# 42yeah/GSRast

Measured on AMD Instinct MI355X. Metric: forward_msplats_per_s, higher is better.
Workload: dtype f32

## Files before the change

### gsrast_amd/_capi.py

```python
from __future__ import annotations

import ctypes as C
import os

import torch

_HERE = os.path.dirname(os.path.abspath(__file__))
_TAG = os.environ.get("GSR_LIB_TAG", "")
LIB_PATH = os.path.join(_HERE, "lib", f"libgsrast_amd{'_' + _TAG if _TAG else ''}.so")

GSR_OK = 0
GSR_ERR_INVALID_ARG = 1
GSR_ERR_ALLOC = 2
GSR_ERR_HIP = 3
GSR_ERR_NO_DEVICE = 4
GSR_ERR_TOO_LARGE = 5
GSR_ERR_INTERNAL = 6
GSR_ERR_STALE_RECEIPT = 7

GSR_FLAG_PROFILE = 0x1
GSR_FLAG_COUNT_STAGED = 0x2
GSR_FLAG_SEMANTICS_INRIA = 0x4
GSR_FLAG_PLAN_SORT = 0x8
GSR_FLAG_PLAN_BLOCKS = 0x10
GSR_FLAG_OVERLAP_EMIT = 0x20
GSR_FLAG_NO_SORTED_LISTS = 0x40
GSR_FLAG_NO_TILE_HISTORY = 0x80
GSR_FLAG_SERIAL_EMIT = 0x100
GSR_FLAG_NO_DEEP_TILES = 0x200
GSR_FLAG_DEEP_TILES_ALL = 0x400
GSR_FLAG_DEEP_WAVES_8 = 0x800
GSR_FLAG_DEEP_WAVES_16 = 0x1000
GSR_FLAG_DEPTH_INVERSE = 0x2000
GSR_PLAN_LISTS_SKIPPED = 0x100
GSR_PLAN_BLEND_FROM_LISTS = 0x200
GSR_PLAN_TILES_REORDERED = 0x400
GSR_PLAN_EMIT_OVERLAPPED = 0x800
GSR_PLAN_COLORS_BESIDE = 0x1000
GSR_PLAN_TILE_ORDER_DROPPED = 0x2000
GSR_PLAN_DEEP_TILES = 0x4000
GSR_SH_LAYOUT_FILE, GSR_SH_LAYOUT_COEFFICIENT_MAJOR = 0, 1
PLAN_NAMES = {0: "none", 1: "sort", 2: "blocks", 3: "generic"}
GSR_NUM_STAGES = 8
STAGE_NAMES = ("preprocess", "scan", "depth_order", "duplicate", "sort_pass1", "sort_pass2", "ranges", "blend")

ALLOC_FN = C.CFUNCTYPE(C.c_void_p, C.c_void_p, C.c_size_t)


class GeometryState(C.Structure):
    _fields_ = [("tiles_touched", C.c_void_p), ("scan_size", C.c_size_t), ("num_rendered", C.c_uint32),
                ("scanning_space", C.c_void_p), ("depths", C.c_void_p), ("clamped", C.c_void_p),
                ("internal_radii", C.c_void_p), ("means2D", C.c_void_p), ("cov3D", C.c_void_p),
                ("conic_opacity", C.c_void_p), ("rgb", C.c_void_p), ("point_offsets", C.c_void_p)]


class ImageState(C.Structure):
    _fields_ = [("ranges", C.c_void_p), ("n_contrib", C.c_void_p), ("accum_alpha", C.c_void_p)]


class BinningState(C.Structure):
    _fields_ = [("keys_unsorted", C.c_void_p), ("keys", C.c_void_p), ("values_unsorted", C.c_void_p),
                ("values", C.c_void_p), ("sorting_size", C.c_size_t), ("sorting_space", C.c_void_p)]


GSR_RECEIPT_MAGIC = 0x31525347
GSR_LISTS_SKIPPED_STAMP = 0xFFFFFFFF


class ForwardReceipt(C.Structure):
    _fields_ = [("magic", C.c_uint32), ("plan_used", C.c_uint32),
                ("num_gaussians", C.c_int32), ("width", C.c_int32), ("height", C.c_int32),
                ("tile_row_begin", C.c_int32), ("tile_row_end", C.c_int32),
                ("num_rendered", C.c_uint32), ("num_visible", C.c_uint32), ("serial", C.c_uint32),
                ("geometry_chunk", C.c_void_p), ("image_chunk", C.c_void_p), ("binning_chunk", C.c_void_p),
                ("async_words", C.c_void_p), ("tile_history", C.c_void_p)]

    def copy(self) -> "ForwardReceipt":
        r = ForwardReceipt()
        C.memmove(C.byref(r), C.byref(self), C.sizeof(ForwardReceipt))
        return r


class ForwardArgs(C.Structure):
    _fields_ = [
        ("struct_size", C.c_uint32), ("flags", C.c_uint32),
        ("geometry_alloc", ALLOC_FN), ("geometry_user", C.c_void_p),
        ("binning_alloc", ALLOC_FN), ("binning_user", C.c_void_p),
        ("image_alloc", ALLOC_FN), ("image_user", C.c_void_p),
        ("num_gaussians", C.c_int32), ("sh_dims", C.c_int32), ("M", C.c_int32),
        ("background", C.c_void_p), ("width", C.c_int32), ("height", C.c_int32),
        ("means3D", C.c_void_p), ("shs", C.c_void_p), ("colors_precomp", C.c_void_p),
        ("opacities", C.c_void_p), ("scales", C.c_void_p), ("scale_modifier", C.c_float),
        ("rotations", C.c_void_p), ("cov3D_precomp", C.c_void_p), ("view_matrix", C.c_void_p),
        ("proj_matrix", C.c_void_p), ("cam_pos", C.c_void_p), ("tan_fovx", C.c_float), ("tan_fovy", C.c_float),
        ("prefiltered", C.c_int32), ("out_color", C.c_void_p), ("radii", C.c_void_p), ("rects", C.c_void_p),
        ("box_min", C.c_void_p), ("box_max", C.c_void_p),
        ("stream", C.c_void_p), ("tile_row_begin", C.c_int32), ("tile_row_end", C.c_int32),
        ("tile_history", C.c_void_p),
        ("num_rendered", C.c_uint32), ("records_staged", C.c_uint64),
        ("stage_ms", C.c_float * GSR_NUM_STAGES),
        ("plan_used", C.c_uint32),
        ("receipt", ForwardReceipt),
        ("out_depth", C.c_void_p),
    ]


class PointsImageState(C.Structure):
    _fields_ = [("depth", C.c_void_p), ("out_color", C.c_void_p), ("default_depth", C.c_void_p), ("winner", C.c_void_p)]


class BackwardArgs(C.Structure):
    _fields_ = [
        ("struct_size", C.c_uint32), ("flags", C.c_uint32),
        ("num_gaussians", C.c_int32), ("width", C.c_int32), ("height", C.c_int32),
        ("background", C.c_void_p),
        ("means2D", C.c_void_p), ("conic_opacity", C.c_void_p), ("colors", C.c_void_p), ("cov3D", C.c_void_p),
        ("radii", C.c_void_p), ("ranges", C.c_void_p), ("n_contrib", C.c_void_p), ("final_t", C.c_void_p),
        ("point_list", C.c_void_p),
        ("means3D", C.c_void_p), ("view_matrix", C.c_void_p), ("tan_fovx", C.c_float), ("tan_fovy", C.c_float),
        ("dL_dout_color", C.c_void_p),
        ("dL_dmean2D", C.c_void_p), ("dL_dconic_opacity", C.c_void_p), ("dL_dcolors", C.c_void_p),
        ("dL_dcov3D", C.c_void_p), ("dL_dshs", C.c_void_p), ("dL_dcov2D", C.c_void_p),
        ("sums_f64", C.c_void_p),
        ("proj_matrix", C.c_void_p), ("scales", C.c_void_p), ("rotations", C.c_void_p), ("scale_modifier", C.c_float),
        ("dL_dmeans3D", C.c_void_p), ("dL_dscales", C.c_void_p), ("dL_drotations", C.c_void_p),
        ("stream", C.c_void_p), ("tile_row_begin", C.c_int32), ("tile_row_end", C.c_int32),
        ("stage_ms", C.c_float * 2),
        ("cam_pos", C.c_void_p), ("shs", C.c_void_p), ("clamped", C.c_void_p), ("sh_dims", C.c_int32),
        ("receipt", ForwardReceipt),
        ("dL_dout_depth", C.c_void_p), ("dL_ddepths", C.c_void_p), ("depth_sums_f64", C.c_void_p),
    ]


class CameraBackwardArgs(C.Structure):
    _fields_ = [
        ("struct_size", C.c_uint32), ("flags", C.c_uint32),
        ("num_gaussians", C.c_int32), ("width", C.c_int32), ("height", C.c_int32),
        ("means3D", C.c_void_p), ("view_matrix", C.c_void_p), ("proj_matrix", C.c_void_p), ("cam_pos", C.c_void_p),
        ("tan_fovx", C.c_float), ("tan_fovy", C.c_float),
        ("cov3D", C.c_void_p), ("radii", C.c_void_p),
        ("shs", C.c_void_p), ("clamped", C.c_void_p), ("sh_dims", C.c_int32),
        ("dL_dmean2D", C.c_void_p), ("dL_dcov2D", C.c_void_p), ("dL_ddepths", C.c_void_p), ("dL_dcolors", C.c_void_p),
        ("dL_dview_matrix", C.c_void_p), ("dL_dproj_matrix", C.c_void_p), ("dL_dcam_pos", C.c_void_p),
        ("scratch", C.c_void_p), ("stream", C.c_void_p), ("stage_ms", C.c_float),
    ]


GSR_ADAM_MAX_TENSORS = 8


class AdamTensor(C.Structure):
    _fields_ = [("param", C.c_void_p), ("grad", C.c_void_p), ("exp_avg", C.c_void_p), ("exp_avg_sq", C.c_void_p),
                ("row_floats", C.c_int32), ("step_size", C.c_float), ("rs", C.c_float), ("b1c", C.c_float),
                ("b2", C.c_float), ("b2c", C.c_float), ("eps", C.c_float)]


class AdamArgs(C.Structure):
    _fields_ = [("struct_size", C.c_uint32), ("num_tensors", C.c_int32), ("num_rows", C.c_int64),
                ("visible", C.c_void_p), ("stream", C.c_void_p), ("tensors", AdamTensor * GSR_ADAM_MAX_TENSORS)]


class PhotoLossArgs(C.Structure):
    _fields_ = [("struct_size", C.c_uint32), ("channels", C.c_int32), ("width", C.c_int32), ("height", C.c_int32),
                ("lambda_dssim", C.c_double), ("image", C.c_void_p), ("target", C.c_void_p), ("scratch", C.c_void_p),
                ("out", C.c_void_p), ("dL_dloss", C.c_void_p), ("dL_dimage", C.c_void_p), ("want_backward", C.c_int32),
                ("stream", C.c_void_p)]


class DensifyArray(C.Structure):
    _fields_ = [("src", C.c_void_p), ("src_exp_avg", C.c_void_p), ("src_exp_avg_sq", C.c_void_p),
                ("dst", C.c_void_p), ("dst_exp_avg", C.c_void_p), ("dst_exp_avg_sq", C.c_void_p)]


class DensifyApplyArgs(C.Structure):
    _fields_ = [("struct_size", C.c_uint32), ("log_shrink", C.c_float), ("n_src", C.c_int64), ("counts", C.c_int32 * 4),
                ("src_of", C.c_void_p), ("noise", C.c_void_p), ("stream", C.c_void_p),
                ("xyz", DensifyArray), ("opacity_logit", DensifyArray), ("log_scale", DensifyArray),
                ("rotation", DensifyArray), ("shs", DensifyArray)]


SIGNATURES = {
    "gsr_geometry_from_chunk": (C.c_void_p, [C.c_void_p, C.c_int, C.POINTER(GeometryState)]),
    "gsr_image_from_chunk": (C.c_void_p, [C.c_void_p, C.c_int, C.POINTER(ImageState)]),
    "gsr_binning_from_chunk": (C.c_void_p, [C.c_void_p, C.c_size_t, C.POINTER(BinningState)]),
    "gsr_required_geometry": (C.c_size_t, [C.c_int]),
    "gsr_required_image": (C.c_size_t, [C.c_int]),
    "gsr_required_binning": (C.c_size_t, [C.c_size_t]),
    "gsr_forward": (C.c_int, [C.POINTER(ForwardArgs)]),
    "gsr_backward": (C.c_int, [C.POINTER(BackwardArgs)]),
    "gsr_camera_backward_scratch_bytes": (C.c_size_t, [C.c_int32]),
    "gsr_camera_backward": (C.c_int, [C.POINTER(CameraBackwardArgs)]),
    "gsr_points_image_from_chunk": (C.c_void_p, [C.c_void_p, C.c_int, C.POINTER(PointsImageState)]),
    "gsr_required_points_image": (C.c_size_t, [C.c_int]),
    "gsr_forward_points": (C.c_int, [C.POINTER(ForwardArgs)]),
    "gsr_last_error": (C.c_int, []),
    "gsr_error_string": (C.c_char_p, [C.c_int]),
    "gsr_last_hip_error": (C.c_char_p, []),
    "gsr_poll_async_error": (C.c_int, [C.POINTER(ForwardReceipt)]),
    "gsr_tile_history_create": (C.c_int, [C.POINTER(C.c_void_p)]),
    "gsr_tile_history_destroy": (C.c_int, [C.c_void_p]),
    "gsr_tile_history_stats": (C.c_int, [C.c_void_p, C.POINTER(C.c_uint32)]),
    "gsr_tile_history_forget_stream": (C.c_int, [C.c_void_p]),
    "gsr_tile_history_times": (C.c_int, [C.c_void_p, C.POINTER(C.c_uint32), C.c_int, C.POINTER(C.c_uint32)]),
    "gsr_thread_release": (C.c_int, []),
    "gsr_reread_environment": (None, []),
    "gsr_device_shape": (None, [C.c_int, C.POINTER(C.c_uint32)]),
    "gsr_higher_msb": (C.c_uint32, [C.c_uint32]),
    "gsr_scan_temp_bytes": (C.c_size_t, [C.c_size_t]),
    "gsr_inclusive_scan_u32": (C.c_int, [C.c_void_p, C.c_void_p, C.c_size_t, C.c_void_p, C.c_void_p]),
    "gsr_sort_temp_bytes": (C.c_size_t, [C.c_size_t]),
    "gsr_sort_pairs_u64_u32": (C.c_int, [C.c_void_p, C.c_void_p, C.c_void_p, C.c_void_p, C.c_size_t, C.c_int, C.c_int,
                                         C.c_void_p, C.c_void_p]),
    "gsr_exchange_unique_id": (C.c_int, [C.c_char_p, C.c_char_p]),
    "gsr_exchange_create": (C.c_int, [C.c_char_p, C.c_char_p, C.c_int, C.c_int, C.POINTER(C.c_void_p)]),
    "gsr_exchange_bands": (C.c_int, [C.c_void_p, C.c_void_p, C.c_int, C.c_int, C.POINTER(C.c_int32), C.c_int, C.c_void_p]),
    "gsr_exchange_plan": (C.c_int, [C.c_int, C.c_int, C.c_int, C.c_int, C.POINTER(C.c_int32), C.c_int, C.c_int,
                                    C.POINTER(C.c_int32), C.POINTER(C.c_int32), C.POINTER(C.c_uint64), C.POINTER(C.c_uint64)]),
    "gsr_exchange_loopback": (C.c_int, [C.c_void_p, C.c_void_p, C.c_void_p, C.c_uint64, C.c_int, C.c_void_p]),
    "gsr_exchange_destroy": (C.c_int, [C.c_void_p]),
    "gsr_exchange_last_error": (C.c_char_p, []),
    "gsr_ply_parse_header": (C.c_int, [C.c_char_p, C.POINTER(C.c_int), C.POINTER(C.c_longlong)]),
    "gsr_ply_activate": (C.c_int, [C.c_void_p, C.c_int, C.c_void_p, C.c_void_p, C.c_void_p, C.c_void_p, C.c_void_p,
                                   C.c_void_p]),
    "gsr_colors_from_dc": (C.c_int, [C.c_int, C.c_void_p, C.c_void_p, C.c_void_p]),
    "gsr_blend_expf": (C.c_int, [C.c_int, C.c_void_p, C.c_void_p, C.c_void_p]),
    "gsr_footprint_misses_tile": (C.c_int, [C.c_int, C.c_void_p, C.c_void_p, C.c_void_p, C.c_int, C.c_int, C.c_void_p, C.c_void_p]),
    "gsr_ply_activate_layout": (C.c_int, [C.c_void_p, C.c_int, C.c_void_p, C.c_void_p, C.c_void_p, C.c_void_p, C.c_void_p,
                                          C.c_int, C.c_void_p]),
    "gsr_activate_params": (C.c_int, [C.c_int] + [C.c_void_p] * 9),
    "gsr_activate_params_backward": (C.c_int, [C.c_int] + [C.c_void_p] * 13),
    "gsr_adam_step": (C.c_int, [C.POINTER(AdamArgs)]),
    "gsr_photo_loss_scratch_bytes": (C.c_size_t, [C.c_int, C.c_int, C.c_int]),
    "gsr_photo_loss_forward": (C.c_int, [C.POINTER(PhotoLossArgs)]),
    "gsr_photo_loss_backward": (C.c_int, [C.POINTER(PhotoLossArgs)]),
    "gsr_densify_accumulate": (C.c_int, [C.c_int64, C.c_void_p, C.c_void_p, C.c_float, C.c_float, C.c_void_p, C.c_void_p,
                                         C.c_void_p, C.c_void_p]),
    "gsr_densify_plan_temp_bytes": (C.c_size_t, [C.c_int64]),
    "gsr_densify_plan": (C.c_int, [C.c_int64] + [C.c_void_p] * 5 + [C.c_float] * 5 + [C.c_int32] + [C.c_void_p] * 4),
    "gsr_densify_apply": (C.c_int, [C.POINTER(DensifyApplyArgs)]),
}

GSR_KNN_LEAF = 64
GSR_KNN_NODE = 32
GSR_KNN_MORTON_BITS = 21
GSR_KNN_MAX_POINTS = 1 << 30
INIT_SIGNATURES = {
    "gsr_knn_temp_bytes": (C.c_size_t, [C.c_int64]),
    "gsr_knn_mean_dist2": (C.c_int, [C.c_int64, C.c_void_p, C.c_void_p, C.c_void_p, C.c_void_p]),
}

OPACITY_SIGNATURES = {
    "gsr_backward_alpha": (C.c_int, [C.POINTER(BackwardArgs), C.c_void_p]),
}

GSR_MCMC_MAX_ROWS = (1 << 31) - 1
GSR_MCMC_MAX_RATIO = 51


class McmcNoiseArgs(C.Structure):
    _fields_ = [("struct_size", C.c_uint32), ("scaler", C.c_float), ("n", C.c_int64), ("xyz", C.c_void_p),
                ("opacity_logit", C.c_void_p), ("log_scale", C.c_void_p), ("rotation", C.c_void_p), ("noise", C.c_void_p),
                ("stream", C.c_void_p)]


class McmcArray(C.Structure):
    _fields_ = [("param", C.c_void_p), ("exp_avg", C.c_void_p), ("exp_avg_sq", C.c_void_p)]


class McmcRelocateArgs(C.Structure):
    _fields_ = [("struct_size", C.c_uint32), ("min_opacity", C.c_float), ("n", C.c_int64), ("m", C.c_int64),
                ("sampled", C.c_void_p), ("dst", C.c_void_p),
                ("xyz", McmcArray), ("opacity_logit", McmcArray), ("log_scale", McmcArray), ("rotation", McmcArray), ("shs", McmcArray),
                ("temp", C.c_void_p), ("stream", C.c_void_p)]


MCMC_SIGNATURES = {
    "gsr_mcmc_noise": (C.c_int, [C.POINTER(McmcNoiseArgs)]),
    "gsr_mcmc_plan_temp_bytes": (C.c_size_t, [C.c_int64]),
    "gsr_mcmc_plan": (C.c_int, [C.c_int64, C.c_void_p, C.c_float, C.c_void_p, C.c_void_p, C.c_void_p, C.c_void_p, C.c_void_p]),
    "gsr_mcmc_relocate_temp_bytes": (C.c_size_t, [C.c_int64]),
    "gsr_mcmc_relocate": (C.c_int, [C.POINTER(McmcRelocateArgs)]),
}

class ContributionArgs(C.Structure):
    _fields_ = [("struct_size", C.c_uint32), ("flags", C.c_uint32),
                ("num_gaussians", C.c_int32), ("width", C.c_int32), ("height", C.c_int32),
                ("means2D", C.c_void_p), ("conic_opacity", C.c_void_p), ("ranges", C.c_void_p), ("n_contrib", C.c_void_p),
                ("point_list", C.c_void_p), ("receipt", ForwardReceipt),
                ("weight_sum", C.c_void_p), ("weight_max", C.c_void_p), ("pixels", C.c_void_p), ("dominant", C.c_void_p),
                ("stream", C.c_void_p), ("stage_ms", C.c_float)]


CONTRIB_SIGNATURES = {
    "gsr_contribution": (C.c_int, [C.POINTER(ContributionArgs)]),
}

_ANTIALIAS_COMMON = [("struct_size", C.c_uint32), ("flags", C.c_uint32),
                     ("num_gaussians", C.c_int32), ("width", C.c_int32), ("height", C.c_int32),
                     ("tan_fovx", C.c_float), ("tan_fovy", C.c_float), ("scale_modifier", C.c_float),
                     ("means3D", C.c_void_p), ("scales", C.c_void_p), ("rotations", C.c_void_p), ("opacities", C.c_void_p),
                     ("view_matrix", C.c_void_p), ("proj_matrix", C.c_void_p)]


class AntialiasArgs(C.Structure):
    _fields_ = _ANTIALIAS_COMMON + [("opacities_out", C.c_void_p), ("compensation", C.c_void_p), ("stream", C.c_void_p)]


class AntialiasBackwardArgs(C.Structure):
    _fields_ = _ANTIALIAS_COMMON + [("dL_dopacities_out", C.c_void_p), ("radii", C.c_void_p),
                                    ("dL_dopacities", C.c_void_p), ("dL_dmeans3D", C.c_void_p), ("dL_dscales", C.c_void_p),
                                    ("dL_drotations", C.c_void_p), ("stream", C.c_void_p)]


ANTIALIAS_SIGNATURES = {
    "gsr_antialias_forward": (C.c_int, [C.POINTER(AntialiasArgs)]),
    "gsr_antialias_backward": (C.c_int, [C.POINTER(AntialiasBackwardArgs)]),
}

GSR_FILTER3D_CAMERA_FLOATS = 20
GSR_FILTER3D_CAMERA_CHUNK = 64


class Filter3dObserveArgs(C.Structure):
    _fields_ = [("struct_size", C.c_uint32), ("flags", C.c_uint32),
                ("num_gaussians", C.c_int32), ("position_stride", C.c_int32), ("num_cameras", C.c_int32),
                ("positions", C.c_void_p), ("cameras", C.c_void_p), ("min_depth", C.c_void_p), ("stream", C.c_void_p)]


class Filter3dFinalizeArgs(C.Structure):
    _fields_ = [("struct_size", C.c_uint32), ("flags", C.c_uint32), ("num_gaussians", C.c_int32), ("max_focal", C.c_float),
                ("min_depth", C.c_void_p), ("filter", C.c_void_p), ("temp", C.c_void_p), ("temp_bytes", C.c_size_t),
                ("stream", C.c_void_p)]


class Filter3dArgs(C.Structure):
    _fields_ = [("struct_size", C.c_uint32), ("flags", C.c_uint32), ("num_gaussians", C.c_int32),
                ("scales", C.c_void_p), ("opacities", C.c_void_p), ("filter", C.c_void_p),
                ("scales_out", C.c_void_p), ("opacities_out", C.c_void_p), ("stream", C.c_void_p)]


class Filter3dBackwardArgs(C.Structure):
    _fields_ = [("struct_size", C.c_uint32), ("flags", C.c_uint32), ("num_gaussians", C.c_int32),
                ("scales", C.c_void_p), ("opacities", C.c_void_p), ("filter", C.c_void_p),
                ("dL_dscales_out", C.c_void_p), ("dL_dopacities_out", C.c_void_p), ("radii", C.c_void_p),
                ("dL_dscales", C.c_void_p), ("dL_dopacities", C.c_void_p), ("stream", C.c_void_p)]


FILTER3D_SIGNATURES = {
    "gsr_filter3d_temp_bytes": (C.c_size_t, [C.c_int32]),
    "gsr_filter3d_observe": (C.c_int, [C.POINTER(Filter3dObserveArgs)]),
    "gsr_filter3d_finalize": (C.c_int, [C.POINTER(Filter3dFinalizeArgs)]),
    "gsr_filter3d_forward": (C.c_int, [C.POINTER(Filter3dArgs)]),
    "gsr_filter3d_backward": (C.c_int, [C.POINTER(Filter3dBackwardArgs)]),
}

class AbsgradArgs(C.Structure):
    _fields_ = [("struct_size", C.c_uint32), ("flags", C.c_uint32), ("backward", C.POINTER(BackwardArgs)),
                ("dL_dout_alpha", C.c_void_p), ("abs_dL_dmean2D", C.c_void_p), ("sums_f64", C.c_void_p), ("stage_ms", C.c_float)]


ABSGRAD_SIGNATURES = {
    "gsr_absgrad": (C.c_int, [C.POINTER(AbsgradArgs)]),
}

GSR_FEATURES_MAX_CHANNELS = 256
GSR_FEATURES_CHUNK = 16
GSR_FEATURES_CHUNK_NARROW = 8


class FeaturesArgs(C.Structure):
    _fields_ = [("struct_size", C.c_uint32), ("flags", C.c_uint32),
                ("num_gaussians", C.c_int32), ("width", C.c_int32), ("height", C.c_int32), ("channels", C.c_int32),
                ("means2D", C.c_void_p), ("conic_opacity", C.c_void_p), ("ranges", C.c_void_p), ("n_contrib", C.c_void_p),
                ("final_t", C.c_void_p), ("point_list", C.c_void_p), ("receipt", ForwardReceipt),
                ("features", C.c_void_p), ("background", C.c_void_p), ("out", C.c_void_p),
                ("dL_dout", C.c_void_p), ("dL_dfeatures", C.c_void_p), ("feature_sums_f64", C.c_void_p),
                ("geometry_sums_f64", C.c_void_p),
                ("tile_row_begin", C.c_int32), ("tile_row_end", C.c_int32), ("stream", C.c_void_p), ("stage_ms", C.c_float)]


FEATURES_SIGNATURES = {
    "gsr_features_temp_bytes": (C.c_size_t, [C.c_int32, C.c_int32]),
    "gsr_features_forward": (C.c_int, [C.POINTER(FeaturesArgs)]),
    "gsr_features_backward": (C.c_int, [C.POINTER(FeaturesArgs)]),
}

class DistortionArgs(C.Structure):
    _fields_ = [("struct_size", C.c_uint32), ("flags", C.c_uint32),
                ("num_gaussians", C.c_int32), ("width", C.c_int32), ("height", C.c_int32), ("power", C.c_int32),
                ("means2D", C.c_void_p), ("conic_opacity", C.c_void_p), ("ranges", C.c_void_p), ("n_contrib", C.c_void_p),
                ("final_t", C.c_void_p), ("point_list", C.c_void_p), ("receipt", ForwardReceipt),
                ("values", C.c_void_p), ("out", C.c_void_p), ("moments", C.c_void_p),
                ("dL_dout", C.c_void_p), ("dL_dvalues", C.c_void_p), ("value_sums_f64", C.c_void_p),
                ("geometry_sums_f64", C.c_void_p),
                ("tile_row_begin", C.c_int32), ("tile_row_end", C.c_int32), ("stream", C.c_void_p), ("stage_ms", C.c_float)]


DISTORTION_SIGNATURES = {
    "gsr_distortion_temp_bytes": (C.c_size_t, [C.c_int32]),
    "gsr_distortion_forward": (C.c_int, [C.POINTER(DistortionArgs)]),
    "gsr_distortion_backward": (C.c_int, [C.POINTER(DistortionArgs)]),
}

_GAUSSIAN_NORMALS_COMMON = [("struct_size", C.c_uint32), ("flags", C.c_uint32), ("num_gaussians", C.c_int32),
                            ("means3D", C.c_void_p), ("scales", C.c_void_p), ("rotations", C.c_void_p), ("view_matrix", C.c_void_p)]
_DEPTH_NORMALS_COMMON = [("struct_size", C.c_uint32), ("flags", C.c_uint32), ("width", C.c_int32), ("height", C.c_int32),
                         ("tan_fovx", C.c_float), ("tan_fovy", C.c_float), ("depth", C.c_void_p)]


class GaussianNormalsArgs(C.Structure):
    _fields_ = _GAUSSIAN_NORMALS_COMMON + [("normals", C.c_void_p), ("stream", C.c_void_p)]


class GaussianNormalsBackwardArgs(C.Structure):
    _fields_ = _GAUSSIAN_NORMALS_COMMON + [("dL_dnormals", C.c_void_p), ("radii", C.c_void_p), ("dL_drotations", C.c_void_p),
                                           ("stream", C.c_void_p)]


class DepthNormalsArgs(C.Structure):
    _fields_ = _DEPTH_NORMALS_COMMON + [("normals", C.c_void_p), ("stream", C.c_void_p)]


class DepthNormalsBackwardArgs(C.Structure):
    _fields_ = _DEPTH_NORMALS_COMMON + [("dL_dnormals", C.c_void_p), ("dL_ddepth", C.c_void_p), ("stream", C.c_void_p)]


NORMALS_SIGNATURES = {
    "gsr_gaussian_normals_forward": (C.c_int, [C.POINTER(GaussianNormalsArgs)]),
    "gsr_gaussian_normals_backward": (C.c_int, [C.POINTER(GaussianNormalsBackwardArgs)]),
    "gsr_depth_normals_forward": (C.c_int, [C.POINTER(DepthNormalsArgs)]),
    "gsr_depth_normals_backward": (C.c_int, [C.POINTER(DepthNormalsBackwardArgs)]),
}

GSR_MEDIAN_NONE = 0xFFFFFFFF


class MedianArgs(C.Structure):
    _fields_ = [("struct_size", C.c_uint32), ("flags", C.c_uint32),
                ("num_gaussians", C.c_int32), ("width", C.c_int32), ("height", C.c_int32), ("threshold", C.c_float),
                ("means2D", C.c_void_p), ("conic_opacity", C.c_void_p), ("ranges", C.c_void_p), ("n_contrib", C.c_void_p),
                ("final_t", C.c_void_p), ("point_list", C.c_void_p), ("receipt", ForwardReceipt),
                ("values", C.c_void_p), ("out", C.c_void_p), ("ids", C.c_void_p), ("dominant_ids", C.c_void_p),
                ("dL_dout", C.c_void_p), ("dL_dvalues", C.c_void_p), ("value_sums_f64", C.c_void_p),
                ("tile_row_begin", C.c_int32), ("tile_row_end", C.c_int32), ("stream", C.c_void_p), ("stage_ms", C.c_float)]


MEDIAN_SIGNATURES = {
    "gsr_median_temp_bytes": (C.c_size_t, [C.c_int32]),
    "gsr_median_forward": (C.c_int, [C.POINTER(MedianArgs)]),
    "gsr_median_backward": (C.c_int, [C.POINTER(MedianArgs)]),
}

_lib = None


class GsrError(RuntimeError):
    def __init__(self, code: int, where: str):
        L = lib()
        msg = L.gsr_error_string(code).decode()
        hip = L.gsr_last_hip_error().decode()
        super().__init__(f"{where}: {msg} (code {code})" + (f" [{hip}]" if hip else ""))
        self.code = code


def lib() -> C.CDLL:
    global _lib
    if _lib is None:
        if not os.path.exists(LIB_PATH):
            raise RuntimeError(
                f"{LIB_PATH} is missing: build the HIP library first (python -m gsrast_amd.build). "
                "gsrast_amd has no CPU or PyTorch fallback.")
        L = C.CDLL(LIB_PATH)
        for name, (res, args) in (list(SIGNATURES.items()) + list(INIT_SIGNATURES.items()) + list(OPACITY_SIGNATURES.items())
                                  + list(MCMC_SIGNATURES.items()) + list(CONTRIB_SIGNATURES.items()) + list(ANTIALIAS_SIGNATURES.items())
                                  + list(FILTER3D_SIGNATURES.items()) + list(ABSGRAD_SIGNATURES.items())
                                  + list(FEATURES_SIGNATURES.items()) + list(DISTORTION_SIGNATURES.items())
                                  + list(NORMALS_SIGNATURES.items()) + list(MEDIAN_SIGNATURES.items())):
            fn = getattr(L, name, None)
            if fn is None and _TAG:
                continue
            if fn is None:
                raise RuntimeError(f"{LIB_PATH} does not export {name}: rebuild it (python -m gsrast_amd.build)")
            fn.restype = res
            fn.argtypes = args
        _lib = L
    return _lib


def check(code: int, where: str) -> None:
    if code != GSR_OK:
        raise GsrError(code, where)


def call(name: str, *args, device=None, where: "str | None" = None) -> None:
    fn = getattr(lib(), name)
    if device is None:
        code = fn(*args)
    else:
        with torch.cuda.device(device):
            code = fn(*args)
    check(code, where or name)


def stream(device) -> int:
    return torch.cuda.current_stream(device).cuda_stream


def aligned16(t: torch.Tensor) -> torch.Tensor:
    t = t.contiguous()
    return t if t.data_ptr() % 16 == 0 else t.clone()
```

### gsrast_amd/build.py

```python
from __future__ import annotations

import os
import subprocess
import sys
from concurrent.futures import ThreadPoolExecutor

HERE = os.path.dirname(os.path.abspath(__file__))
CSRC = os.path.join(HERE, "csrc")
LIB_DIR = os.path.join(HERE, "lib")
OBJ_DIR = os.path.join(LIB_DIR, "obj")
LIB_PATH = os.path.join(LIB_DIR, "libgsrast_amd.so")

HIPCC = os.environ.get("HIPCC", "/opt/rocm/bin/hipcc")
ARCH = "gfx950"
COMMON = (["--offload-arch=" + ARCH, "-O3", "-std=c++17", "-fPIC", "-ffp-contract=off", "-Wall", "-Wno-unused-function"]
          + os.environ.get("GSR_DEFINES", "").split())
PER_FILE = {"antialias.hip": ["-fno-slp-vectorize"]}


def _sources():
    return sorted(f for f in os.listdir(CSRC) if f.endswith(".hip"))


def _headers_mtime() -> float:
    paths = [os.path.join(CSRC, f) for f in os.listdir(CSRC) if f.endswith((".hpp", ".h"))]
    paths += [os.path.join(HERE, "..", "include", h) for h in ("gsrast_amd.h", "gsrast_amd_init.h", "gsrast_amd_opacity.h", "gsrast_amd_mcmc.h",
                                                                      "gsrast_amd_contrib.h", "gsrast_amd_antialias.h", "gsrast_amd_filter3d.h", "gsrast_amd_absgrad.h",
                                                                      "gsrast_amd_features.h", "gsrast_amd_distortion.h", "gsrast_amd_normals.h", "gsrast_amd_median.h")]
    return max(os.path.getmtime(p) for p in paths)


def _compile(src: str, force: bool, obj_dir: str = OBJ_DIR) -> str:
    obj = os.path.join(obj_dir, src[:-4] + ".o")
    spath = os.path.join(CSRC, src)
    stale = (force or not os.path.exists(obj) or os.path.getmtime(obj) < os.path.getmtime(spath)
             or os.path.getmtime(obj) < _headers_mtime())
    if stale:
        cmd = [HIPCC] + COMMON + PER_FILE.get(src, []) + ["-c", spath, "-o", obj]
        r = subprocess.run(cmd, capture_output=True, text=True)
        if r.returncode != 0:
            raise RuntimeError(f"hipcc failed for {src}:\n{r.stdout}\n{r.stderr}")
        if r.stderr.strip():
            sys.stderr.write(r.stderr)
    return obj


def build(force: bool = False, verbose: bool = False, tag: str = "") -> str:
    obj_dir = OBJ_DIR + ("_" + tag if tag else "")
    lib_path = LIB_PATH if not tag else os.path.join(LIB_DIR, f"libgsrast_amd_{tag}.so")
    force = force or bool(tag)
    os.makedirs(obj_dir, exist_ok=True)
    srcs = _sources()
    with ThreadPoolExecutor(max_workers=min(4, len(srcs))) as ex:
        objs = list(ex.map(lambda s: _compile(s, force, obj_dir), srcs))
    newest = max(os.path.getmtime(o) for o in objs)
    if force or not os.path.exists(lib_path) or os.path.getmtime(lib_path) < newest:
        cmd = [HIPCC, "--offload-arch=" + ARCH, "-shared", "-fPIC", "-o", lib_path] + objs + ["-ldl"]
        r = subprocess.run(cmd, capture_output=True, text=True)
        if r.returncode != 0:
            raise RuntimeError(f"link failed:\n{r.stdout}\n{r.stderr}")
    if verbose:
        print("built", lib_path)
    return lib_path


if __name__ == "__main__":
    _tag = sys.argv[sys.argv.index("--tag") + 1] if "--tag" in sys.argv else ""
    build(force="--force" in sys.argv, verbose=True, tag=_tag)
```

### gsrast_amd/csrc/backward.hip

```cpp
#include <hip/hip_runtime.h>
#include <hip/amd_detail/amd_hip_unsafe_atomics.h>

#include "backward_policy.hpp"
#include "../../include/gsrast_amd_opacity.h"
#include "blend_core.hpp"
#include "blockbin.hpp"
#include "gaussian_chain.hpp"
#include "wave_reduce.hpp"

namespace gsr {
namespace {

struct RenderBackwardParams {
    const uint2* ranges;
    const uint32_t* point_list;
    BlockFeed feed;
    const float2* means2D;
    const float* colors;
    const float4* conic_opacity;
    const float* final_t;
    const uint32_t* n_contrib;
    const float* background;
    const float* dL_dout;
    float* dL_dmean2D;
    float* dL_dconic_opacity;
    float* dL_dcolors;
    float* dL_dcov2D;
    double* sums64;
    FrameDims dims;
    int num_tiles;
    const uint32_t* tile_order;
    const float* dL_dout_depth;
    const float4* means3D;
    const float* view;
    uint32_t depth_inverse;
    float* dL_ddepths;
    double* depth_sums64;
    const float* dL_dout_alpha;
};

__device__ __forceinline__ float wave_sum12(float a0, float a1, float a2, float a3, float a4, float a5, float a6, float a7, float a8,
                                            float a9, float a10, float a11) {
    const int lane = threadIdx.x & (kWave - 1);
    const float u = wave_sum8(a0, a1, a2, a3, a4, a5, a6, a7, lane);
    const float w = wave_sum4(a8, a9, a10, a11);
    return (lane & 7) == 4 ? w : u;
}

constexpr uint32_t kAccMaxUnits = 2;
constexpr uint32_t kAccFloats = 12;
template <bool DEPTH> constexpr uint32_t kAccOf = DEPTH ? kAccFloats + 1u : kAccFloats;
template <bool DEPTH>
__device__ __forceinline__ bool block_acc_fits(const BlockFeed& f, uint32_t b) {
    return f.acc != nullptr && (unsigned long long)kAccOf<DEPTH> * (unsigned long long)f.meta.list_start()[f.meta.nbp] <= f.acc_floats &&
           f.meta.walked()[b] <= kAccMaxUnits;
}

constexpr uint32_t kAccParts = 4;
template <bool DEPTH>
__device__ __forceinline__ void walked_slice(const BlockFeed& f, size_t& e0, size_t& e1) {
    const uint32_t b = blockIdx.x / kAccParts, part = blockIdx.x % kAccParts;
    e0 = e1 = 0;
    if (!block_acc_fits<DEPTH>(f, b)) return;
    const size_t first = f.meta.list_start()[b], end = f.meta.list_start()[b + 1];
    const size_t upto = min(end, first + (size_t)f.meta.walked()[b] * kUnit);
    const size_t per = ((upto - first + kAccParts - 1) / kAccParts + 3) / 4 * 4;
    e0 = min(upto, first + part * per);
    e1 = min(upto, e0 + per);
}

template <bool DEPTH>
__global__ __launch_bounds__(256) void zero_block_acc_kernel(const BlockFeed f) {
    constexpr uint32_t kAcc = kAccOf<DEPTH>;
    size_t e0, e1;
    walked_slice<DEPTH>(f, e0, e1);
    for (size_t i = kAcc * e0 + threadIdx.x; i < kAcc * e1; i += 256) f.acc[i] = 0.0f;
}

template <bool DEPTH>
__global__ __launch_bounds__(256) void flush_block_acc_kernel(const BlockFeed f, float* __restrict__ dL_dmean2D,
                                                              float* __restrict__ dL_dconic_opacity, float* __restrict__ dL_dcolors,
                                                              float* __restrict__ dL_dcov2D, double* __restrict__ sums64,
                                                              float* __restrict__ dL_ddepths, double* __restrict__ depth_sums64) {
    constexpr uint32_t kAcc = kAccOf<DEPTH>;
    size_t e0, e1;
    walked_slice<DEPTH>(f, e0, e1);
    for (size_t e = e0 + threadIdx.x; e < e1; e += 256) {
        const float* a = f.acc + kAcc * e;
        float v[kAcc];
#pragma unroll
        for (int k = 0; k < (int)kAcc; ++k) v[k] = a[k];
        bool any = false;
#pragma unroll
        for (int k = 0; k < (int)kAcc; ++k) any = any || v[k] != 0.0f;
        if (!any) continue;
        const size_t id = f.ent_idx[e];
        if constexpr (DEPTH) {
            if (v[kAccFloats] != 0.0f) {
                if (sums64) unsafeAtomicAdd(depth_sums64 + id, (double)v[kAccFloats]);
                else unsafeAtomicAdd(dL_ddepths + id, v[kAccFloats]);
            }
        }
        if (sums64) {
#pragma unroll
            for (int k = 0; k < (int)kAccFloats; ++k)
                if (v[k] != 0.0f) unsafeAtomicAdd(sums64 + kAccFloats * id + k, (double)v[k]);
            continue;
        }
        unsafeAtomicAdd(dL_dmean2D + 2 * id, v[0]); unsafeAtomicAdd(dL_dmean2D + 2 * id + 1, v[1]);
        unsafeAtomicAdd(dL_dconic_opacity + 4 * id, v[2]); unsafeAtomicAdd(dL_dconic_opacity + 4 * id + 1, v[3]);
        unsafeAtomicAdd(dL_dconic_opacity + 4 * id + 2, v[4]); unsafeAtomicAdd(dL_dconic_opacity + 4 * id + 3, v[5]);
        unsafeAtomicAdd(dL_dcolors + 3 * id, v[6]); unsafeAtomicAdd(dL_dcolors + 3 * id + 1, v[7]); unsafeAtomicAdd(dL_dcolors + 3 * id + 2, v[8]);
        if (dL_dcov2D) {
            unsafeAtomicAdd(dL_dcov2D + 4 * id, v[9]); unsafeAtomicAdd(dL_dcov2D + 4 * id + 1, v[10]); unsafeAtomicAdd(dL_dcov2D + 4 * id + 2, v[11]);
        }
    }
}

template <bool DEPTH> struct DepthSlots { __device__ static float* get() { return nullptr; } };
template <> struct DepthSlots<true> {
    __device__ static float* get() {
        __shared__ float s_dep[kWave];
        return s_dep;
    }
};

template <bool DEPTH, bool ALPHA>
__global__ __launch_bounds__(64) void render_backward_kernel(const RenderBackwardParams p) {
    float* const s_dep = DepthSlots<DEPTH>::get();
    __shared__ uint32_t s_id[kWave];
    __shared__ float2 s_xy[kWave];
    __shared__ float4 s_co[kWave];
    __shared__ float4 s_rgb[kWave];
    __shared__ float s_floor[kWave];
    __shared__ unsigned long long s_exp[32];
    exp_table_init(s_exp, (int)threadIdx.x);

    const int tile_local = tile_of_workgroup(p.tile_order ? (int)p.tile_order[blockIdx.x] : (int)blockIdx.x, p.dims.grid_x, p.dims.row_end - p.dims.row_begin);
    if (tile_local < 0) return;
    const int tile = p.dims.row_begin * p.dims.grid_x + tile_local;
    const int tx = tile % p.dims.grid_x, ty = tile / p.dims.grid_x;
    const int lane = threadIdx.x;
    const int px = tx * kTile + (lane & 15), py0 = ty * kTile + (lane >> 4);
    const float fx = (float)px;
    const size_t plane = (size_t)p.dims.width * (size_t)p.dims.height;
    const float bg0 = p.background[0], bg1 = p.background[1], bg2 = p.background[2];

    uint32_t last[4];
    float T[4], S[4], g0[4], g1[4], g2[4], fy[4];
    float gd[4] = {0.0f, 0.0f, 0.0f, 0.0f};
    uint32_t hi = 0;
#pragma unroll
    for (int k = 0; k < 4; ++k) {
        const int py = py0 + 4 * k;
        fy[k] = (float)py;
        const bool inside = px < p.dims.width && py < p.dims.height;
        last[k] = 0; T[k] = 1.0f; g0[k] = g1[k] = g2[k] = 0.0f;
        [[maybe_unused]] float ga = 0.0f;
        if (inside) {
            const size_t pid = (size_t)py * (size_t)p.dims.width + (size_t)px;
            last[k] = p.n_contrib[pid];
            T[k] = p.final_t[pid];
            g0[k] = p.dL_dout[pid]; g1[k] = p.dL_dout[pid + plane]; g2[k] = p.dL_dout[pid + 2 * plane];
            if constexpr (DEPTH) gd[k] = p.dL_dout_depth[pid];
            if constexpr (ALPHA) ga = p.dL_dout_alpha[pid];
        }
        if constexpr (ALPHA) S[k] = T[k] * ((bg0 * g0[k] + bg1 * g1[k] + bg2 * g2[k]) - ga);
        else S[k] = T[k] * (bg0 * g0[k] + bg1 * g1[k] + bg2 * g2[k]);
        hi = max(hi, last[k]);
    }
#pragma unroll
    for (int off = 32; off > 0; off >>= 1) hi = max(hi, (uint32_t)__shfl_xor((int)hi, off, kWave));
    if (hi == 0) return;
    const uint2 range = p.ranges[tile];
    const TileBox box = tile_box(tx, ty, p.dims.width, p.dims.height);

    constexpr uint32_t kAcc = kAccOf<DEPTH>;
    constexpr int kSumOfRow[8] = {0, 4, 2, 6, 1, 5, 3, 7};
    constexpr int kSumOfRow4[4] = {8, 10, 9, 11};
    int my_sum = (lane & 7) == 0 ? kSumOfRow[lane >> 3] : ((lane & 15) == 4 ? kSumOfRow4[lane >> 4] : -1);
    if (my_sum >= 9 && !p.dL_dcov2D && !p.sums64) my_sum = -1;
    float* direct_base = my_sum < 2 ? p.dL_dmean2D + my_sum : (my_sum < 6 ? p.dL_dconic_opacity + (my_sum - 2) :
                         (my_sum < 9 ? p.dL_dcolors + (my_sum - 6) : p.dL_dcov2D + (my_sum - 9)));
    const uint32_t direct_stride = my_sum < 2 ? 2u : (my_sum < 6 ? 4u : (my_sum < 9 ? 3u : 4u));
    bool per_entry = false;
    auto walk_batch = [&](const bool present, const uint32_t id, const uint32_t idx_l, const uint32_t key, const float2 xy_l,
                          const float4 co_l) {
        const bool keep = present && !record_misses_tile(xy_l, co_l, box);
        const unsigned long long kept_mask = __ballot(keep);
        if (keep) {
            const uint32_t slot = __builtin_amdgcn_mbcnt_hi((uint32_t)(kept_mask >> 32), __builtin_amdgcn_mbcnt_lo((uint32_t)kept_mask, 0u));
            s_id[slot] = key;
            s_xy[slot] = xy_l;
            s_co[slot] = co_l;
            const float* col = p.colors + 3 * (size_t)id;
            s_rgb[slot] = make_float4(col[0], col[1], col[2], __uint_as_float(idx_l));
            if constexpr (DEPTH) {
                const float4 m = p.means3D[id];
                const float z = (p.view[2] * m.x + p.view[6] * m.y) + (p.view[10] * m.z + p.view[14] * 1.0f);
                s_dep[slot] = p.depth_inverse ? 1.0f / z : z;
            }
            const float op = co_l.w;
            s_floor[slot] = !(op > -__builtin_inff()) ? -__builtin_inff() : (op <= 0.0f ? __builtin_inff() : -__logf(255.0f * op) - 1e-3f);
        }
        for (int j = (int)__popcll(kept_mask) - 1; j >= 0; --j) {
            const uint32_t idx0 = __float_as_uint(s_rgb[j].w);
            const float2 xy = s_xy[j];
            const float4 co = s_co[j];
            const float dx = xy.x - fx;
            float a_mx = 0.0f, a_my = 0.0f, a_A = 0.0f, a_B = 0.0f, a_C = 0.0f, a_op = 0.0f, a_r = 0.0f, a_g = 0.0f, a_b = 0.0f;
            float a_m00 = 0.0f, a_m01 = 0.0f, a_m11 = 0.0f;
            float a_d = 0.0f;
            float dep = 0.0f;
            if constexpr (DEPTH) dep = s_dep[j];
            bool any = false;
            const float4 col = s_rgb[j];
            const float hxx = -0.5f * dx * dx, flo = s_floor[j];
#pragma unroll
            for (int k = 0; k < 4; ++k) {
                const unsigned long long inlist = __ballot(idx0 < last[k]);
                if (inlist == 0ull) continue;
                const float dy = xy.y - fy[k];
                const float power = -0.5f * (co.x * dx * dx + co.z * dy * dy) - co.y * dx * dy;
                const unsigned long long cand = inlist & ~__ballot(power > 0.0f) & __ballot(power >= flo);
                if (cand == 0ull) continue;
                const float G = exp_ref(power, s_exp);
                const float raw = co.w * G;
                const float alpha = fminf(0.99f, raw);
                const unsigned long long act_mask = cand & ~__ballot(alpha < 1.0f / 255.0f);
                if (act_mask == 0ull) continue;
                const bool act = __builtin_amdgcn_inverse_ballot_w64(act_mask);
                any = true;
                const float inv = __builtin_amdgcn_rcpf(1.0f - alpha);
                const float Tn = T[k] * inv;
                T[k] = act ? Tn : T[k];
                float cg = __builtin_fmaf(col.x, g0[k], __builtin_fmaf(col.y, g1[k], col.z * g2[k]));
                if constexpr (DEPTH) cg = __builtin_fmaf(dep, gd[k], cg);
                const float w = act ? alpha * Tn : 0.0f;
                a_r = __builtin_fmaf(w, g0[k], a_r); a_g = __builtin_fmaf(w, g1[k], a_g); a_b = __builtin_fmaf(w, g2[k], a_b);
                if constexpr (DEPTH) a_d = __builtin_fmaf(w, gd[k], a_d);
                const float dL_dalpha = __builtin_fmaf(Tn, cg, -(S[k] * inv));
                S[k] = __builtin_fmaf(cg, w, S[k]);
                const bool live = __builtin_amdgcn_inverse_ballot_w64(act_mask & ~__ballot(raw > 0.99f));
                const float gop = live ? G * dL_dalpha : 0.0f;
                const float dpow = live ? raw * dL_dalpha : 0.0f;
                a_op += gop;
                a_A = __builtin_fmaf(hxx, dpow, a_A);
                a_B = __builtin_fmaf(-(dx * dy), dpow, a_B);
                a_C = __builtin_fmaf(-0.5f * dy * dy, dpow, a_C);
                const float ux = __builtin_fmaf(co.x, dx, co.y * dy), uy = __builtin_fmaf(co.y, dx, co.z * dy);
                a_mx = __builtin_fmaf(-ux, dpow, a_mx);
                a_my = __builtin_fmaf(-uy, dpow, a_my);
                const float hux = 0.5f * dpow * ux, huy = 0.5f * dpow * uy;
                a_m00 = __builtin_fmaf(hux, ux, a_m00); a_m01 = __builtin_fmaf(hux, uy, a_m01); a_m11 = __builtin_fmaf(huy, uy, a_m11);
            }
            if (!any) continue;
            const float total = wave_sum12(a_mx, a_my, a_A, a_B, a_C, a_op, a_r, a_g, a_b, a_m00, a_m01, a_m11);
            if (my_sum >= 0) {
                const size_t key = s_id[j];
                if (!per_entry && p.sums64) unsafeAtomicAdd(p.sums64 + kAccFloats * key + my_sum, (double)total);
                else unsafeAtomicAdd(per_entry ? p.feed.acc + kAcc * key + my_sum : direct_base + direct_stride * key, total);
            }
            if constexpr (DEPTH) {
                float td = a_d;
#pragma unroll
                for (int off = 32; off > 0; off >>= 1) td += __shfl_xor(td, off, kWave);
                if (lane == 2 && td != 0.0f) {
                    const size_t key = s_id[j];
                    if (per_entry) unsafeAtomicAdd(p.feed.acc + kAcc * key + kAccFloats, td);
                    else if (p.depth_sums64) unsafeAtomicAdd(p.depth_sums64 + key, (double)td);
                    else unsafeAtomicAdd(p.dL_ddepths + key, td);
                }
            }
        }
    };

    struct Batch {
        bool valid = false, present = false;
        uint32_t id = 0, idx_l = 0, key = 0;
        float2 xy = {0.0f, 0.0f};
        float4 co = {0.0f, 0.0f, 0.0f, 0.0f};
    };
    const BlockFeed& f = p.feed;
    const uint32_t b = (uint32_t)(ty / kBH) * (uint32_t)f.nbx + (uint32_t)(tx / kBW);
    per_entry = f.ent_idx != nullptr && block_acc_fits<DEPTH>(f, b);
    const bool sorted = p.point_list && !per_entry;
    int it_c = (int)((hi - 1) / kWave);
    const uint32_t col = (uint32_t)(tx % kBW), row = 8u + (uint32_t)(ty % kBH), t_in_block = (uint32_t)((ty % kBH) * kBW + tx % kBW);
    uint32_t u0 = 0, list0 = 0, it_u = 0, it_nz = 0, tm_lo = 0, tm_hi = 0, start_v = 0;
    if (!sorted) {
        u0 = f.meta.unit_start()[b];
        const uint32_t u1 = f.meta.unit_start()[b + 1];
        list0 = f.meta.list_start()[b];
        uint32_t below = 0;
        for (uint32_t k = u0; k < u1; k += kWave) {
            const uint32_t u = k + (uint32_t)lane;
            below += (uint32_t)__popcll(__ballot(u < u1 && f.prefix[(size_t)u * 64 + t_in_block] < hi));
        }
        it_u = u0 + below;
    }
    auto next_batch = [&]() {
        Batch nb;
        if (sorted) {
            if (it_c < 0) return nb;
            const uint32_t first = (uint32_t)it_c * kWave;
            --it_c;
            nb.valid = true;
            nb.present = (uint32_t)lane < min((uint32_t)kWave, hi - first);
            nb.idx_l = first + (uint32_t)lane;
            nb.id = p.point_list[range.x + (nb.present ? nb.idx_l : 0u)];
            nb.key = nb.id;
            return nb;
        }
        while (it_nz == 0u) {
            if (it_u == u0) return nb;
            --it_u;
            const uint32_t base = f.prefix[(size_t)it_u * 64 + t_in_block];
            const uint2* um = f.unit_masks + (size_t)it_u * 16 * kBatches + (lane & (kBatches - 1));
            const uint2 xm = um[col * kBatches], ym = um[row * kBatches];
            tm_lo = (lane < kBatches) ? (xm.x & ym.x) : 0u;
            tm_hi = (lane < kBatches) ? (xm.y & ym.y) : 0u;
            const uint32_t c = (uint32_t)__popc(tm_lo) + (uint32_t)__popc(tm_hi);
            start_v = base + prefix32_inclusive(c) - c;
            it_nz = (uint32_t)__ballot(c != 0u && start_v < hi);
        }
        const int w = 31 - __builtin_clz(it_nz);
        it_nz &= ~(1u << w);
        const uint32_t lo = (uint32_t)__builtin_amdgcn_readlane((int)tm_lo, w);
        const uint32_t hi_m = (uint32_t)__builtin_amdgcn_readlane((int)tm_hi, w);
        const uint32_t start = (uint32_t)__builtin_amdgcn_readlane((int)start_v, w);
        const unsigned long long mask = ((unsigned long long)hi_m << 32) | lo;
        nb.valid = true;
        nb.idx_l = start + __builtin_amdgcn_mbcnt_hi(hi_m, __builtin_amdgcn_mbcnt_lo(lo, 0u));
        nb.present = __builtin_amdgcn_inverse_ballot_w64(mask) && nb.idx_l < hi;
        const uint32_t e = list0 + (it_u - u0) * kUnit + (uint32_t)w * kWave + (uint32_t)lane;
        nb.id = f.ent_idx[nb.present ? e : list0];
        nb.key = per_entry ? e : nb.id;
        return nb;
    };
    auto fetch = [&](Batch& nb) {
        const uint32_t at = (nb.valid && nb.present) ? nb.id : 0u;
        nb.xy = p.means2D[at];
        nb.co = p.conic_opacity[at];
    };
    Batch b0 = next_batch();
    fetch(b0);
    Batch b1 = next_batch();
    while (b0.valid) {
        fetch(b1);
        Batch b2 = next_batch();
        walk_batch(b0.present, b0.id, b0.idx_l, b0.key, b0.xy, b0.co);
        b0 = b1;
        b1 = b2;
    }
}

struct PreprocessBackwardParams {
    int n;
    const float4* means3D;
    const float* cov3D;
    const int32_t* radii;
    const float* view;
    float tan_fovx, tan_fovy, focal;
    const float4* dL_dconic_opacity;
    const float4* dL_dcov2D;
    double* sums64;
    float2* out_mean2D; float4* out_conic_opacity; float* out_colors; float4* out_cov2D;
    const float* dL_dcolors;
    int chain;
    float* dL_dcov3D;
    float* dL_dshs;
    const float* proj;
    const float4* scales;
    const float4* rotations;
    float scale_modifier;
    int width, height;
    const float2* dL_dmean2D;
    float4* dL_dmeans3D;
    float4* dL_dscales;
    float4* dL_drotations;
    int inria, sh_deg;
    float focal_x, focal_y, w_eps;
    const float* shs;
    const float* cam_pos;
    const uint8_t* clamped;
    int depth, depth_inverse;
    const float* dL_ddepths;
    double* depth_sums64;
    float* out_ddepths;
};

__constant__ float kShC2[5] = {1.0925484305920792f, -1.0925484305920792f, 0.31539156525252005f, -1.0925484305920792f,
                               0.5462742152960396f};
__constant__ float kShC3[7] = {-0.5900435899266435f, 2.890611442640554f, -0.4570457994644658f, 0.3731763325901154f,
                               -0.4570457994644658f, 1.445305721320277f, -0.5900435899266435f};

__device__ __forceinline__ void sh_basis_grad(int deg, float x, float y, float z, float (&B)[16], float (&G)[16][3]) {
    constexpr float C0 = 0.28209479177387814f, C1 = 0.4886025119029199f;
#pragma unroll
    for (int k = 0; k < 16; ++k) { B[k] = 0.0f; G[k][0] = G[k][1] = G[k][2] = 0.0f; }
    B[0] = C0;
    if (deg > 0) {
        B[1] = -C1 * y; B[2] = C1 * z; B[3] = -C1 * x;
        G[1][1] = -C1; G[2][2] = C1; G[3][0] = -C1;
    }
    if (deg > 1) {
        const float xx = x * x, yy = y * y, zz = z * z, xy = x * y, yz = y * z, xz = x * z;
        B[4] = kShC2[0] * xy; B[5] = kShC2[1] * yz; B[6] = kShC2[2] * (2.0f * zz - xx - yy); B[7] = kShC2[3] * xz; B[8] = kShC2[4] * (xx - yy);
        G[4][0] = kShC2[0] * y; G[4][1] = kShC2[0] * x;
        G[5][1] = kShC2[1] * z; G[5][2] = kShC2[1] * y;
        G[6][0] = -2.0f * kShC2[2] * x; G[6][1] = -2.0f * kShC2[2] * y; G[6][2] = 4.0f * kShC2[2] * z;
        G[7][0] = kShC2[3] * z; G[7][2] = kShC2[3] * x;
        G[8][0] = 2.0f * kShC2[4] * x; G[8][1] = -2.0f * kShC2[4] * y;
        if (deg > 2) {
            B[9] = kShC3[0] * y * (3.0f * xx - yy); B[10] = kShC3[1] * xy * z; B[11] = kShC3[2] * y * (4.0f * zz - xx - yy);
            B[12] = kShC3[3] * z * (2.0f * zz - 3.0f * xx - 3.0f * yy); B[13] = kShC3[4] * x * (4.0f * zz - xx - yy);
            B[14] = kShC3[5] * z * (xx - yy); B[15] = kShC3[6] * x * (xx - 3.0f * yy);
            G[9][0] = kShC3[0] * 6.0f * xy; G[9][1] = kShC3[0] * (3.0f * xx - 3.0f * yy);
            G[10][0] = kShC3[1] * yz; G[10][1] = kShC3[1] * xz; G[10][2] = kShC3[1] * xy;
            G[11][0] = kShC3[2] * -2.0f * xy; G[11][1] = kShC3[2] * (4.0f * zz - xx - 3.0f * yy); G[11][2] = kShC3[2] * 8.0f * yz;
            G[12][0] = kShC3[3] * -6.0f * xz; G[12][1] = kShC3[3] * -6.0f * yz; G[12][2] = kShC3[3] * (6.0f * zz - 3.0f * xx - 3.0f * yy);
            G[13][0] = kShC3[4] * (4.0f * zz - 3.0f * xx - yy); G[13][1] = kShC3[4] * -2.0f * xy; G[13][2] = kShC3[4] * 8.0f * xz;
            G[14][0] = kShC3[5] * 2.0f * xz; G[14][1] = kShC3[5] * -2.0f * yz; G[14][2] = kShC3[5] * (xx - yy);
            G[15][0] = kShC3[6] * (3.0f * xx - 3.0f * yy); G[15][1] = kShC3[6] * -6.0f * xy;
        }
    }
}

constexpr int kShRow = 49;
template <bool INRIA>
__global__ __launch_bounds__(256) void preprocess_backward_kernel(const PreprocessBackwardParams p) {
    __shared__ float s_sh[INRIA ? 4 * kWave * kShRow : 1];
    const int idx = blockIdx.x * 256 + threadIdx.x;
    const bool valid = idx < p.n;
    const bool has_tile = valid && (p.radii == nullptr || p.radii[idx] > 0);
    const bool visible = has_tile && p.chain != 0;
    float4 mean = make_float4(0.0f, 0.0f, 0.0f, 0.0f), g = mean, sc = mean, rot = mean;
    float2 g2 = make_float2(0.0f, 0.0f), c3a = g2, c3b = g2, c3c = g2;
    float gc[3] = {0.0f, 0.0f, 0.0f};
    double sum[12] = {0, 0, 0, 0, 0, 0, 0, 0, 0, 0, 0, 0};
    if (has_tile && p.sums64) {
        const double2* sp = reinterpret_cast<const double2*>(p.sums64 + 12 * (size_t)idx);
#pragma unroll
        for (int k = 0; k < 6; ++k) { const double2 v2 = sp[k]; sum[2 * k] = v2.x; sum[2 * k + 1] = v2.y; }
    }
    double gdep = 0.0;
    if (p.depth && has_tile) gdep = p.sums64 ? p.depth_sums64[idx] : (p.chain ? (double)p.dL_ddepths[idx] : 0.0);
    if (visible) {
        mean = p.means3D[idx];
        const float2* c3p = reinterpret_cast<const float2*>(p.cov3D + 6 * (size_t)idx);
        c3a = c3p[0]; c3b = c3p[1]; c3c = c3p[2];
        if (!p.sums64) {
            g = p.dL_dconic_opacity[idx];
            if (p.dL_dmeans3D) g2 = p.dL_dmean2D[idx];
            if (p.dL_dshs) {
                const float* gcp = p.dL_dcolors + 3 * (size_t)idx;
                gc[0] = gcp[0]; gc[1] = gcp[1]; gc[2] = gcp[2];
            }
            if (p.dL_dcov2D) { const float4 gcv = p.dL_dcov2D[idx]; sum[9] = gcv.x; sum[10] = gcv.y; sum[11] = gcv.z; }
            sum[0] = g2.x; sum[1] = g2.y; sum[2] = g.x; sum[3] = g.y; sum[4] = g.z; sum[5] = g.w; sum[6] = gc[0]; sum[7] = gc[1]; sum[8] = gc[2];
        }
        if (p.dL_dscales) { sc = p.scales[idx]; rot = p.rotations[idx]; }
    }
    if (p.sums64) { gc[0] = (float)sum[6]; gc[1] = (float)sum[7]; gc[2] = (float)sum[8]; }
    const bool have_cov2D = p.sums64 != nullptr || p.dL_dcov2D != nullptr;
    typedef double R;
    R out[6] = {0, 0, 0, 0, 0, 0};
    R gmean[3] = {0, 0, 0};
    if (visible) {
        float txf, tyf, tzf;
        view_point<false>(p.view, mean, txf, tyf, tzf);
        const RatioClamp cl = clamp_ratios_libm(txf, tyf, tzf, 1.3f * p.tan_fovx, 1.3f * p.tan_fovy);
        const ProjectionFrame f = projection_frame(p.view, (R)tzf, (R)cl.cx, (R)cl.cy, cl.clx, cl.cly, INRIA ? (R)p.focal_x : (R)p.focal,
                                                   INRIA ? (R)p.focal_y : (R)p.focal);
        const R c3[6] = {(R)c3a.x, (R)c3a.y, (R)c3b.x, (R)c3b.y, (R)c3c.x, (R)c3c.y};
        const R s[3][3] = {{c3[0], c3[1], c3[2]}, {c3[1], c3[3], c3[4]}, {c3[2], c3[4], c3[5]}};
        R a, b, cc;
        cov2d_f64(f, s, a, b, cc);
        a = a + 0.3;
        cc = cc + 0.3;
        const R det = a * cc - b * b;
        if (det != 0.0) {
            R m00 = sum[9], m01 = sum[10], m11 = sum[11];
            if (!have_cov2D) {
                const R inv = 1.0 / det;
                const R k00 = cc * inv, k01 = -b * inv, k11 = a * inv;
                const R q00 = sum[2], q01 = 0.5 * sum[3], q11 = sum[4];
                const R r00 = k00 * q00 + k01 * q01, r01 = k00 * q01 + k01 * q11;
                const R r10 = k01 * q00 + k11 * q01, r11 = k01 * q01 + k11 * q11;
                m00 = -(r00 * k00 + r01 * k01); m01 = -(r00 * k01 + r01 * k11);
                m11 = -(r10 * k01 + r11 * k11);
            }
            R gS[3][3];
            sigma_gradient(f, m00, m01, m11, gS);
            out[0] = gS[0][0]; out[1] = 2.0 * gS[0][1]; out[2] = 2.0 * gS[0][2];
            out[3] = gS[1][1]; out[4] = 2.0 * gS[1][2]; out[5] = gS[2][2];
            if (p.dL_dmeans3D) mean_gradient(f, s, m00, m01, m11, gmean);
        }
        if (p.dL_dmeans3D) {
            const float* pm = p.proj;
            const R mw_ = INRIA ? 1.0 : (R)mean.w;
            const R mx = (R)mean.x, my = (R)mean.y, mz = (R)mean.z;
            const R hx = ((R)pm[0] * mx + (R)pm[4] * my) + ((R)pm[8] * mz + (R)pm[12] * mw_);
            const R hy = ((R)pm[1] * mx + (R)pm[5] * my) + ((R)pm[9] * mz + (R)pm[13] * mw_);
            const R wp = (INRIA ? (R)p.w_eps : (R)0.001f) + (((R)pm[3] * mx + (R)pm[7] * my) + ((R)pm[11] * mz + (R)pm[15] * mw_));
            const R iw = 1.0 / wp, iw2 = iw * iw;
#pragma unroll
            for (int j = 0; j < 3; ++j) {
                const R dx = 0.5 * (R)p.width * ((R)pm[4 * j + 0] * iw - hx * (R)pm[4 * j + 3] * iw2);
                const R dy = 0.5 * (R)p.height * ((R)pm[4 * j + 1] * iw - hy * (R)pm[4 * j + 3] * iw2);
                gmean[j] += dx * sum[0] + dy * sum[1];
            }
            if (p.depth) {
                const R gz = p.depth_inverse ? -gdep / (f.tz * f.tz) : gdep;
#pragma unroll
                for (int j = 0; j < 3; ++j) gmean[j] += gz * f.v[4 * j + 2];
            }
        }
    }
    [[maybe_unused]] const int lane = threadIdx.x & (kWave - 1), wave = threadIdx.x / kWave;
    [[maybe_unused]] float* sh_rows = s_sh + (INRIA ? wave * kWave * kShRow : 0);
    [[maybe_unused]] const size_t sh_first = ((size_t)blockIdx.x * 256 + (size_t)wave * kWave) * 48, sh_limit = (size_t)p.n * 48;
    if constexpr (INRIA) {
        if (p.dL_dshs) {
            const int terms = (p.sh_deg + 1) * (p.sh_deg + 1);
            if (__ballot(visible) != 0ull) {
                const int pieces = p.sh_deg > 2 ? 12 : (p.sh_deg > 1 ? 7 : (p.sh_deg > 0 ? 3 : 1));
                float4 piece[12];
#pragma unroll
                for (int q = 0; q < 12; ++q) {
                    const int f4 = q * kWave + lane;
                    const size_t at = sh_first + 4 * (size_t)f4;
                    piece[q] = ((f4 % 12) < pieces && at + 3 < sh_limit) ? *reinterpret_cast<const float4*>(p.shs + at)
                                                                        : make_float4(0.0f, 0.0f, 0.0f, 0.0f);
                }
#pragma unroll
                for (int q = 0; q < 12; ++q) {
                    const int f4 = q * kWave + lane;
                    float* dst = sh_rows + (f4 / 12) * kShRow + (f4 % 12) * 4;
                    dst[0] = piece[q].x; dst[1] = piece[q].y; dst[2] = piece[q].z; dst[3] = piece[q].w;
                }
            }
            float* row = sh_rows + lane * kShRow;
            float dx = 0.0f, dy = 0.0f, dz = 0.0f, il = 0.0f;
            float B[16], G[16][3];
            float g[3] = {0.0f, 0.0f, 0.0f};
            if (visible) {
                dx = mean.x - p.cam_pos[0]; dy = mean.y - p.cam_pos[1]; dz = mean.z - p.cam_pos[2];
                const float len = sqrtf(dx * dx + dy * dy + dz * dz);
                il = 1.0f / len;
                dx *= il; dy *= il; dz *= il;
#pragma unroll
                for (int c = 0; c < 3; ++c) g[c] = p.clamped[3 * (size_t)idx + c] ? 0.0f : gc[c];
            }
            sh_basis_grad(p.sh_deg, dx, dy, dz, B, G);
            float gd[3] = {0.0f, 0.0f, 0.0f};
#pragma unroll
            for (int k = 0; k < 16; ++k) {
                const bool on = visible && k < terms;
                if (on) {
                    const float w = row[3 * k] * g[0] + row[3 * k + 1] * g[1] + row[3 * k + 2] * g[2];
                    gd[0] += G[k][0] * w; gd[1] += G[k][1] * w; gd[2] += G[k][2] * w;
                }
                row[3 * k] = on ? B[k] * g[0] : 0.0f;
                row[3 * k + 1] = on ? B[k] * g[1] : 0.0f;
                row[3 * k + 2] = on ? B[k] * g[2] : 0.0f;
            }
            if (visible) {
                const float dot = dx * gd[0] + dy * gd[1] + dz * gd[2];
                gmean[0] += (gd[0] - dx * dot) * il; gmean[1] += (gd[1] - dy * dot) * il; gmean[2] += (gd[2] - dz * dot) * il;
            }
        }
    }
    R gsc[3] = {0, 0, 0}, gq[4] = {0, 0, 0, 0};
    if (p.dL_dscales && visible) {
        const R gS[3][3] = {{out[0], 0.5 * out[1], 0.5 * out[2]}, {0.5 * out[1], out[3], 0.5 * out[4]}, {0.5 * out[2], 0.5 * out[4], out[5]}};
        const R mod = (R)p.scale_modifier;
        const R sv[3] = {mod * (R)sc.x, mod * (R)sc.y, mod * (R)sc.z};
        R Rm[3][3], qn[4], inv, gR[3][3];
        rotation_f64<INRIA>(rot, Rm, qn, inv);
        scale_rotation_gradient(gS, Rm, sv, mod, gsc, gR);
        quaternion_gradient<INRIA>(gR, qn, inv, gq);
    }
    if constexpr (INRIA) {
        if (p.dL_dshs) {
#pragma unroll
            for (int q = 0; q < 12; ++q) {
                const int f4 = q * kWave + lane;
                const size_t at = sh_first + 4 * (size_t)f4;
                const float* src = sh_rows + (f4 / 12) * kShRow + (f4 % 12) * 4;
                if (at + 3 < sh_limit) *reinterpret_cast<float4*>(p.dL_dshs + at) = make_float4(src[0], src[1], src[2], src[3]);
            }
        }
    }
    if (valid && p.sums64) {
        if (p.out_mean2D) p.out_mean2D[idx] = make_float2((float)sum[0], (float)sum[1]);
        if (p.out_conic_opacity) p.out_conic_opacity[idx] = make_float4((float)sum[2], (float)sum[3], (float)sum[4], (float)sum[5]);
        if (p.out_colors) {
            float* oc = p.out_colors + 3 * (size_t)idx;
            oc[0] = (float)sum[6]; oc[1] = (float)sum[7]; oc[2] = (float)sum[8];
        }
        if (p.out_cov2D) p.out_cov2D[idx] = make_float4((float)sum[9], (float)sum[10], (float)sum[11], 0.0f);
        if (p.depth) {
            if (p.out_ddepths) p.out_ddepths[idx] = (float)gdep;
            if (gdep != 0.0) p.depth_sums64[idx] = 0.0;
        }
        bool touched = false;
#pragma unroll
        for (int k = 0; k < 12; ++k) touched = touched || sum[k] != 0.0;
        if (touched) {
            double2* sp = reinterpret_cast<double2*>(p.sums64 + 12 * (size_t)idx);
#pragma unroll
            for (int k = 0; k < 6; ++k) sp[k] = make_double2(0.0, 0.0);
        }
    }
    if (valid && p.chain) {
        if (p.dL_dmeans3D) p.dL_dmeans3D[idx] = make_float4((float)gmean[0], (float)gmean[1], (float)gmean[2], 0.0f);
        if (p.dL_dscales) {
            p.dL_dscales[idx] = make_float4((float)gsc[0], (float)gsc[1], (float)gsc[2], 0.0f);
            if (p.dL_drotations) p.dL_drotations[idx] = make_float4((float)gq[0], (float)gq[1], (float)gq[2], (float)gq[3]);
        }
        if (p.dL_dcov3D) {
            float2* dst = reinterpret_cast<float2*>(p.dL_dcov3D + 6 * (size_t)idx);
            dst[0] = make_float2((float)out[0], (float)out[1]);
            dst[1] = make_float2((float)out[2], (float)out[3]);
            dst[2] = make_float2((float)out[4], (float)out[5]);
        }
    }
    if (p.dL_dshs && !INRIA) {
        const float v0 = visible ? 0.4f * gc[0] : 0.0f, v1 = visible ? 0.4f * gc[1] : 0.0f, v2 = visible ? 0.4f * gc[2] : 0.0f;
        const int q = lane & 3;
        const size_t wave_first = (size_t)idx - (size_t)lane;
#pragma unroll
        for (int it = 0; it < 4; ++it) {
            const int src = it * 16 + (lane >> 2);
            const float a = __shfl(v0, src, kWave), b = __shfl(v1, src, kWave), c = __shfl(v2, src, kWave);
            const size_t gi = wave_first + (size_t)src;
            if (gi < (size_t)p.n)
            {
                typedef float f32x4 __attribute__((ext_vector_type(4)));
                const f32x4 val = {q == 0 ? a : 0.0f, q == 0 ? b : 0.0f, q == 0 ? c : 0.0f, 0.0f};
                __builtin_nontemporal_store(val, reinterpret_cast<f32x4*>(p.dL_dshs + 48 * gi) + q);
            }
        }
    }
}


struct BackwardCall {
    gsr_backward_args* const a;
    const hipStream_t stream;
    const BackwardChoice choice;
    const float* const dL_dout_alpha;
    BlockFeed feed = {};
    bool from_blocks = false, lists_written = true, nothing_rendered = false;
    CallEvents<3> events;

    BackwardCall(gsr_backward_args* a_, const BackwardChoice& choice_, const float* alpha_)
        : a(a_), stream((hipStream_t)a_->stream), choice(choice_), dL_dout_alpha(alpha_) {}
    int begin_profile() { if (choice.profile) GSR_TRY(events.create()); return mark(0); }
    int mark(int k) { if (choice.profile) GSR_HIP_TRY(hipEventRecord(events.ev[k], stream)); return GSR_OK; }
};

int resolve_lists(BackwardCall& c) {
    const gsr_backward_args* const a = c.a;
    const FrameDims& d = c.choice.d;
    if (c.choice.have_receipt) {
        GSR_TRY(lists_of_receipt(a->receipt, a->num_gaussians, a->width, a->height, d.row_begin, d.row_end, a->point_list, &c.feed,
                                 &c.from_blocks, &c.lists_written));
        c.nothing_rendered = a->receipt.num_rendered == 0;
        return GSR_OK;
    }
    uint32_t first = 0;
    GSR_HIP_TRY(hipMemcpyAsync(&first, a->point_list, sizeof(first), hipMemcpyDeviceToHost, c.stream));
    GSR_HIP_TRY(hipStreamSynchronize(c.stream));
    return first == GSR_LISTS_SKIPPED_STAMP ? GSR_ERR_INVALID_ARG : GSR_OK;
}

int clear_range(const BackwardCall& c, int first, int last) {
    for (int k = first; k < last; ++k) {
        const BackwardOutput& o = kBackwardOutputs[k];
        float* const array = c.a->*o.array;
        if (!array || (o.array == &gsr_backward_args::dL_ddepths && !c.choice.depth)) continue;
        GSR_HIP_TRY(hipMemsetAsync(array, 0, sizeof(float) * (size_t)o.row_floats * (size_t)c.a->num_gaussians, c.stream));
    }
    return GSR_OK;
}

int clear_outputs(const BackwardCall& c) {
    return (!c.choice.wide || c.nothing_rendered) ? clear_range(c, 0, kBackwardSums) : GSR_OK;
}

int finish_without_instances(const BackwardCall& c) {
    return clear_range(c, kBackwardSums, (int)(sizeof(kBackwardOutputs) / sizeof(kBackwardOutputs[0])));
}

RenderBackwardParams render_params(const BackwardCall& c) {
    const gsr_backward_args* const a = c.a;
    const FrameDims& d = c.choice.d;
    RenderBackwardParams r;
    r.ranges = reinterpret_cast<const uint2*>(a->ranges);
    r.point_list = c.lists_written ? a->point_list : nullptr;
    r.feed = c.feed;
    r.means2D = reinterpret_cast<const float2*>(a->means2D);
    r.colors = a->colors;
    r.conic_opacity = reinterpret_cast<const float4*>(a->conic_opacity);
    r.final_t = a->final_t;
    r.n_contrib = a->n_contrib;
    r.background = a->background;
    r.dL_dout = a->dL_dout_color;
    r.dL_dmean2D = a->dL_dmean2D;
    r.dL_dconic_opacity = a->dL_dconic_opacity;
    r.dL_dcolors = a->dL_dcolors;
    r.dL_dcov2D = a->dL_dcov2D;
    r.sums64 = a->sums_f64;
    r.dims = d;
    r.num_tiles = (d.row_end - d.row_begin) * d.grid_x;
    r.tile_order = c.choice.have_receipt ? tile_order_of_call(a->receipt, d.row_begin, d.row_end) : nullptr;
    r.dL_dout_depth = a->dL_dout_depth;
    r.means3D = reinterpret_cast<const float4*>(a->means3D);
    r.view = a->view_matrix;
    r.depth_inverse = c.choice.depth_inverse ? 1u : 0u;
    r.dL_ddepths = a->dL_ddepths;
    r.depth_sums64 = c.choice.wide ? a->depth_sums_f64 : nullptr;
    r.dL_dout_alpha = c.dL_dout_alpha;
    return r;
}

PreprocessBackwardParams chain_params(const BackwardCall& c, const RenderBackwardParams& r) {
    const gsr_backward_args* const a = c.a;
    const ProfileLens lens = profile_lens(c.choice.inria, a->width, a->height, a->tan_fovx, a->tan_fovy, a->sh_dims);
    PreprocessBackwardParams q;
    q.n = a->num_gaussians;
    q.means3D = reinterpret_cast<const float4*>(a->means3D);
    q.cov3D = a->cov3D;
    q.radii = a->radii;
    q.view = a->view_matrix;
    q.tan_fovx = a->tan_fovx; q.tan_fovy = a->tan_fovy;
    q.focal = lens.focal_y;
    q.dL_dconic_opacity = reinterpret_cast<const float4*>(a->dL_dconic_opacity);
    q.dL_dcov2D = reinterpret_cast<const float4*>(a->dL_dcov2D);
    q.sums64 = a->sums_f64;
    q.out_mean2D = reinterpret_cast<float2*>(a->dL_dmean2D);
    q.out_conic_opacity = reinterpret_cast<float4*>(a->dL_dconic_opacity);
    q.out_colors = a->dL_dcolors;
    q.out_cov2D = reinterpret_cast<float4*>(a->dL_dcov2D);
    q.dL_dcolors = a->dL_dcolors;
    q.dL_dcov3D = a->dL_dcov3D;
    q.chain = c.choice.chain ? 1 : 0;
    q.dL_dshs = c.choice.chain ? a->dL_dshs : nullptr;
    q.proj = a->proj_matrix;
    q.scales = reinterpret_cast<const float4*>(a->scales);
    q.rotations = reinterpret_cast<const float4*>(a->rotations);
    q.scale_modifier = a->scale_modifier;
    q.width = a->width; q.height = a->height;
    q.dL_dmean2D = reinterpret_cast<const float2*>(a->dL_dmean2D);
    q.dL_dmeans3D = reinterpret_cast<float4*>(a->dL_dmeans3D);
    q.dL_dscales = reinterpret_cast<float4*>(a->dL_dscales);
    q.dL_drotations = reinterpret_cast<float4*>(a->dL_drotations);
    q.inria = c.choice.inria ? 1 : 0;
    q.sh_deg = lens.sh_deg;
    q.focal_x = lens.focal_x; q.focal_y = lens.focal_y; q.w_eps = lens.w_eps;
    q.depth = c.choice.depth ? 1 : 0;
    q.depth_inverse = (int)r.depth_inverse;
    q.dL_ddepths = a->dL_ddepths;
    q.depth_sums64 = r.depth_sums64;
    q.out_ddepths = a->dL_ddepths;
    q.shs = a->shs; q.cam_pos = a->cam_pos; q.clamped = a->clamped;
    return q;
}

template <bool DEPTH>
int launch_render_as(const BackwardCall& c, const RenderBackwardParams& r) {
    const gsr_backward_args* const a = c.a;
    const FrameDims& d = c.choice.d;
    const unsigned acc_wgs = (unsigned)(((d.grid_x + kBW - 1) / kBW) * ((d.grid_y + kBH - 1) / kBH)) * kAccParts;
    const bool per_entry = c.from_blocks && c.feed.acc;
    if (per_entry) {
        hipLaunchKernelGGL(zero_block_acc_kernel<DEPTH>, dim3(acc_wgs), dim3(256), 0, c.stream, c.feed);
        GSR_LAUNCH_CHECK("zero_block_acc_kernel");
    }
    const dim3 grid((unsigned)patch_workgroups(d.grid_x, d.row_end - d.row_begin));
    if (c.choice.alpha) hipLaunchKernelGGL((render_backward_kernel<DEPTH, true>), grid, dim3(kWave), 0, c.stream, r);
    else hipLaunchKernelGGL((render_backward_kernel<DEPTH, false>), grid, dim3(kWave), 0, c.stream, r);
    GSR_LAUNCH_CHECK("render_backward_kernel");
    if (per_entry) {
        hipLaunchKernelGGL(flush_block_acc_kernel<DEPTH>, dim3(acc_wgs), dim3(256), 0, c.stream, c.feed, a->dL_dmean2D,
                           a->dL_dconic_opacity, a->dL_dcolors, a->dL_dcov2D, a->sums_f64, r.dL_ddepths, r.depth_sums64);
        GSR_LAUNCH_CHECK("flush_block_acc_kernel");
    }
    return GSR_OK;
}
int launch_render(const BackwardCall& c, const RenderBackwardParams& r) {
    if (r.num_tiles <= 0) return GSR_OK;
    return c.choice.depth ? launch_render_as<true>(c, r) : launch_render_as<false>(c, r);
}

int launch_chain(const BackwardCall& c, const PreprocessBackwardParams& q) {
    const dim3 grid((unsigned)((q.n + 255) / 256));
    if (c.choice.inria) hipLaunchKernelGGL(preprocess_backward_kernel<true>, grid, dim3(256), 0, c.stream, q);
    else hipLaunchKernelGGL(preprocess_backward_kernel<false>, grid, dim3(256), 0, c.stream, q);
    GSR_LAUNCH_CHECK("preprocess_backward_kernel");
    return GSR_OK;
}

int read_profile(BackwardCall& c) {
    if (!c.choice.profile) return GSR_OK;
    GSR_HIP_TRY(hipStreamSynchronize(c.stream));
    GSR_HIP_TRY(hipEventElapsedTime(&c.a->stage_ms[0], c.events.ev[0], c.events.ev[1]));
    GSR_HIP_TRY(hipEventElapsedTime(&c.a->stage_ms[1], c.events.ev[1], c.events.ev[2]));
    return GSR_OK;
}

int backward_stages(BackwardCall& c) {
    GSR_TRY(resolve_lists(c));
    GSR_TRY(clear_outputs(c));
    if (c.nothing_rendered) return finish_without_instances(c);
    GSR_TRY(c.begin_profile());
    const RenderBackwardParams r = render_params(c);
    GSR_TRY(launch_render(c, r));
    GSR_TRY(c.mark(1));
    if (c.choice.chain || c.choice.wide) GSR_TRY(launch_chain(c, chain_params(c, r)));
    GSR_TRY(c.mark(2));
    return read_profile(c);
}

}
}

using namespace gsr;

static int backward_impl(gsr_backward_args* a, const float* dL_dout_alpha) {
    if (!a || a->struct_size != sizeof(gsr_backward_args)) return GSR_ERR_INVALID_ARG;
    a->stage_ms[0] = a->stage_ms[1] = 0.0f;
    BackwardChoice choice;
    GSR_TRY(choose_backward(*a, &choice, dL_dout_alpha));
    BackwardCall call(a, choice, dL_dout_alpha);
    return backward_stages(call);
}

extern "C" int gsr_backward(gsr_backward_args* a) { return entry_point(backward_impl, a, (const float*)nullptr); }
extern "C" int gsr_backward_alpha(gsr_backward_args* a, const float* dL_dout_alpha) { return entry_point(backward_impl, a, dL_dout_alpha); }
```

### gsrast_amd/csrc/backward_policy.hpp

```cpp
#pragma once
#include <stddef.h>
#include <stdint.h>

#include "../../include/gsrast_amd.h"
#include "frame_policy.hpp"

namespace gsr {

struct BackwardChoice {
    bool wide;
    bool chain;
    bool depth;
    bool inria;
    bool have_receipt;
    bool profile;
    bool depth_inverse;
    bool alpha;
    FrameDims d;
};

inline int choose_backward(const gsr_backward_args& a, BackwardChoice* out, const float* dL_dout_alpha = nullptr) {
    BackwardChoice c{};
    if (a.num_gaussians <= 0 || a.width <= 0 || a.height <= 0 || !a.background || !a.means2D || !a.conic_opacity || !a.colors ||
        !a.ranges || !a.n_contrib || !a.final_t || !a.dL_dout_color)
        return GSR_ERR_INVALID_ARG;
    c.wide = a.sums_f64 != nullptr;
    if (!c.wide && (!a.dL_dmean2D || !a.dL_dconic_opacity || !a.dL_dcolors)) return GSR_ERR_INVALID_ARG;
    c.chain = a.dL_dcov3D || (c.wide && (a.dL_dmeans3D || a.dL_dscales || a.dL_dshs));
    if (c.chain && (!a.cov3D || !a.means3D || !a.view_matrix || !a.radii)) return GSR_ERR_INVALID_ARG;
    if ((a.dL_dmeans3D || a.dL_dscales || a.dL_drotations) && !c.chain) return GSR_ERR_INVALID_ARG;
    if (a.dL_dmeans3D && !a.proj_matrix) return GSR_ERR_INVALID_ARG;
    if ((a.dL_dscales || a.dL_drotations) && (!a.scales || !a.rotations || !a.dL_dscales)) return GSR_ERR_INVALID_ARG;
    c.inria = (a.flags & GSR_FLAG_SEMANTICS_INRIA) != 0;
    if (c.inria && a.dL_dshs && (!a.shs || !a.cam_pos || !a.clamped || !a.means3D)) return GSR_ERR_INVALID_ARG;
    c.depth = a.dL_dout_depth != nullptr;
    if (c.depth && (!a.means3D || !a.view_matrix || (c.wide ? !a.depth_sums_f64 : !a.dL_ddepths))) return GSR_ERR_INVALID_ARG;
    c.alpha = dL_dout_alpha != nullptr;
    c.profile = (a.flags & GSR_FLAG_PROFILE) != 0;
    c.depth_inverse = (a.flags & GSR_FLAG_DEPTH_INVERSE) != 0;
    if (tile_band(a.width, a.height, a.tile_row_begin, a.tile_row_end, &c.d) != GSR_OK) return GSR_ERR_INVALID_ARG;
    c.have_receipt = a.receipt.magic != 0;
    if (!c.have_receipt && !a.point_list) return GSR_ERR_INVALID_ARG;
    *out = c;
    return GSR_OK;
}

struct ProfileLens { float focal_x, focal_y, w_eps; int sh_deg; };
inline ProfileLens profile_lens(bool inria, int width, int height, float tan_fovx, float tan_fovy, int sh_dims) {
    ProfileLens l;
    l.focal_y = (float)height / (2.0f * tan_fovy);
    l.focal_x = inria ? (float)width / (2.0f * tan_fovx) : l.focal_y;
    l.w_eps = inria ? 0.0000001f : 0.001f;
    l.sh_deg = sh_dims < 0 ? 0 : (sh_dims > 3 ? 3 : sh_dims);
    return l;
}

struct BackwardOutput { float* gsr_backward_args::*array; int row_floats; };
constexpr int kBackwardSums = 5;
constexpr BackwardOutput kBackwardOutputs[] = {
    {&gsr_backward_args::dL_dmean2D, 2},  {&gsr_backward_args::dL_dconic_opacity, 4}, {&gsr_backward_args::dL_dcolors, 3},
    {&gsr_backward_args::dL_dcov2D, 4},   {&gsr_backward_args::dL_ddepths, 1},
    {&gsr_backward_args::dL_dcov3D, 6},   {&gsr_backward_args::dL_dshs, 48},          {&gsr_backward_args::dL_dmeans3D, 4},
    {&gsr_backward_args::dL_dscales, 4},  {&gsr_backward_args::dL_drotations, 4},
};

}
```

### gsrast_amd/csrc/distortion.hip

```cpp
#include <hip/hip_runtime.h>

#include "list_walk.hpp"
#include "../../include/gsrast_amd_distortion.h"

namespace gsr {
namespace {

struct DistortionParams {
    WalkFrame frame;
    const float* values;
    float* out;
    float* moments;
    const float* dL_dout;
    double* value_sums;
    double* geometry_sums;
};

struct DistortionStage : ReplayStage {
    float value[kWave];
};

template <int POWER>
__global__ __launch_bounds__(kWave) void distortion_forward_kernel(const DistortionParams p) {
    __shared__ DistortionStage st;
    const int lane = (int)threadIdx.x;
    int tx, ty;
    const int tile = walk_tile(p.frame, &tx, &ty);
    if (tile < 0) return;
    const size_t plane = (size_t)p.frame.dims.width * (size_t)p.frame.dims.height;

    TileLanes s;
    tile_lanes_init(s, tx, ty, lane, p.frame.dims.width, p.frame.dims.height, -1);
    float D[4] = {}, M1[4] = {}, M2[4] = {}, m0[4] = {};

    replay_walk(p.frame, tile, tx, ty, lane, s, st, [&](const TileBox& box, const RecordBatch& b) {
        const uint32_t kept = stage_replay(box, st, b, p.frame.num_gaussians, [&](uint32_t slot, uint32_t id) {
            st.value[slot] = p.values[id];
        });
        for (uint32_t j = 0; j < kept; ++j) {
            const ReplayRecord r = replay_candidates(s, st, j);
            if (!r.any()) continue;
            const float m = st.value[j];
            replay_blend(s, st, j, r, [&](const int k, const unsigned long long live, const float alpha) {
                if (__builtin_amdgcn_inverse_ballot_w64(live)) {
                    const float T = s.T[k];
                    if (T == 1.0f) m0[k] = m;
                    const float d = m - m0[k], w = alpha * T, Ap = 1.0f - T;
                    float e;
                    if constexpr (POWER == 2) {
                        const float dd = d * d;
                        e = __builtin_fmaf(dd, Ap, __builtin_fmaf(-2.0f * d, M1[k], M2[k]));
                        M2[k] = __builtin_fmaf(dd, w, M2[k]);
                    } else {
                        e = __builtin_fmaf(d, Ap, -M1[k]);
                    }
                    D[k] = __builtin_fmaf(w, e, D[k]);
                    M1[k] = __builtin_fmaf(d, w, M1[k]);
                }
            });
        }
    });
#pragma unroll
    for (int k = 0; k < 4; ++k) {
        if (!s.inside[k]) continue;
        const size_t pid = (size_t)(s.py0 + 4 * k) * (size_t)p.frame.dims.width + (size_t)s.px;
        p.out[pid] = 2.0f * D[k];
        p.moments[pid] = m0[k];
        p.moments[plane + pid] = M1[k];
        p.moments[2 * plane + pid] = M2[k];
    }
}

template <int POWER, bool GEO>
__global__ __launch_bounds__(kWave) void distortion_backward_kernel(const DistortionParams p) {
    __shared__ BackStage st;
    __shared__ float s_value[kWave];
    const int lane = threadIdx.x;
    int tx, ty;
    const int tile = walk_tile(p.frame, &tx, &ty);
    if (tile < 0) return;
    const size_t plane = (size_t)p.frame.dims.width * (size_t)p.frame.dims.height;

    [[maybe_unused]] const bool files_value = sum8_of_lane(lane) == GeometrySums::kExtra;

    BackLanes s;
    float g[4] = {}, m0[4] = {}, M1n[4] = {};
    [[maybe_unused]] float M2n[4] = {};
    [[maybe_unused]] float An[4], Tf[4], Tb[4], Ms[4], S[4];
    float m = 0.0f, a_v = 0.0f;
    [[maybe_unused]] GeometrySums geo(lane);
    back_walk<true>(
        p.frame, tile, tx, ty, lane, s, st,
         [&](const int k, const size_t pid) {
            g[k] = p.dL_dout[pid];
            m0[k] = p.moments[pid];
            M1n[k] = p.moments[plane + pid];
            if constexpr (POWER == 2) M2n[k] = p.moments[2 * plane + pid];
        },
         [&]() {
#pragma unroll
            for (int k = 0; k < 4; ++k) {
                if constexpr (POWER == 2) An[k] = 1.0f - s.T[k];
                else { Tf[k] = s.T[k]; Tb[k] = s.T[k]; Ms[k] = 0.0f; }
                if constexpr (GEO) S[k] = 0.0f;
            }
        },
         [&](const uint32_t slot, const uint32_t id) { s_value[slot] = p.values[id]; },
         [&](const int j) {
            m = s_value[j];
            a_v = 0.0f;
            if constexpr (GEO) geo.clear();
        },
         [&](const int k, const BackPixel& px) {
            const float d = m - m0[k];
            float dv;
            [[maybe_unused]] float c = 0.0f;
            if constexpr (POWER == 2) {
                const float t = __builtin_fmaf(d, An[k], -M1n[k]);
                dv = 4.0f * t;
                if constexpr (GEO) c = 2.0f * __builtin_fmaf(d * d, An[k], __builtin_fmaf(-2.0f * d, M1n[k], M2n[k]));
            } else {
                const float As = Tb[k] - Tf[k], Ap = 1.0f - px.Tn;
                dv = 2.0f * (Ap - As);
                if constexpr (GEO) {
                    const float M1p = (M1n[k] - Ms[k]) - px.w * d;
                    c = 2.0f * ((__builtin_fmaf(d, Ap, -M1p) + Ms[k]) - d * As);
                    Ms[k] = __builtin_fmaf(px.w, d, Ms[k]);
                }
                Tb[k] = px.act ? px.Tn : Tb[k];
            }
            a_v = __builtin_fmaf(px.w * g[k], dv, a_v);
            if constexpr (GEO) {
                const float dL_dalpha = g[k] * __builtin_fmaf(px.Tn, c, -(S[k] * px.inv));
                S[k] = __builtin_fmaf(c, px.w, S[k]);
                geo.add(px, dL_dalpha);
            }
        },
         [&](const int j) {
            const size_t id = st.id[j];
            if constexpr (GEO) {
                const float total = geo.file(p.geometry_sums, id, lane, a_v);
                if (files_value && total != 0.0f) unsafeAtomicAdd(p.value_sums + id, (double)total);
            } else {
                const float total = wave_sum2(a_v, 0.0f);
                if (lane == 31 && total != 0.0f) unsafeAtomicAdd(p.value_sums + id, (double)total);
            }
        });
}

int distortion_check(gsr_distortion_args* a, bool backward, FrameDims* d, bool* nothing) {
    GSR_TRY(walk_pass_check(a, d, nothing));
    if (a->power != 1 && a->power != 2) return GSR_ERR_INVALID_ARG;
    if (!a->values || !a->moments) return GSR_ERR_INVALID_ARG;
    if (backward ? (!a->dL_dout || !a->dL_dvalues || !a->value_sums_f64) : !a->out) return GSR_ERR_INVALID_ARG;
    if (backward && (misaligned(a->value_sums_f64, 8) || misaligned(a->geometry_sums_f64, 8))) return GSR_ERR_INVALID_ARG;
    return GSR_OK;
}

DistortionParams distortion_params(const gsr_distortion_args* a, const WalkFrame& frame) {
    DistortionParams p;
    p.frame = frame;
    p.values = a->values;
    p.out = a->out;
    p.moments = a->moments;
    p.dL_dout = a->dL_dout;
    p.value_sums = a->value_sums_f64;
    p.geometry_sums = a->geometry_sums_f64;
    return p;
}

int distortion_forward_impl(gsr_distortion_args* a) {
    FrameDims d;
    bool nothing = false;
    GSR_TRY(distortion_check(a, false, &d, &nothing));
    return walk_pass_call(a, d, nothing, nullptr, [&](const WalkFrame& frame, unsigned blocks, hipStream_t stream) {
        const DistortionParams p = distortion_params(a, frame);
        const dim3 grid(blocks);
        if (a->power == 2) hipLaunchKernelGGL(distortion_forward_kernel<2>, grid, dim3(kWave), 0, stream, p);
        else hipLaunchKernelGGL(distortion_forward_kernel<1>, grid, dim3(kWave), 0, stream, p);
        GSR_LAUNCH_CHECK("distortion_forward_kernel");
        return GSR_OK;
    });
}

int distortion_backward_impl(gsr_distortion_args* a) {
    FrameDims d;
    bool nothing = false;
    GSR_TRY(distortion_check(a, true, &d, &nothing));
    const WalkSums sums = {(size_t)a->num_gaussians, a->value_sums_f64, a->dL_dvalues};
    return walk_pass_call(a, d, nothing, &sums, [&](const WalkFrame& frame, unsigned blocks, hipStream_t stream) {
        const DistortionParams p = distortion_params(a, frame);
        const bool square = a->power == 2, geo = a->geometry_sums_f64 != nullptr;
        const dim3 grid(blocks);
        if (square && geo) hipLaunchKernelGGL((distortion_backward_kernel<2, true>), grid, dim3(kWave), 0, stream, p);
        else if (square) hipLaunchKernelGGL((distortion_backward_kernel<2, false>), grid, dim3(kWave), 0, stream, p);
        else if (geo) hipLaunchKernelGGL((distortion_backward_kernel<1, true>), grid, dim3(kWave), 0, stream, p);
        else hipLaunchKernelGGL((distortion_backward_kernel<1, false>), grid, dim3(kWave), 0, stream, p);
        GSR_LAUNCH_CHECK("distortion_backward_kernel");
        return GSR_OK;
    });
}

}
}

extern "C" size_t gsr_distortion_temp_bytes(int32_t num_gaussians) {
    return num_gaussians <= 0 ? 0 : sizeof(double) * (size_t)num_gaussians;
}
extern "C" int gsr_distortion_forward(gsr_distortion_args* a) { return gsr::entry_point(gsr::distortion_forward_impl, a); }
extern "C" int gsr_distortion_backward(gsr_distortion_args* a) { return gsr::entry_point(gsr::distortion_backward_impl, a); }
```

### gsrast_amd/csrc/features.hip

```cpp
#include <hip/hip_runtime.h>

#include "list_walk.hpp"
#include "../../include/gsrast_amd_features.h"

namespace gsr {
namespace {

constexpr int kChunkNarrow = GSR_FEATURES_CHUNK_NARROW, kChunkWide = GSR_FEATURES_CHUNK;
static_assert(kChunkNarrow % 8 == 0 && kChunkNarrow >= 8 && kChunkWide % 8 == 0 && kChunkWide >= kChunkNarrow && kChunkWide <= 32,
              "the reduction packs eight sums per register");
inline int chunk_of(int channels) { return channels <= kChunkNarrow ? kChunkNarrow : kChunkWide; }

struct FeatureParams {
    WalkFrame frame;
    const float* features;
    const float* background;
    float* out;
    const float* dL_dout;
    double* feature_sums;
    double* geometry_sums;
    uint32_t channels;
};

template <int K>
__device__ __forceinline__ void stage_feature_row(float* slot, const float* row, uint32_t nc) {
#pragma unroll
    for (int c = 0; c < K; c += 4) {
        float4 v;
        v.x = (uint32_t)c < nc ? row[c] : 0.0f;
        v.y = (uint32_t)(c + 1) < nc ? row[c + 1] : 0.0f;
        v.z = (uint32_t)(c + 2) < nc ? row[c + 2] : 0.0f;
        v.w = (uint32_t)(c + 3) < nc ? row[c + 3] : 0.0f;
        *reinterpret_cast<float4*>(slot + c) = v;
    }
}
template <int K>
__device__ __forceinline__ void load_feature_row(float (&feat)[K], const float* slot) {
#pragma unroll
    for (int c = 0; c < K; c += 4) {
        const float4 v = *reinterpret_cast<const float4*>(slot + c);
        feat[c] = v.x; feat[c + 1] = v.y; feat[c + 2] = v.z; feat[c + 3] = v.w;
    }
}

template <int K>
struct FeatureStage : ReplayStage {
    float feat[kWave * K];
};

template <int K>
__global__ __launch_bounds__(kWave) void features_forward_kernel(const FeatureParams p) {
    __shared__ FeatureStage<K> st;
    const int lane = (int)threadIdx.x;
    int tx, ty;
    const int tile = walk_tile(p.frame, &tx, &ty);
    if (tile < 0) return;
    const uint32_t c0 = blockIdx.y * (uint32_t)K, nc = min((uint32_t)K, p.channels - c0);
    const size_t plane = (size_t)p.frame.dims.width * (size_t)p.frame.dims.height;

    TileLanes s;
    tile_lanes_init(s, tx, ty, lane, p.frame.dims.width, p.frame.dims.height, -1);
    float acc[4][K];
#pragma unroll
    for (int k = 0; k < 4; ++k)
#pragma unroll
        for (int c = 0; c < K; ++c) acc[k][c] = 0.0f;

    const bool has_list = replay_walk(p.frame, tile, tx, ty, lane, s, st, [&](const TileBox& box, const RecordBatch& b) {
        const uint32_t kept = stage_replay(box, st, b, p.frame.num_gaussians, [&](uint32_t slot, uint32_t id) {
            stage_feature_row<K>(&st.feat[slot * K], p.features + (size_t)id * (size_t)p.channels + c0, nc);
        });
        for (uint32_t j = 0; j < kept; ++j) {
            const ReplayRecord r = replay_candidates(s, st, j);
            if (!r.any()) continue;
            float feat[K];
            load_feature_row<K>(feat, &st.feat[j * K]);
            replay_blend(s, st, j, r, [&](const int k, const unsigned long long live, const float alpha) {
                if (__builtin_amdgcn_inverse_ballot_w64(live)) {
                    const float w = alpha * s.T[k];
#pragma unroll
                    for (int c = 0; c < K; ++c) acc[k][c] = __builtin_fmaf(feat[c], w, acc[k][c]);
                }
            });
        }
    });
#pragma unroll
    for (int k = 0; k < 4; ++k) {
        if (!s.inside[k]) continue;
        const size_t pid = (size_t)(s.py0 + 4 * k) * (size_t)p.frame.dims.width + (size_t)s.px;
        const float tf = has_list ? p.frame.final_t[pid] : 1.0f;
#pragma unroll
        for (int c = 0; c < K; ++c) {
            if ((uint32_t)c >= nc) continue;
            float* dst = p.out + (size_t)(c0 + (uint32_t)c) * plane + pid;
            if (p.background) *dst = acc[k][c] + tf * p.background[c0 + (uint32_t)c];
            else *dst = acc[k][c];
        }
    }
}

template <int K, bool GEO>
__global__ __launch_bounds__(kWave) void features_backward_kernel(const FeatureParams p) {
    __shared__ BackStage st;
    __shared__ __attribute__((aligned(16))) float s_feat[kWave * K];
    const int lane = threadIdx.x;
    int tx, ty;
    const int tile = walk_tile(p.frame, &tx, &ty);
    if (tile < 0) return;
    const size_t plane = (size_t)p.frame.dims.width * (size_t)p.frame.dims.height;
    const uint32_t c0 = blockIdx.y * (uint32_t)K, nc = min((uint32_t)K, p.channels - c0);

    const int my_feat = sum8_of_lane(lane);

    BackLanes s;
    float g[4][K] = {};
    [[maybe_unused]] float S[4];
    float a_f[K];
    [[maybe_unused]] float feat[K];
    [[maybe_unused]] GeometrySums geo(lane);
    back_walk<true>(
        p.frame, tile, tx, ty, lane, s, st,
         [&](const int k, const size_t pid) {
#pragma unroll
            for (int c = 0; c < K; ++c)
                if ((uint32_t)c < nc) g[k][c] = p.dL_dout[(size_t)(c0 + (uint32_t)c) * plane + pid];
        },
         [&]() {
            if constexpr (GEO) {
#pragma unroll
                for (int k = 0; k < 4; ++k) {
                    float bgg = 0.0f;
                    if (p.background) {
#pragma unroll
                        for (int c = 0; c < K; ++c)
                            if ((uint32_t)c < nc) bgg = __builtin_fmaf(p.background[c0 + (uint32_t)c], g[k][c], bgg);
                    }
                    S[k] = s.T[k] * bgg;
                }
            }
        },
         [&](const uint32_t slot, const uint32_t id) {
            if constexpr (GEO) stage_feature_row<K>(&s_feat[slot * K], p.features + (size_t)id * (size_t)p.channels + c0, nc);
        },
         [&](const int j) {
#pragma unroll
            for (int c = 0; c < K; ++c) a_f[c] = 0.0f;
            if constexpr (GEO) {
                load_feature_row<K>(feat, &s_feat[j * K]);
                geo.clear();
            }
        },
         [&](const int k, const BackPixel& px) {
#pragma unroll
            for (int c = 0; c < K; ++c) a_f[c] = __builtin_fmaf(px.w, g[k][c], a_f[c]);
            if constexpr (GEO) {
                float cg = feat[K - 1] * g[k][K - 1];
#pragma unroll
                for (int c = K - 2; c >= 0; --c) cg = __builtin_fmaf(feat[c], g[k][c], cg);
                const float dL_dalpha = __builtin_fmaf(px.Tn, cg, -(S[k] * px.inv));
                S[k] = __builtin_fmaf(cg, px.w, S[k]);
                geo.add(px, dL_dalpha);
            }
        },
         [&](const int j) {
            const size_t id = st.id[j];
#pragma unroll
            for (int c = 0; c < K; c += 8) {
                const float total = wave_sum8(a_f[c], a_f[c + 1], a_f[c + 2], a_f[c + 3], a_f[c + 4], a_f[c + 5], a_f[c + 6], a_f[c + 7], lane);
                if (my_feat >= 0 && (uint32_t)(c + my_feat) < nc && total != 0.0f)
                    unsafeAtomicAdd(p.feature_sums + id * (size_t)p.channels + c0 + (uint32_t)(c + my_feat), (double)total);
            }
            if constexpr (GEO) geo.file(p.geometry_sums, id, lane, 0.0f);
        });
}

int features_check(gsr_features_args* a, bool backward, FrameDims* d, bool* nothing) {
    GSR_TRY(walk_pass_check(a, d, nothing));
    if (a->channels < 1 || a->channels > GSR_FEATURES_MAX_CHANNELS) return GSR_ERR_INVALID_ARG;
    if (!a->features) return GSR_ERR_INVALID_ARG;
    if (backward ? (!a->dL_dout || !a->dL_dfeatures || !a->feature_sums_f64) : !a->out) return GSR_ERR_INVALID_ARG;
    if (backward && (misaligned(a->feature_sums_f64, 8) || misaligned(a->geometry_sums_f64, 8))) return GSR_ERR_INVALID_ARG;
    return GSR_OK;
}

FeatureParams feature_params(const gsr_features_args* a, const WalkFrame& frame) {
    FeatureParams p;
    p.frame = frame;
    p.features = a->features;
    p.background = a->background;
    p.out = a->out;
    p.dL_dout = a->dL_dout;
    p.feature_sums = a->feature_sums_f64;
    p.geometry_sums = a->geometry_sums_f64;
    p.channels = (uint32_t)a->channels;
    return p;
}

int features_forward_impl(gsr_features_args* a) {
    FrameDims d;
    bool nothing = false;
    GSR_TRY(features_check(a, false, &d, &nothing));
    return walk_pass_call(a, d, nothing, nullptr, [&](const WalkFrame& frame, unsigned blocks, hipStream_t stream) {
        const FeatureParams p = feature_params(a, frame);
        const int k = chunk_of(a->channels);
        const dim3 grid(blocks, (unsigned)((a->channels + k - 1) / k));
        if (k == kChunkNarrow) hipLaunchKernelGGL(features_forward_kernel<kChunkNarrow>, grid, dim3(kWave), 0, stream, p);
        else hipLaunchKernelGGL(features_forward_kernel<kChunkWide>, grid, dim3(kWave), 0, stream, p);
        GSR_LAUNCH_CHECK("features_forward_kernel");
        return GSR_OK;
    });
}

int features_backward_impl(gsr_features_args* a) {
    FrameDims d;
    bool nothing = false;
    GSR_TRY(features_check(a, true, &d, &nothing));
    const WalkSums sums = {(size_t)a->num_gaussians * (size_t)a->channels, a->feature_sums_f64, a->dL_dfeatures};
    return walk_pass_call(a, d, nothing, &sums, [&](const WalkFrame& frame, unsigned blocks, hipStream_t stream) {
        const FeatureParams p = feature_params(a, frame);
        const int k = chunk_of(a->channels);
        const bool narrow = k == kChunkNarrow, geo = a->geometry_sums_f64 != nullptr;
        const dim3 grid(blocks, (unsigned)((a->channels + k - 1) / k));
        if (narrow && geo) hipLaunchKernelGGL((features_backward_kernel<kChunkNarrow, true>), grid, dim3(kWave), 0, stream, p);
        else if (narrow) hipLaunchKernelGGL((features_backward_kernel<kChunkNarrow, false>), grid, dim3(kWave), 0, stream, p);
        else if (geo) hipLaunchKernelGGL((features_backward_kernel<kChunkWide, true>), grid, dim3(kWave), 0, stream, p);
        else hipLaunchKernelGGL((features_backward_kernel<kChunkWide, false>), grid, dim3(kWave), 0, stream, p);
        GSR_LAUNCH_CHECK("features_backward_kernel");
        return GSR_OK;
    });
}

}
}

extern "C" size_t gsr_features_temp_bytes(int32_t num_gaussians, int32_t channels) {
    if (num_gaussians <= 0 || channels < 1 || channels > GSR_FEATURES_MAX_CHANNELS) return 0;
    return sizeof(double) * (size_t)num_gaussians * (size_t)channels;
}
extern "C" int gsr_features_forward(gsr_features_args* a) { return gsr::entry_point(gsr::features_forward_impl, a); }
extern "C" int gsr_features_backward(gsr_features_args* a) { return gsr::entry_point(gsr::features_backward_impl, a); }
```

### gsrast_amd/csrc/list_walk.hpp

```cpp
#pragma once
#include <hip/hip_runtime.h>
#include <hip/amd_detail/amd_hip_unsafe_atomics.h>

#include "blend_core.hpp"
#include "blockbin.hpp"
#include "wave_reduce.hpp"

namespace gsr {

struct WalkFrame {
    const uint2* ranges;
    const uint32_t* point_list;
    const float2* means2D;
    const float4* conic_opacity;
    const uint32_t* n_contrib;
    const float* final_t;
    FrameDims dims;
    const uint32_t* tile_order;
    uint32_t num_gaussians;
    uint32_t num_rendered;
};

__device__ __forceinline__ int walk_tile(const WalkFrame& f, int* tx, int* ty) {
    const int rows = f.dims.row_end - f.dims.row_begin;
    const int tile_local = tile_of_workgroup(f.tile_order ? (int)f.tile_order[blockIdx.x] : (int)blockIdx.x, f.dims.grid_x, rows);
    if (tile_local < 0) return -1;
    const int tile = f.dims.row_begin * f.dims.grid_x + tile_local;
    *tx = tile % f.dims.grid_x;
    *ty = tile / f.dims.grid_x;
    return tile;
}
__device__ __forceinline__ bool walk_range(const WalkFrame& f, int tile, uint2* range) {
    *range = f.ranges[tile];
    return f.num_rendered != 0u && range->x < range->y && range->y <= f.num_rendered;
}

struct ReplayStage {
    float2 xy[kWave];
    float4 co[kWave];
    float4 raw[kWave];
    uint32_t number[kWave];
    unsigned long long exp_tab[32];
};

template <typename Payload>
__device__ __forceinline__ uint32_t stage_replay(const TileBox& box, ReplayStage& st, const RecordBatch& b, uint32_t num_gaussians, Payload payload) {
    const bool present = b.present() && b.id < num_gaussians;
    const uint32_t rank = b.rank(), pos = b.pos;
    const bool keep = present && !record_misses_tile(b.xy, b.co, box);
    const unsigned long long m2 = __ballot(keep);
    if (keep) {
        const uint32_t slot = __builtin_amdgcn_mbcnt_hi((uint32_t)(m2 >> 32), __builtin_amdgcn_mbcnt_lo((uint32_t)m2, 0u));
        const float dxm = fmaxf(fabsf(b.xy.x - box.x_lo), fabsf(b.xy.x - box.x_hi)), dym = fmaxf(fabsf(b.xy.y - box.y_lo), fabsf(b.xy.y - box.y_hi));
        const float terms = fabsf(b.co.x) * dxm * dxm + fabsf(b.co.z) * dym * dym + 2.0f * fabsf(b.co.y) * dxm * dym;
        const float p0 = -__logf(255.0f * b.co.w);
        const float floor2 = !(b.co.w > -__builtin_inff()) ? -__builtin_inff() : (b.co.w <= 0.0f ? __builtin_inff() : (p0 - 1e-3f - 1e-6f * terms) * kLog2e);
        const bool filtered = terms < 1.0e6f;
        st.xy[slot] = b.xy;
        st.co[slot] = filtered ? make_float4((-0.5f * kLog2e) * b.co.x, -kLog2e * b.co.y, (-0.5f * kLog2e) * b.co.z, floor2)
                               : make_float4(0.0f, 0.0f, 0.0f, -__builtin_inff());
        st.raw[slot] = b.co;
        st.number[slot] = pos + rank + 1u;
        payload(slot, b.id);
    }
    return (uint32_t)__popcll(m2);
}

struct ReplayRecord {
    float dx;
    f32x2 dy01, dy23;
    unsigned long long cand[4];
    __device__ __forceinline__ bool any() const { return (cand[0] | cand[1] | cand[2] | cand[3]) != 0ull; }
};
__device__ __forceinline__ ReplayRecord replay_candidates(const TileLanes& s, const ReplayStage& st, uint32_t j) {
    ReplayRecord r;
    const float2 xy = st.xy[j];
    const float4 q = st.co[j];
    const uint32_t number = st.number[j];
    r.dx = xy.x - s.fx;
    const float h0 = (q.x * r.dx) * r.dx;
    const float g = q.y * r.dx;
    f32x2 gy; gy.x = xy.y; gy.y = xy.y;
    f32x2 gg; gg.x = g; gg.y = g;
    f32x2 hh; hh.x = h0; hh.y = h0;
    f32x2 cz; cz.x = q.z; cz.y = q.z;
    r.dy01 = gy - s.fy01; r.dy23 = gy - s.fy23;
    const f32x2 fw01 = __builtin_elementwise_fma(r.dy01, __builtin_elementwise_fma(cz, r.dy01, gg), hh);
    const f32x2 fw23 = __builtin_elementwise_fma(r.dy23, __builtin_elementwise_fma(cz, r.dy23, gg), hh);
    const float filter[4] = {fw01.x, fw01.y, fw23.x, fw23.y};
#pragma unroll
    for (int k = 0; k < 4; ++k)
        r.cand[k] = __ballot(filter[k] <= kFilterSlack * kLog2e) & __ballot(filter[k] >= q.w) & __ballot(number <= s.last[k]);
    return r;
}

template <typename OnLive>
__device__ __forceinline__ void replay_blend(TileLanes& s, const ReplayStage& st, uint32_t j, const ReplayRecord& r, OnLive on_live) {
    constexpr float kAlphaMin = 1.0f / 255.0f;
    const float4 raw = st.raw[j];
    const float t1 = (raw.x * r.dx) * r.dx, bdx = raw.y * r.dx;
#pragma unroll
    for (int pair = 0; pair < 2; ++pair) {
        if ((r.cand[2 * pair] | r.cand[2 * pair + 1]) == 0ull) continue;
        const f32x2 dy = pair == 0 ? r.dy01 : r.dy23;
        const f32x2 pw = -0.5f * (t1 + (raw.z * dy) * dy) - bdx * dy;
        const float e0 = exp_ref(pw.x, st.exp_tab), e1 = exp_ref(pw.y, st.exp_tab);
#pragma unroll
        for (int h = 0; h < 2; ++h) {
            const int k = 2 * pair + h;
            if (r.cand[k] == 0ull) continue;
            const float power = h == 0 ? pw.x : pw.y;
            const float alpha = fminf(0.99f, raw.w * (h == 0 ? e0 : e1));
            const unsigned long long live = r.cand[k] & ~__ballot(power > 0.0f) & ~__ballot(alpha < kAlphaMin);
            if (live == 0ull) continue;
            on_live(k, live, alpha);
            if (__builtin_amdgcn_inverse_ballot_w64(live)) s.T[k] = s.T[k] * (1.0f - alpha);
        }
    }
}

template <typename OnBatch>
__device__ __forceinline__ bool replay_walk(const WalkFrame& f, int tile, int tx, int ty, int lane, TileLanes& s, ReplayStage& st, OnBatch on_batch) {
    uint2 range;
    if (!walk_range(f, tile, &range)) return false;
    uint32_t mine = 0u;
#pragma unroll
    for (int k = 0; k < 4; ++k) {
        if (s.inside[k]) s.last[k] = f.n_contrib[(size_t)(s.py0 + 4 * k) * (size_t)f.dims.width + (size_t)s.px];
        mine = mine > s.last[k] ? mine : s.last[k];
    }
    const uint32_t walk = min(range.y - range.x, wave_max_u32(mine));
    if (walk == 0u) return true;
    exp_table_init(st.exp_tab, lane);
    const TileBox box = tile_box(tx, ty, f.dims.width, f.dims.height);
    auto next_batch = [&](uint32_t pos) {
        RecordBatch nb;
        nb.valid = pos < walk;
        if (nb.valid) {
            const uint32_t cnt = min((uint32_t)kWave, walk - pos);
            nb.mask = cnt == kWave ? ~0ull : ((1ull << cnt) - 1ull);
            nb.pos = pos;
            if ((uint32_t)lane < cnt) nb.id = f.point_list[range.x + pos + (uint32_t)lane];
        }
        return nb;
    };
    auto fetch = [&](RecordBatch& b) {
        b.xy = make_float2(0.0f, 0.0f);
        b.co = make_float4(0.0f, 0.0f, 0.0f, 0.0f);
        if (b.valid && b.present() && b.id < f.num_gaussians) { b.xy = f.means2D[b.id]; b.co = f.conic_opacity[b.id]; }
    };
    RecordBatch b0 = next_batch(0);
    fetch(b0);
    RecordBatch b1 = next_batch(kWave);
    for (uint32_t pos = 2 * kWave; b0.valid; pos += kWave) {
        fetch(b1);
        RecordBatch b2 = next_batch(pos);
        on_batch(box, b0);
        b0 = b1;
        b1 = b2;
    }
    return true;
}

struct BackLanes {
    int px, py0;
    float fx, fy[4];
    uint32_t last[4];
    float T[4];
};
struct BackStage {
    float4 co[kWave];
    float2 xy[kWave];
    uint32_t id[kWave];
    uint32_t pos[kWave];
    float floor[kWave];
    unsigned long long exp_tab[32];
};
struct BackPixel {
    unsigned long long act_mask;
    bool act;
    float dx, dy;
    float4 co;
    float G, raw;
    float inv, Tn;
    float w;
    __device__ __forceinline__ bool live() const { return __builtin_amdgcn_inverse_ballot_w64(act_mask & ~__ballot(raw > 0.99f)); }
    __device__ __forceinline__ float ux() const { return __builtin_fmaf(co.x, dx, co.y * dy); }
    __device__ __forceinline__ float uy() const { return __builtin_fmaf(co.y, dx, co.z * dy); }
};

__device__ __forceinline__ int sum8_of_lane(int lane) {
    constexpr int kSumOfRow[8] = {0, 4, 2, 6, 1, 5, 3, 7};
    return (lane & 7) == 0 ? kSumOfRow[lane >> 3] : -1;
}

struct GeometrySums {
    static constexpr uint32_t kFloats = 12;
    float mx, my, A, B, C, op, m00, m01, m11;
    __device__ __forceinline__ void clear() { mx = my = A = B = C = op = m00 = m01 = m11 = 0.0f; }
    __device__ __forceinline__ void add(const BackPixel& px, const float dL_dalpha) {
        const float dx = px.dx, dy = px.dy;
        const bool live = px.live();
        const float gop = live ? px.G * dL_dalpha : 0.0f;
        const float dpow = live ? px.raw * dL_dalpha : 0.0f;
        op += gop;
        A = __builtin_fmaf(-0.5f * dx * dx, dpow, A);
        B = __builtin_fmaf(-(dx * dy), dpow, B);
        C = __builtin_fmaf(-0.5f * dy * dy, dpow, C);
        const float ux = px.ux(), uy = px.uy();
        mx = __builtin_fmaf(-ux, dpow, mx);
        my = __builtin_fmaf(-uy, dpow, my);
        const float hux = 0.5f * dpow * ux, huy = 0.5f * dpow * uy;
        m00 = __builtin_fmaf(hux, ux, m00); m01 = __builtin_fmaf(hux, uy, m01); m11 = __builtin_fmaf(huy, uy, m11);
    }
    static constexpr int kExtra = 6;
    int slot;
    __device__ __forceinline__ explicit GeometrySums(const int lane) {
        constexpr int kSumOfRow4[4] = {9, 11, 10, 12};
        const int of8 = sum8_of_lane(lane);
        slot = (lane & 7) == 0 ? (of8 < kExtra ? of8 : -1) : ((lane & 15) == 4 && kSumOfRow4[lane >> 4] < 12 ? kSumOfRow4[lane >> 4] : -1);
    }
    __device__ __forceinline__ float file(double* geometry_sums, const size_t id, const int lane, const float extra) const {
        const float t8 = wave_sum8(mx, my, A, B, C, op, extra, 0.0f, lane);
        const float t4 = wave_sum4(m00, m01, m11, 0.0f);
        const float total = (lane & 7) == 4 ? t4 : t8;
        if (slot >= 0 && total != 0.0f) unsafeAtomicAdd(geometry_sums + kFloats * id + (uint32_t)slot, (double)total);
        return t8;
    }
};

template <bool LIST_FIRST, typename Seed, typename Start, typename Payload, typename Begin, typename OnPixel, typename File>
__device__ __forceinline__ void back_walk(const WalkFrame& f, int tile, int tx, int ty, int lane, BackLanes& s, BackStage& st, Seed seed,
                                          Start start, Payload payload, Begin begin, OnPixel on_pixel, File file) {
    exp_table_init(st.exp_tab, lane);
    uint2 range;
    const bool has_list = walk_range(f, tile, &range);
    if (LIST_FIRST && !has_list) return;
    s.px = tx * kTile + (lane & 15); s.py0 = ty * kTile + (lane >> 4);
    s.fx = (float)s.px;
    uint32_t hi = 0;
#pragma unroll
    for (int k = 0; k < 4; ++k) {
        const int py = s.py0 + 4 * k;
        s.fy[k] = (float)py;
        const bool inside = s.px < f.dims.width && py < f.dims.height;
        s.last[k] = 0; s.T[k] = 1.0f;
        if (inside) {
            const size_t pid = (size_t)py * (size_t)f.dims.width + (size_t)s.px;
            s.last[k] = f.n_contrib[pid];
            s.T[k] = f.final_t[pid];
            seed(k, pid);
        }
        hi = max(hi, s.last[k]);
    }
    if (!has_list) return;
    hi = min(wave_max_u32(hi), range.y - range.x);
    if (hi == 0) return;
    start();
    const TileBox box = tile_box(tx, ty, f.dims.width, f.dims.height);

    auto walk_batch = [&](const bool present, const uint32_t id, const uint32_t idx_l, const float2 xy_l, const float4 co_l) {
        const bool keep = present && !record_misses_tile(xy_l, co_l, box);
        const unsigned long long kept_mask = __ballot(keep);
        if (keep) {
            const uint32_t slot = __builtin_amdgcn_mbcnt_hi((uint32_t)(kept_mask >> 32), __builtin_amdgcn_mbcnt_lo((uint32_t)kept_mask, 0u));
            st.id[slot] = id;
            st.pos[slot] = idx_l;
            st.xy[slot] = xy_l;
            st.co[slot] = co_l;
            payload(slot, id);
            const float op = co_l.w;
            st.floor[slot] = !(op > -__builtin_inff()) ? -__builtin_inff() : (op <= 0.0f ? __builtin_inff() : -__logf(255.0f * op) - 1e-3f);
        }
        for (int j = (int)__popcll(kept_mask) - 1; j >= 0; --j) {
            const uint32_t idx0 = st.pos[j];
            const float2 xy = st.xy[j];
            BackPixel px;
            px.co = st.co[j];
            px.dx = xy.x - s.fx;
            const float4 co = px.co;
            const float dx = px.dx, flo = st.floor[j];
            begin(j);
            bool any = false;
#pragma unroll
            for (int k = 0; k < 4; ++k) {
                const unsigned long long inlist = __ballot(idx0 < s.last[k]);
                if (inlist == 0ull) continue;
                const float dy = xy.y - s.fy[k];
                const float power = -0.5f * (co.x * dx * dx + co.z * dy * dy) - co.y * dx * dy;
                const unsigned long long cand = inlist & ~__ballot(power > 0.0f) & __ballot(power >= flo);
                if (cand == 0ull) continue;
                px.G = exp_ref(power, st.exp_tab);
                px.raw = co.w * px.G;
                const float alpha = fminf(0.99f, px.raw);
                px.act_mask = cand & ~__ballot(alpha < 1.0f / 255.0f);
                if (px.act_mask == 0ull) continue;
                px.act = __builtin_amdgcn_inverse_ballot_w64(px.act_mask);
                any = true;
                px.dy = dy;
                px.inv = __builtin_amdgcn_rcpf(1.0f - alpha);
                px.Tn = s.T[k] * px.inv;
                s.T[k] = px.act ? px.Tn : s.T[k];
                px.w = px.act ? alpha * px.Tn : 0.0f;
                on_pixel(k, px);
            }
            if (any) file(j);
        }
    };

    struct Batch {
        bool valid = false, present = false;
        uint32_t id = 0, idx_l = 0;
        float2 xy = {0.0f, 0.0f};
        float4 co = {0.0f, 0.0f, 0.0f, 0.0f};
    };
    int it_c = (int)((hi - 1) / kWave);
    auto next_batch = [&]() {
        Batch nb;
        if (it_c < 0) return nb;
        const uint32_t first = (uint32_t)it_c * kWave;
        --it_c;
        nb.valid = true;
        nb.idx_l = first + (uint32_t)lane;
        nb.present = (uint32_t)lane < min((uint32_t)kWave, hi - first);
        nb.id = f.point_list[range.x + (nb.present ? nb.idx_l : 0u)];
        nb.present = nb.present && nb.id < f.num_gaussians;
        return nb;
    };
    auto fetch = [&](Batch& nb) {
        const uint32_t at = (nb.valid && nb.present) ? nb.id : 0u;
        nb.xy = f.means2D[at];
        nb.co = f.conic_opacity[at];
    };
    Batch b0 = next_batch();
    fetch(b0);
    Batch b1 = next_batch();
    while (b0.valid) {
        fetch(b1);
        Batch b2 = next_batch();
        walk_batch(b0.present, b0.id, b0.idx_l, b0.xy, b0.co);
        b0 = b1;
        b1 = b2;
    }
}

inline int walk_check(const gsr_forward_receipt& r, int n, int width, int height, int row_begin, int row_end, bool band_as_is,
                      const void* point_list, FrameDims* d, bool* nothing) {
    if (r.magic != GSR_RECEIPT_MAGIC) return GSR_ERR_INVALID_ARG;
    if (tile_band(width, height, row_begin, row_end, d) != GSR_OK) return GSR_ERR_INVALID_ARG;
    if (band_as_is) { d->row_begin = row_begin; d->row_end = row_end; }
    BlockFeed block_lists;
    bool from_blocks = false, lists_written = true;
    GSR_TRY(lists_of_receipt(r, n, width, height, d->row_begin, d->row_end, point_list, &block_lists, &from_blocks, &lists_written));
    *nothing = r.num_rendered == 0 || d->row_begin == d->row_end;
    if (!*nothing && (!lists_written || !point_list)) return GSR_ERR_INVALID_ARG;
    return GSR_OK;
}

inline WalkFrame walk_frame(const uint32_t* ranges, const uint32_t* point_list, const float* means2D, const float* conic_opacity,
                            const uint32_t* n_contrib, const float* final_t, const FrameDims& d, int num_gaussians, uint32_t num_rendered) {
    WalkFrame f;
    f.ranges = reinterpret_cast<const uint2*>(ranges);
    f.point_list = point_list;
    f.means2D = reinterpret_cast<const float2*>(means2D);
    f.conic_opacity = reinterpret_cast<const float4*>(conic_opacity);
    f.n_contrib = n_contrib;
    f.final_t = final_t;
    f.dims = d;
    f.tile_order = nullptr;
    f.num_gaussians = (uint32_t)num_gaussians;
    f.num_rendered = num_rendered;
    return f;
}

template <typename Args>
inline int walk_pass_check(Args* a, FrameDims* d, bool* nothing) {
    if (!a || a->struct_size != sizeof(Args)) return GSR_ERR_INVALID_ARG;
    a->stage_ms = 0.0f;
    if (a->num_gaussians <= 0 || a->width <= 0 || a->height <= 0) return GSR_ERR_INVALID_ARG;
    if (!a->means2D || !a->conic_opacity || !a->ranges || !a->n_contrib || !a->final_t) return GSR_ERR_INVALID_ARG;
    if (misaligned(a->means2D, 8) || misaligned(a->conic_opacity, 16) || misaligned(a->ranges, 8)) return GSR_ERR_INVALID_ARG;
    return walk_check(a->receipt, a->num_gaussians, a->width, a->height, a->tile_row_begin, a->tile_row_end, false, a->point_list, d, nothing);
}
template <typename Args>
inline WalkFrame walk_frame(const Args* a, const FrameDims& d) {
    return walk_frame(a->ranges, a->point_list, a->means2D, a->conic_opacity, a->n_contrib, a->final_t, d, a->num_gaussians,
                      a->receipt.num_rendered);
}

struct StageTimer {
    CallEvents<2> events;
    bool on = false;
    int begin(bool profile, hipStream_t stream) {
        on = profile;
        if (!on) return GSR_OK;
        GSR_TRY(events.create());
        GSR_HIP_TRY(hipEventRecord(events.ev[0], stream));
        return GSR_OK;
    }
    int end(hipStream_t stream, float* ms) {
        if (!on) return GSR_OK;
        GSR_HIP_TRY(hipEventRecord(events.ev[1], stream));
        GSR_HIP_TRY(hipEventSynchronize(events.ev[1]));
        GSR_HIP_TRY(hipEventElapsedTime(ms, events.ev[0], events.ev[1]));
        return GSR_OK;
    }
};

inline long long finish_sums_workgroups(size_t count) { return (long long)((count + 255) / 256); }
namespace {
template <int V>
__global__ __launch_bounds__(256) void finish_sums_kernel(size_t count, double* __restrict__ sums, float* __restrict__ out) {
    static_assert(V == 1 || V == 2, "one float or a float2 per thread");
    const size_t i = (size_t)blockIdx.x * 256 + threadIdx.x;
    if (i >= count) return;
    double v[V];
#pragma unroll
    for (int e = 0; e < V; ++e) v[e] = sums[V * i + e];
    if constexpr (V == 2) *reinterpret_cast<float2*>(out + 2 * i) = make_float2((float)v[0], (float)v[1]);
    else out[i] = (float)v[0];
#pragma unroll
    for (int e = 0; e < V; ++e)
        if (v[e] != 0.0) sums[V * i + e] = 0.0;
}
template <int V>
inline int launch_finish_sums(size_t count, double* sums, float* out, hipStream_t stream) {
    hipLaunchKernelGGL(finish_sums_kernel<V>, dim3((unsigned)finish_sums_workgroups(count)), dim3(256), 0, stream, count, sums, out);
    GSR_LAUNCH_CHECK("finish_sums_kernel");
    return GSR_OK;
}

struct WalkSums {
    size_t count;
    double* sums;
    float* out;
};
template <typename Args, typename Launch>
inline int walk_pass_call(Args* a, const FrameDims& d, bool nothing, const WalkSums* backward, Launch launch) {
    const long long blocks = patch_workgroups(d.grid_x, d.row_end - d.row_begin);
    if (exceeds_grid(blocks) || (backward && exceeds_grid(finish_sums_workgroups(backward->count)))) return GSR_ERR_TOO_LARGE;
    hipStream_t stream = static_cast<hipStream_t>(a->stream);
    StageTimer timer;
    GSR_TRY(timer.begin((a->flags & GSR_FLAG_PROFILE) != 0, stream));
    if (backward ? !nothing : d.row_begin != d.row_end) {
        WalkFrame frame = walk_frame(a, d);
        if (backward) frame.tile_order = tile_order_of_call(a->receipt, d.row_begin, d.row_end);
        GSR_TRY(launch(frame, (unsigned)blocks, stream));
    }
    if (backward) GSR_TRY(launch_finish_sums<1>(backward->count, backward->sums, backward->out, stream));
    return timer.end(stream, &a->stage_ms);
}
}

}
```

### gsrast_amd/rasterizer.py

```python
from __future__ import annotations

import ctypes as C

import numpy as np
import torch

from . import _capi, backward_plan
from .backward_plan import DEPTHS, INTO, ROW_FLOATS, SET
from .camera import Camera


class ChunkBuffer:

    def __init__(self, device: torch.device):
        self.device = device
        self.tensor: torch.Tensor | None = None
        self.capacity = 0
        self.calls: list[int] = []
        self._cb = _capi.ALLOC_FN(self._alloc)

    def _alloc(self, _user, nbytes):
        self.calls.append(int(nbytes))
        try:
            if nbytes > self.capacity:
                self.tensor = None
                self.tensor = torch.empty(2 * int(nbytes), dtype=torch.uint8, device=self.device)
                self.capacity = 2 * int(nbytes)
            return self.tensor.data_ptr()
        except Exception:
            return None

    @property
    def callback(self):
        return self._cb

    def base(self) -> int:
        return 0 if self.tensor is None else self.tensor.data_ptr()

    def view(self, ptr: int, count: int, dtype: torch.dtype) -> torch.Tensor:
        off = ptr - self.base()
        nbytes = count * torch.empty((), dtype=dtype).element_size()
        assert 0 <= off and off + nbytes <= self.capacity, "state pointer outside its chunk"
        return self.tensor[off:off + nbytes].view(dtype)


def _dev(a, device, dtype=torch.float32) -> torch.Tensor:
    if isinstance(a, torch.Tensor):
        return a.to(device=device, dtype=dtype).contiguous()
    return torch.from_numpy(np.ascontiguousarray(a)).to(device=device, dtype=dtype).contiguous()


class BackwardBuffers:

    def __init__(self, device: torch.device):
        self.device, self.n = device, 0
        self.sets: dict[str, dict[str, torch.Tensor]] = {}
        self.scratch: dict[str, torch.Tensor] = {}

    def fit(self, n: int) -> None:
        if n != self.n:
            self.n = n
            self.sets.clear()
            self.scratch.clear()

    def get(self, name: str, *shape, dtype=torch.float32) -> torch.Tensor:
        if name not in self.scratch:
            self.scratch[name] = torch.empty(shape, dtype=dtype, device=self.device)
        return self.scratch[name]

    def sums(self, name: str, *shape) -> torch.Tensor:
        t = self.scratch.get(name)
        if t is None or t.numel() < int(np.prod(shape)):
            t = self.scratch[name] = torch.zeros(shape, dtype=torch.float64, device=self.device)
        return t

    def take(self, plan: backward_plan.BackwardPlan, semantics: str, with_cov3D: bool, into: "dict | None") -> dict:
        own = None
        if plan.takes_output_set:
            own = self.sets.get(semantics)
            if own is None or ("dL_dcov3D" in own) != with_cov3D:
                own = self.sets[semantics] = {k: (torch.zeros if k == "dL_dshs" else torch.empty)(
                    (self.n, ROW_FLOATS[k]), dtype=torch.float32, device=self.device) for k in backward_plan.output_set(with_cov3D)}
        return {k: into[k] if source == INTO else own[k] if source == SET else
                self.get(k, *((self.n,) if k == DEPTHS else (self.n, ROW_FLOATS[k]))) for k, source in plan.sources.items()}


_PLAN_USED_FLAGS = (("last_blend_from_lists", _capi.GSR_PLAN_BLEND_FROM_LISTS),
                    ("last_tiles_reordered", _capi.GSR_PLAN_TILES_REORDERED),
                    ("last_tile_order_dropped", _capi.GSR_PLAN_TILE_ORDER_DROPPED),
                    ("last_emit_overlapped", _capi.GSR_PLAN_EMIT_OVERLAPPED),
                    ("last_colors_beside", _capi.GSR_PLAN_COLORS_BESIDE),
                    ("last_deep_tiles", _capi.GSR_PLAN_DEEP_TILES))


class SplatRasterizer:

    def __init__(self, width: int, height: int, device="cuda:0", background=(0.0, 0.0, 0.0)):
        self.lib = _capi.lib()
        if not torch.cuda.is_available():
            raise RuntimeError("SplatRasterizer needs a HIP device (no CPU fallback exists)")
        self.device = torch.device(device)
        self.width, self.height = int(width), int(height)
        self.geom = ChunkBuffer(self.device)
        self.binning = ChunkBuffer(self.device)
        self.image = ChunkBuffer(self.device)
        self.background = _dev(np.asarray(background, np.float32), self.device)
        self.out_color = torch.zeros((3, self.height, self.width), dtype=torch.float32, device=self.device)
        self.out_depth: torch.Tensor | None = None
        self.last_depth: "bool | str" = False
        self.num_gaussians = 0
        self.use_rects = True
        self.last_num_rendered = 0
        self.last_records_staged = 0
        self.last_plan = "none"
        for name, _ in _PLAN_USED_FLAGS:
            setattr(self, name, False)
        self.last_lists_written = True
        self.last_receipt: _capi.ForwardReceipt | None = None
        self.last_stage_ms: dict[str, float] = {}
        self.last_backward_ms: tuple = ()
        self.last_camera_ms: "float | None" = None
        self.last_absgrad_ms: "float | None" = None
        self.last_features_ms: "float | None" = None
        self.last_distortion_ms: "float | None" = None
        self.last_median_ms: "float | None" = None
        self._distortion_moments: "tuple[int | None, int, torch.Tensor | None]" = (None, 0, None)
        self.rects: torch.Tensor | None = None
        self._bw = BackwardBuffers(self.device)
        self._colors_of_call: "tuple[int | None, torch.Tensor | None]" = (None, None)
        self._means3: torch.Tensor | None = None
        self._cam_dev = torch.zeros(35, dtype=torch.float32, device=self.device)
        self._cam_host = torch.zeros(35, dtype=torch.float32).pin_memory()
        self._view, self._proj, self._cam_pos = self._cam_dev[0:16], self._cam_dev[16:32], self._cam_dev[32:35]
        self._last_cam = None
        self._state_epoch = 0
        self._history = C.c_void_p()
        _capi.call("gsr_tile_history_create", C.byref(self._history), device=self.device)

    _history = None

    def __del__(self):
        h, self._history = self._history, None
        if h is not None and h.value:
            try:
                torch.cuda.synchronize(self.device)
                self.lib.gsr_tile_history_destroy(h)
            except Exception:
                pass

    def configure_from_scene(self, scene: dict, use_rects: bool = True) -> None:
        self.means3D = _dev(scene["means3D"], self.device)
        self.scales = _dev(scene["scales"], self.device)
        self.rotations = _dev(scene["rotations"], self.device)
        self.opacities = _dev(scene["opacities"], self.device)
        self.shs = _dev(scene["shs"], self.device)
        self.num_gaussians = int(self.means3D.shape[0])
        assert self.means3D.shape == (self.num_gaussians, 4) and self.scales.shape == (self.num_gaussians, 4)
        assert self.rotations.shape == (self.num_gaussians, 4) and self.shs.shape == (self.num_gaussians, 48)
        self.use_rects = use_rects
        self._colors_dc, self._colors_key = None, None
        self.rects = (torch.zeros((self.num_gaussians, 2), dtype=torch.int32, device=self.device)
                      if use_rects else None)
        self._state_epoch += 1

    def bind_scene(self, means3D: torch.Tensor, scales: torch.Tensor, rotations: torch.Tensor, opacities: torch.Tensor,
                   shs: torch.Tensor, use_rects: "bool | None" = None) -> None:
        n = int(means3D.shape[0])
        for name, t, shape in (("means3D", means3D, (n, 4)), ("scales", scales, (n, 4)), ("rotations", rotations, (n, 4)),
                               ("opacities", opacities, (n,)), ("shs", shs, (n, 48))):
            assert isinstance(t, torch.Tensor) and t.dtype == torch.float32 and t.device == self.device, name
            assert tuple(t.shape) == shape and t.is_contiguous(), (name, tuple(t.shape), shape)
        self.means3D, self.scales, self.rotations, self.opacities, self.shs = means3D, scales, rotations, opacities, shs
        if use_rects is None:
            use_rects = self.use_rects
        if not use_rects:
            self.rects = None
        elif self.rects is None or self.rects.shape[0] != n:
            self.rects = torch.zeros((n, 2), dtype=torch.int32, device=self.device)
        self.use_rects = use_rects
        self.num_gaussians = n
        self._colors_dc, self._colors_key = None, None
        self._state_epoch += 1

    def set_camera(self, cam: Camera) -> None:
        assert cam.width == self.width and cam.height == self.height
        if cam is self._last_cam:
            return
        h = self._cam_host.numpy()
        h[0:16] = np.asarray(cam.view, np.float32).reshape(16)
        h[16:32] = np.asarray(cam.proj, np.float32).reshape(16)
        h[32:35] = np.asarray(cam.cam_pos, np.float32).reshape(3)
        self._cam_dev.copy_(self._cam_host, non_blocking=True)
        self._tan = (float(cam.tan_fovx), float(cam.tan_fovy))
        self._last_cam = cam
        self._state_epoch += 1

    def set_camera_device(self, view: torch.Tensor, proj: torch.Tensor, cam_pos: torch.Tensor, tan_fovx: float,
                          tan_fovy: float) -> None:
        with torch.no_grad():
            for dst, src, k in ((self._view, view, 16), (self._proj, proj, 16), (self._cam_pos, cam_pos, 3)):
                assert isinstance(src, torch.Tensor) and src.device == self.device and src.numel() == k, (src.shape, k)
                dst.copy_(src.detach().reshape(k))
        self._tan = (float(tan_fovx), float(tan_fovy))
        self._last_cam = None
        self._state_epoch += 1

    def _forward_args(self, means3D: torch.Tensor, out_color: torch.Tensor) -> _capi.ForwardArgs:
        a = _capi.ForwardArgs()
        a.struct_size = C.sizeof(_capi.ForwardArgs)
        a.geometry_alloc, a.binning_alloc, a.image_alloc = self.geom.callback, self.binning.callback, self.image.callback
        a.num_gaussians, a.sh_dims, a.M = self.num_gaussians, 3, 16
        a.background = self.background.data_ptr()
        a.width, a.height = self.width, self.height
        a.means3D, a.shs = means3D.data_ptr(), self.shs.data_ptr()
        a.view_matrix, a.proj_matrix, a.cam_pos = self._view.data_ptr(), self._proj.data_ptr(), self._cam_pos.data_ptr()
        a.tan_fovx, a.tan_fovy = self._tan
        a.out_color = out_color.data_ptr()
        a.stream = _capi.stream(self.device)
        return a

    def draw(self, cam: Camera | None = None, *, profile: bool = False, count_staged: bool = False,
             tile_rows: tuple[int, int] | None = None, scale_modifier: float = 1.0,
             sync: bool = True, semantics: str = "gscuda", sh_degree: int = 3, plan: str = "auto",
             overlap_emit: "bool | None" = None, sorted_lists: bool = True, colors_precomp: "bool | torch.Tensor" = False,
             tile_history: "bool | str" = True, deep_tiles: "bool | str | None" = None,
             depth: "bool | str" = False, into: "dict | None" = None) -> torch.Tensor:
        if cam is not None:
            self.set_camera(cam)
        self._state_epoch += 1
        out_color, out_depth = self.out_color, None
        if into is not None:
            assert set(into) <= {"out_color", "out_depth"}, sorted(into)
            for k, shape in (("out_color", (3, self.height, self.width)), ("out_depth", (self.height, self.width))):
                self._check_into(into.get(k), shape, k)
            out_color = into.get("out_color", out_color)
            out_depth = into.get("out_depth")
        a = self._forward_args(self.means3D, out_color)
        inria = semantics == "inria"
        assert semantics in ("gscuda", "inria")
        a.flags = ((_capi.GSR_FLAG_PROFILE if profile else 0) | (_capi.GSR_FLAG_COUNT_STAGED if count_staged else 0)
                   | (_capi.GSR_FLAG_SEMANTICS_INRIA if inria else 0)
                   | {"auto": 0, "sort": _capi.GSR_FLAG_PLAN_SORT, "blocks": _capi.GSR_FLAG_PLAN_BLOCKS}[plan]
                   | (_capi.GSR_FLAG_OVERLAP_EMIT if overlap_emit else (_capi.GSR_FLAG_SERIAL_EMIT if overlap_emit is False else 0))
                   | (0 if sorted_lists else _capi.GSR_FLAG_NO_SORTED_LISTS)
                   | (0 if tile_history else _capi.GSR_FLAG_NO_TILE_HISTORY)
                   | {"all": _capi.GSR_FLAG_DEEP_TILES_ALL, "all8": _capi.GSR_FLAG_DEEP_WAVES_8, "all16": _capi.GSR_FLAG_DEEP_WAVES_16,
                      False: _capi.GSR_FLAG_NO_DEEP_TILES, None: 0}[deep_tiles]
                   | (_capi.GSR_FLAG_DEPTH_INVERSE if depth == "inverse" else 0))
        assert depth in (False, True, "inverse"), depth
        if inria:
            a.sh_dims = sh_degree
        if isinstance(colors_precomp, torch.Tensor):
            assert colors_precomp.shape == (self.num_gaussians, 3) and colors_precomp.dtype == torch.float32
            assert colors_precomp.device == self.device and colors_precomp.is_contiguous()
            colors_used = colors_precomp
        else:
            assert not (colors_precomp and inria), "upstream colour depends on the view direction"
            colors_used = self.precomputed_colors() if colors_precomp else None
        a.colors_precomp = colors_used.data_ptr() if colors_used is not None else None
        a.opacities, a.scales = self.opacities.data_ptr(), self.scales.data_ptr()
        a.scale_modifier = scale_modifier
        a.rotations = self.rotations.data_ptr()
        a.rects = self.rects.data_ptr() if (self.rects is not None and not inria) else None
        a.tile_history = self._history if tile_history is True else None
        if depth:
            if out_depth is None:
                if self.out_depth is None:
                    self.out_depth = torch.zeros((self.height, self.width), dtype=torch.float32, device=self.device)
                out_depth = self.out_depth
            a.out_depth = out_depth.data_ptr()
        if tile_rows is not None:
            a.tile_row_begin, a.tile_row_end = int(tile_rows[0]), int(tile_rows[1])
        _capi.call("gsr_forward", C.byref(a), device=self.device)
        self.last_receipt = a.receipt.copy()
        self.last_colors_precomp = colors_used is not None
        self.last_depth = depth
        self._colors_of_call = (int(a.receipt.serial), colors_used)
        self.last_num_rendered = int(a.num_rendered)
        self.last_records_staged = int(a.records_staged)
        self.last_plan = _capi.PLAN_NAMES[int(a.plan_used) & 0xFF]
        self.last_lists_written = not (int(a.plan_used) & _capi.GSR_PLAN_LISTS_SKIPPED)
        for name, bit in _PLAN_USED_FLAGS:
            setattr(self, name, bool(int(a.plan_used) & bit))
        self.last_stage_ms = {n: float(a.stage_ms[i]) for i, n in enumerate(_capi.STAGE_NAMES)} if profile else {}
        if sync:
            torch.cuda.current_stream(self.device).synchronize()
            self.poll_async_error()
        return out_color

    def opacity_map(self) -> torch.Tensor:
        return 1.0 - self.map_image_state()["finalT"]

    def tile_history_stats(self) -> dict:
        out = (C.c_uint32 * 6)()
        _capi.call("gsr_tile_history_stats", self._history, out)
        return {"mean_ticks": int(out[0]), "longest_ticks": int(out[1]), "similarity": int(out[2]) / 1000.0,
                "order_dropped": bool(out[3]), "calls": int(out[4]), "overlapped": bool(out[5])}

    def tile_history_times(self):
        tiles = ((self.width + 15) // 16) * ((self.height + 15) // 16)
        out, deep = (C.c_uint32 * tiles)(), C.c_uint32(0)
        _capi.call("gsr_tile_history_times", self._history, out, tiles, C.byref(deep))
        raw = np.frombuffer(out, dtype=np.uint32).copy()
        return raw & 0x7FFFFFFF, (raw >> 31).astype(bool), int(deep.value)

    def precomputed_colors(self) -> torch.Tensor:
        key = (self.shs.data_ptr(), self.shs._version)
        if self._colors_dc is None or self._colors_key != key:
            c = torch.empty((self.num_gaussians, 3), dtype=torch.float32, device=self.device)
            _capi.call("gsr_colors_from_dc", self.num_gaussians, self.shs.data_ptr(), c.data_ptr(), _capi.stream(self.device),
                       device=self.device)
            self._colors_dc, self._colors_key = c, key
        return self._colors_dc

    def poll_async_error(self, receipt: "_capi.ForwardReceipt | None" = None) -> None:
        r = receipt if receipt is not None else self.last_receipt
        _capi.call("gsr_poll_async_error", C.byref(r), where="gsr_forward (device side)")

    def draw_points(self, cam: Camera | None = None, sync: bool = True) -> torch.Tensor:
        if cam is not None:
            self.set_camera(cam)
        self._state_epoch += 1
        if self._means3 is None or self._means3.shape[0] != self.num_gaussians:
            self._means3 = self.means3D[:, :3].contiguous()
        a = self._forward_args(self._means3, self.out_color)
        _capi.call("gsr_forward_points", C.byref(a), device=self.device)
        if sync:
            torch.cuda.current_stream(self.device).synchronize()
        return self.out_color

    def map_points_image_state(self) -> dict:
        st = _capi.PointsImageState()
        P = self.width * self.height
        self.lib.gsr_points_image_from_chunk(self.image.base(), P, C.byref(st))
        v = self.image.view
        return {"depth": v(st.depth, P, torch.float32).view(self.height, self.width),
                "outColor": v(st.out_color, 3 * P, torch.float32).view(3, self.height, self.width)}

    def _map_frame(self, a, num_rendered: int) -> _capi.GeometryState:
        gst, ist, bst = _capi.GeometryState(), _capi.ImageState(), _capi.BinningState()
        self.lib.gsr_geometry_from_chunk(self.geom.base(), self.num_gaussians, C.byref(gst))
        self.lib.gsr_image_from_chunk(self.image.base(), self.width * self.height, C.byref(ist))
        self.lib.gsr_binning_from_chunk(self.binning.base(), num_rendered, C.byref(bst))
        frame = {"means2D": gst.means2D, "conic_opacity": gst.conic_opacity, "ranges": ist.ranges, "n_contrib": ist.n_contrib,
                 "final_t": ist.accum_alpha, "point_list": bst.values}
        for k, _ in a._fields_:
            if k in frame:
                setattr(a, k, frame[k])
        return gst

    def _walk_args(self, kind, rcpt: _capi.ForwardReceipt, tile_rows: "tuple[int, int] | None", profile: bool):
        a = kind()
        a.struct_size = C.sizeof(kind)
        a.flags = _capi.GSR_FLAG_PROFILE if profile else 0
        a.num_gaussians, a.width, a.height = self.num_gaussians, self.width, self.height
        self._map_frame(a, int(rcpt.num_rendered))
        a.receipt = rcpt
        if tile_rows is None:
            tile_rows = (int(rcpt.tile_row_begin), int(rcpt.tile_row_end))
        a.tile_row_begin, a.tile_row_end = int(tile_rows[0]), int(tile_rows[1])
        a.stream = _capi.stream(self.device)
        return a

    def _check_into(self, t: "torch.Tensor | None", shape: tuple, what=None) -> None:
        if t is None:
            return
        assert t.dtype == torch.float32 and t.device == self.device and t.is_contiguous(), what
        assert tuple(t.shape) == tuple(shape), (what, tuple(t.shape))

    def _new_output(self, rcpt: _capi.ForwardReceipt, tile_rows: "tuple[int, int] | None", shape: tuple) -> torch.Tensor:
        whole = tile_rows is None and (int(rcpt.tile_row_begin), int(rcpt.tile_row_end)) == (0, (self.height + 15) // 16)
        return (torch.empty if whole else torch.zeros)(shape, dtype=torch.float32, device=self.device)

    def _call(self, fn: str, a, *, drop: tuple = (), ms: "str | None" = None, sync: bool = False) -> None:
        try:
            _capi.call(fn, C.byref(a), device=self.device)
        except _capi.GsrError:
            for name in drop:
                self._bw.scratch.pop(name, None)
            raise
        if ms is not None:
            setattr(self, ms, float(a.stage_ms) if a.flags & _capi.GSR_FLAG_PROFILE else None)
        if sync:
            torch.cuda.current_stream(self.device).synchronize()

    def _check_dL_dalpha(self, dL_dalpha: "torch.Tensor | None") -> None:
        if dL_dalpha is not None:
            assert isinstance(dL_dalpha, torch.Tensor) and dL_dalpha.dtype == torch.float32, "dL_dalpha: a float32 tensor"
            assert dL_dalpha.device == self.device, ("dL_dalpha", dL_dalpha.device, self.device)
            assert tuple(dL_dalpha.shape) == (self.height, self.width), ("dL_dalpha", tuple(dL_dalpha.shape))

    def _depth_gradient(self, dL_ddepth: "torch.Tensor | None", depth: "bool | str | None"):
        if dL_ddepth is None:
            return None, None
        gd = dL_ddepth.to(device=self.device, dtype=torch.float32).contiguous()
        assert gd.shape == (self.height, self.width)
        return gd, backward_plan.depth_mode(depth, self.last_depth)

    def _backward_args(self, rcpt: "_capi.ForwardReceipt | None", col: "torch.Tensor | None", semantics: str,
                       sh_degree: int) -> _capi.BackwardArgs:
        a = _capi.BackwardArgs()
        a.struct_size = C.sizeof(_capi.BackwardArgs)
        gst = self._map_frame(a, int(rcpt.num_rendered) if rcpt is not None else self.last_num_rendered)
        if semantics == "inria":
            a.flags = _capi.GSR_FLAG_SEMANTICS_INRIA
            a.cam_pos, a.shs, a.clamped, a.sh_dims = self._cam_pos.data_ptr(), self.shs.data_ptr(), gst.clamped, int(sh_degree)
        a.num_gaussians, a.width, a.height = self.num_gaussians, self.width, self.height
        a.background = self.background.data_ptr()
        a.cov3D, a.radii = gst.cov3D, gst.internal_radii
        a.colors = col.data_ptr() if col is not None else gst.rgb
        a.means3D, a.view_matrix = self.means3D.data_ptr(), self._view.data_ptr()
        a.tan_fovx, a.tan_fovy = self._tan
        a.stream = _capi.stream(self.device)
        if rcpt is not None:
            a.receipt = rcpt
        return a

    def backward(self, dL_dout: torch.Tensor, *, profile: bool = False, with_cov3D: bool = True,
                 tile_rows: tuple[int, int] | None = None, scale_modifier: float = 1.0, semantics: str = "gscuda",
                 sh_degree: int = 3, receipt: "_capi.ForwardReceipt | None | bool" = None, wide_sums: bool = True,
                 outputs: "tuple[str, ...] | None" = None, dL_ddepth: "torch.Tensor | None" = None,
                 depth: "bool | str | None" = None, camera: bool = False, into: "dict | None" = None,
                 sync: bool = True, dL_dalpha: "torch.Tensor | None" = None, features: "tuple | None" = None,
                 distortion: "tuple | None" = None) -> dict:
        n, dev = self.num_gaussians, self.device
        rcpt = self.last_receipt if receipt is None else (None if receipt is False else receipt)
        if distortion is not None:
            assert wide_sums, "distortion= needs wide_sums: the distortion term reaches the chain through the sums_f64 scratch"
            assert rcpt is not None, "distortion= needs the receipt of a draw()"
            assert isinstance(distortion, (tuple, list)) and len(distortion) in (2, 3, 4), "distortion=(values, dL_ddistortion_map[, power[, moments]])"
            distortion_power = int(distortion[2]) if len(distortion) > 2 else 2
            assert distortion_power in (1, 2), ("power", distortion_power)
            distortion_moments = self._distortion_moments_of(rcpt, distortion_power, distortion[3] if len(distortion) > 3 else None)
        if features is not None:
            assert wide_sums, "features= needs wide_sums: the feature term reaches the chain through the sums_f64 scratch"
            assert rcpt is not None, "features= needs the receipt of a draw()"
            assert isinstance(features, (tuple, list)) and len(features) in (2, 3), "features=(F, dL_dfeature_map[, background])"
        col = self._colors_of(rcpt)
        plan = backward_plan.plan_backward(semantics, with_cov3D, wide_sums, None if outputs is None else tuple(outputs),
                                           None if into is None else tuple(into), dL_ddepth is not None, camera, col is not None)
        self._check_dL_dalpha(dL_dalpha)
        g = dL_dout.to(device=dev, dtype=torch.float32).contiguous()
        assert g.shape == (3, self.height, self.width)
        for k, t in (into or {}).items():
            if k != "camera":
                self._check_into(t, (n, ROW_FLOATS[k]), k)
        gd, mode = self._depth_gradient(dL_ddepth, depth)
        self._bw.fit(n)
        arrays = self._bw.take(plan, semantics, with_cov3D, into)
        a = self._backward_args(rcpt, col, semantics, sh_degree)
        a.flags |= (_capi.GSR_FLAG_PROFILE if profile else 0) | (_capi.GSR_FLAG_DEPTH_INVERSE if mode == "inverse" else 0)
        a.dL_dout_color = g.data_ptr()
        if dL_ddepth is not None:
            a.dL_dout_depth = gd.data_ptr()
        for k, t in arrays.items():
            setattr(a, k, t.data_ptr())
        if wide_sums:
            a.sums_f64 = self._bw.sums("sums_f64", n, 12).data_ptr()
            if dL_ddepth is not None:
                a.depth_sums_f64 = self._bw.sums("depth_sums_f64", n).data_ptr()
        if plan.chain_inputs:
            a.proj_matrix, a.scales, a.rotations = self._proj.data_ptr(), self.scales.data_ptr(), self.rotations.data_ptr()
            a.scale_modifier = scale_modifier
        if tile_rows is not None:
            a.tile_row_begin, a.tile_row_end = int(tile_rows[0]), int(tile_rows[1])
        feature_call = None
        if features is not None:
            feature_call, feature_keep = self._features_call(rcpt, features[0], features[2] if len(features) > 2 else None,
                                                             dL_dout=features[1], tile_rows=tile_rows, profile=profile)
        distortion_call = None
        if distortion is not None:
            distortion_call, distortion_keep = self._distortion_call(rcpt, distortion[0], distortion_power, distortion_moments,
                                                                     dL_dout=distortion[1], tile_rows=tile_rows, profile=profile)
        try:
            if feature_call is not None:
                feature_call.geometry_sums_f64 = a.sums_f64
                _capi.call("gsr_features_backward", C.byref(feature_call), device=dev)
            if distortion_call is not None:
                distortion_call.geometry_sums_f64 = a.sums_f64
                _capi.call("gsr_distortion_backward", C.byref(distortion_call), device=dev)
            if dL_dalpha is None:
                _capi.call("gsr_backward", C.byref(a), device=dev)
            else:
                ga = dL_dalpha.contiguous()
                _capi.call("gsr_backward_alpha", C.byref(a), ga.data_ptr(), device=dev)
        except _capi.GsrError:
            if wide_sums:
                self._bw.scratch.pop("sums_f64", None)
                self._bw.scratch.pop("depth_sums_f64", None)
            self._bw.scratch.pop("feature_sums_f64", None)
            self._bw.scratch.pop("distortion_sums_f64", None)
            raise
        self.last_backward_ms = (float(a.stage_ms[0]), float(a.stage_ms[1])) if profile else ()
        if feature_call is not None:
            self.last_features_ms = float(feature_call.stage_ms) if profile else None
            arrays["dL_dfeatures"] = feature_keep[-1]
        if distortion_call is not None:
            self.last_distortion_ms = float(distortion_call.stage_ms) if profile else None
            arrays["dL_dvalues"] = distortion_keep[-1]
        if camera:
            arrays.update(self.camera_backward({k: arrays[k] for k in plan.camera_inputs}, semantics=semantics,
                                               sh_degree=sh_degree, shs_colour="dL_dcolors" in plan.camera_inputs, depth=mode,
                                               profile=profile, sync=False, into=into["camera"] if plan.camera_into else None))
        if sync:
            torch.cuda.current_stream(dev).synchronize()
        return {k: arrays[k] for k in tuple(plan.result) + (("dL_dfeatures",) if feature_call is not None else ())
                + (("dL_dvalues",) if distortion_call is not None else ())}

    def _features_call(self, rcpt: _capi.ForwardReceipt, features: torch.Tensor, background, *, out: "torch.Tensor | None" = None,
                       dL_dout: "torch.Tensor | None" = None, into: "torch.Tensor | None" = None,
                       tile_rows: "tuple[int, int] | None" = None, profile: bool = False):
        n, dev = self.num_gaussians, self.device
        assert isinstance(features, torch.Tensor) and features.dtype == torch.float32 and features.device == dev, "features: a float32 tensor on this device"
        assert features.dim() == 2 and features.shape[0] == n, ("features", tuple(features.shape), n)
        c = int(features.shape[1])
        f = features.detach().contiguous()
        keep = [f]
        a = self._walk_args(_capi.FeaturesArgs, rcpt, tile_rows, profile)
        a.channels, a.features = c, f.data_ptr()
        if background is not None:
            bg = _dev(background, dev).reshape(-1)
            assert bg.numel() == c, ("background", tuple(bg.shape), c)
            keep.append(bg)
            a.background = bg.data_ptr()
        if out is not None:
            a.out = out.data_ptr()
            keep.append(out)
        if dL_dout is not None:
            g = dL_dout.to(device=dev, dtype=torch.float32).contiguous()
            assert tuple(g.shape) == (c, self.height, self.width), ("dL_dfeature_map", tuple(g.shape))
            self._check_into(into, (n, c))
            res = into if into is not None else torch.empty((n, c), dtype=torch.float32, device=dev)
            self._bw.fit(n)
            a.dL_dout, a.dL_dfeatures = g.data_ptr(), res.data_ptr()
            a.feature_sums_f64 = self._bw.sums("feature_sums_f64", n * c).data_ptr()
            keep += [g, res]
        return a, keep

    def render_features(self, features: torch.Tensor, *, background=None, receipt: "_capi.ForwardReceipt | None" = None,
                        tile_rows: "tuple[int, int] | None" = None, into: "torch.Tensor | None" = None, profile: bool = False,
                        sync: bool = True) -> torch.Tensor:
        rcpt = self.last_receipt if receipt is None else receipt
        assert rcpt is not None, "render_features needs the receipt of a draw()"
        assert isinstance(features, torch.Tensor) and features.dim() == 2, "features: [N,C]"
        shape = (int(features.shape[1]), self.height, self.width)
        self._check_into(into, shape)
        out = into if into is not None else self._new_output(rcpt, tile_rows, shape)
        a, _keep = self._features_call(rcpt, features, background, out=out, tile_rows=tile_rows, profile=profile)
        self._call("gsr_features_forward", a, ms="last_features_ms", sync=sync)
        return out

    def features_backward(self, features: torch.Tensor, dL_dout: torch.Tensor, *, background=None,
                          receipt: "_capi.ForwardReceipt | None" = None, tile_rows: "tuple[int, int] | None" = None,
                          into: "torch.Tensor | None" = None, profile: bool = False, sync: bool = True) -> torch.Tensor:
        rcpt = self.last_receipt if receipt is None else receipt
        assert rcpt is not None, "features_backward needs the receipt of a draw()"
        a, keep = self._features_call(rcpt, features, background, dL_dout=dL_dout, into=into, tile_rows=tile_rows, profile=profile)
        self._call("gsr_features_backward", a, drop=("feature_sums_f64",), ms="last_features_ms", sync=sync)
        return keep[-1]

    def _distortion_moments_of(self, rcpt: _capi.ForwardReceipt, power: int, moments: "torch.Tensor | None") -> torch.Tensor:
        if moments is None:
            serial, kept_power, kept = self._distortion_moments
            assert kept is not None and serial == int(rcpt.serial) and kept_power == power, (
                "distortion: the moments kept by this rasterizer are stale — they are those of render_distortion for another "
                "frame or power (or there are none): call render_distortion(values, power=...) for this draw() first")
            moments = kept
        self._check_into(moments, (3, self.height, self.width), "moments")
        return moments

    def _distortion_call(self, rcpt: _capi.ForwardReceipt, values: torch.Tensor, power: int, moments: torch.Tensor, *,
                         out: "torch.Tensor | None" = None, dL_dout: "torch.Tensor | None" = None,
                         into: "torch.Tensor | None" = None, tile_rows: "tuple[int, int] | None" = None, profile: bool = False):
        n, dev = self.num_gaussians, self.device
        assert isinstance(values, torch.Tensor) and values.dtype == torch.float32 and values.device == dev, "values: a float32 tensor on this device"
        assert values.dim() == 1 and values.shape[0] == n, ("values", tuple(values.shape), n)
        v = values.detach().contiguous()
        keep = [v, moments]
        a = self._walk_args(_capi.DistortionArgs, rcpt, tile_rows, profile)
        a.power, a.values, a.moments = int(power), v.data_ptr(), moments.data_ptr()
        if out is not None:
            a.out = out.data_ptr()
            keep.append(out)
        if dL_dout is not None:
            g = dL_dout.to(device=dev, dtype=torch.float32).contiguous()
            assert tuple(g.shape) == (self.height, self.width), ("dL_ddistortion_map", tuple(g.shape))
            self._check_into(into, (n,))
            res = into if into is not None else torch.empty((n,), dtype=torch.float32, device=dev)
            self._bw.fit(n)
            a.dL_dout, a.dL_dvalues = g.data_ptr(), res.data_ptr()
            a.value_sums_f64 = self._bw.sums("distortion_sums_f64", n).data_ptr()
            keep += [g, res]
        return a, keep

    def render_distortion(self, values: torch.Tensor, *, power: int = 2, receipt: "_capi.ForwardReceipt | None" = None,
                          tile_rows: "tuple[int, int] | None" = None, into: "torch.Tensor | None" = None, profile: bool = False,
                          sync: bool = True) -> torch.Tensor:
        rcpt = self.last_receipt if receipt is None else receipt
        assert rcpt is not None, "render_distortion needs the receipt of a draw()"
        assert power in (1, 2), ("power", power)
        shape = (self.height, self.width)
        self._check_into(into, shape)
        out = into if into is not None else self._new_output(rcpt, tile_rows, shape)
        moments = self._new_output(rcpt, tile_rows, (3,) + shape)
        a, _keep = self._distortion_call(rcpt, values, power, moments, out=out, tile_rows=tile_rows, profile=profile)
        self._distortion_moments = (None, 0, None)
        self._call("gsr_distortion_forward", a, ms="last_distortion_ms")
        self._distortion_moments = (int(rcpt.serial), int(power), moments)
        if sync:
            torch.cuda.current_stream(self.device).synchronize()
        return out

    def distortion_backward(self, values: torch.Tensor, dL_dmap: torch.Tensor, *, power: int = 2,
                            receipt: "_capi.ForwardReceipt | None" = None, tile_rows: "tuple[int, int] | None" = None,
                            into: "torch.Tensor | None" = None, moments: "torch.Tensor | None" = None, profile: bool = False,
                            sync: bool = True) -> torch.Tensor:
        rcpt = self.last_receipt if receipt is None else receipt
        assert rcpt is not None, "distortion_backward needs the receipt of a draw()"
        assert power in (1, 2), ("power", power)
        a, keep = self._distortion_call(rcpt, values, power, self._distortion_moments_of(rcpt, power, moments), dL_dout=dL_dmap,
                                        into=into, tile_rows=tile_rows, profile=profile)
        self._call("gsr_distortion_backward", a, drop=("distortion_sums_f64",), ms="last_distortion_ms", sync=sync)
        return keep[-1]

    def render_median(self, values: "torch.Tensor | None" = None, *, threshold: float = 0.5, ids: bool = True, dominant: bool = False,
                      receipt: "_capi.ForwardReceipt | None" = None, tile_rows: "tuple[int, int] | None" = None,
                      out: "dict | None" = None, profile: bool = False, sync: bool = True) -> dict:
        rcpt = self.last_receipt if receipt is None else receipt
        assert rcpt is not None, "render_median needs the receipt of a draw()"
        dev, shape = self.device, (self.height, self.width)
        want = (("map",) if values is not None else ()) + (("ids",) if ids else ()) + (("dominant_ids",) if dominant else ())
        assert want, "render_median: nothing asked for (values, ids or dominant)"
        out = dict(out or {})
        assert set(out) <= set(want), ("out", sorted(out), want)
        res = {}
        for k in want:
            dtype = torch.float32 if k == "map" else torch.int32
            t = out.get(k)
            if t is None:
                t = (torch.zeros(shape, dtype=dtype, device=dev) if k == "map" else torch.full(shape, -1, dtype=dtype, device=dev))
            assert t.dtype == dtype and t.device == dev and t.is_contiguous() and tuple(t.shape) == shape, (k, t.dtype, tuple(t.shape))
            res[k] = t
        a = self._walk_args(_capi.MedianArgs, rcpt, tile_rows, profile)
        a.threshold = float(threshold)
        keep = None
        if values is not None:
            assert isinstance(values, torch.Tensor) and values.dtype == torch.float32 and values.device == dev, "values: a float32 tensor on this device"
            assert values.dim() == 1 and values.shape[0] == self.num_gaussians, ("values", tuple(values.shape), self.num_gaussians)
            keep = values.detach().contiguous()
            a.values, a.out = keep.data_ptr(), res["map"].data_ptr()
        if ids:
            a.ids = res["ids"].data_ptr()
        if dominant:
            a.dominant_ids = res["dominant_ids"].data_ptr()
        self._call("gsr_median_forward", a, ms="last_median_ms", sync=sync)
        return res

    def median_backward(self, ids: torch.Tensor, dL_dmap: torch.Tensor, *, tile_rows: "tuple[int, int] | None" = None,
                        into: "torch.Tensor | None" = None, profile: bool = False, sync: bool = True) -> torch.Tensor:
        n, dev = self.num_gaussians, self.device
        assert isinstance(ids, torch.Tensor) and ids.dtype == torch.int32 and ids.device == dev and ids.is_contiguous(), "ids: the int32 map of render_median"
        assert tuple(ids.shape) == (self.height, self.width), ("ids", tuple(ids.shape))
        g = dL_dmap.to(device=dev, dtype=torch.float32).contiguous()
        assert tuple(g.shape) == (self.height, self.width), ("dL_dmap", tuple(g.shape))
        self._check_into(into, (n,))
        res = into if into is not None else torch.empty((n,), dtype=torch.float32, device=dev)
        self._bw.fit(n)
        a = _capi.MedianArgs()
        a.struct_size = C.sizeof(_capi.MedianArgs)
        a.flags = _capi.GSR_FLAG_PROFILE if profile else 0
        a.num_gaussians, a.width, a.height = n, self.width, self.height
        a.ids, a.dL_dout, a.dL_dvalues = ids.data_ptr(), g.data_ptr(), res.data_ptr()
        a.value_sums_f64 = self._bw.sums("median_sums_f64", n).data_ptr()
        if tile_rows is not None:
            a.tile_row_begin, a.tile_row_end = int(tile_rows[0]), int(tile_rows[1])
        a.stream = _capi.stream(dev)
        self._call("gsr_median_backward", a, drop=("median_sums_f64",), ms="last_median_ms", sync=sync)
        return res

    def pick(self, x: int, y: int, *, threshold: float = 0.5, dominant: bool = False) -> "int | None":
        x, y = int(x), int(y)
        assert 0 <= x < self.width and 0 <= y < self.height, ("pick", x, y)
        rcpt = self.last_receipt
        assert rcpt is not None, "pick needs a draw()"
        row = y // 16
        if not (int(rcpt.tile_row_begin) <= row < int(rcpt.tile_row_end)):
            return None
        res = self.render_median(threshold=threshold, ids=not dominant, dominant=dominant, tile_rows=(row, row + 1), sync=False)
        i = int(res["dominant_ids" if dominant else "ids"][y, x])
        return None if i < 0 else i

    def absgrad(self, dL_dout: torch.Tensor, *, dL_ddepth: "torch.Tensor | None" = None, depth: "bool | str | None" = None,
                dL_dalpha: "torch.Tensor | None" = None, receipt: "_capi.ForwardReceipt | None" = None, semantics: str = "gscuda",
                tile_rows: "tuple[int, int] | None" = None, into: "torch.Tensor | None" = None, sync: bool = True,
                profile: bool = False) -> torch.Tensor:
        n, dev = self.num_gaussians, self.device
        rcpt = self.last_receipt if receipt is None else receipt
        assert rcpt is not None, "absgrad needs the receipt of a draw()"
        assert semantics in ("gscuda", "inria"), semantics
        self._check_dL_dalpha(dL_dalpha)
        g = dL_dout.to(device=dev, dtype=torch.float32).contiguous()
        assert g.shape == (3, self.height, self.width)
        self._check_into(into, (n, 2))
        gd, mode = self._depth_gradient(dL_ddepth, depth)
        self._bw.fit(n)
        b = self._backward_args(rcpt, self._colors_of(rcpt), semantics, 3)
        b.dL_dout_color = g.data_ptr()
        if dL_ddepth is not None:
            b.dL_dout_depth = gd.data_ptr()
        if tile_rows is not None:
            b.tile_row_begin, b.tile_row_end = int(tile_rows[0]), int(tile_rows[1])
        out = into if into is not None else torch.empty((n, 2), dtype=torch.float32, device=dev)
        a = _capi.AbsgradArgs()
        a.struct_size = C.sizeof(_capi.AbsgradArgs)
        a.flags = (_capi.GSR_FLAG_PROFILE if profile else 0) | (_capi.GSR_FLAG_DEPTH_INVERSE if mode == "inverse" else 0)
        a.backward = C.pointer(b)
        ga = dL_dalpha.contiguous() if dL_dalpha is not None else None
        a.dL_dout_alpha = ga.data_ptr() if ga is not None else None
        a.abs_dL_dmean2D = out.data_ptr()
        a.sums_f64 = self._bw.sums("absgrad_sums_f64", n, 2).data_ptr()
        self._call("gsr_absgrad", a, drop=("absgrad_sums_f64",), ms="last_absgrad_ms", sync=sync)
        return out

    def _colors_of(self, rcpt: "_capi.ForwardReceipt | None") -> "torch.Tensor | None":
        serial, col = self._colors_of_call
        return col if rcpt is None or int(rcpt.serial) == serial else None

    def camera_backward(self, grads: dict, *, semantics: str = "gscuda", sh_degree: int = 3, depth: "bool | str | None" = None,
                        shs_colour: "bool | None" = None, receipt: "_capi.ForwardReceipt | None" = None,
                        profile: bool = False, sync: bool = True, into: "torch.Tensor | None" = None) -> dict:
        assert semantics in ("gscuda", "inria") and depth in (None, False, True, "inverse"), (semantics, depth)
        n, dev = self.num_gaussians, self.device
        inria = semantics == "inria"
        if shs_colour is None:
            shs_colour = inria and self._colors_of(self.last_receipt if receipt is None else receipt) is None
        gst = _capi.GeometryState()
        self.lib.gsr_geometry_from_chunk(self.geom.base(), n, C.byref(gst))
        self._bw.fit(n)
        scratch = self._bw.get("camera_scratch", int(self.lib.gsr_camera_backward_scratch_bytes(n)), dtype=torch.uint8)
        g = self._bw.get("camera_grad", 35)

        def ptr(k):
            t = grads[k]
            assert t.dtype == torch.float32 and t.is_contiguous() and t.device == dev and t.shape[0] == n, k
            return t.data_ptr()
        a = _capi.CameraBackwardArgs()
        a.struct_size = C.sizeof(_capi.CameraBackwardArgs)
        a.flags = ((_capi.GSR_FLAG_PROFILE if profile else 0) | (_capi.GSR_FLAG_SEMANTICS_INRIA if inria else 0)
                   | (_capi.GSR_FLAG_DEPTH_INVERSE if depth == "inverse" else 0))
        a.num_gaussians, a.width, a.height = n, self.width, self.height
        a.means3D, a.view_matrix, a.proj_matrix = self.means3D.data_ptr(), self._view.data_ptr(), self._proj.data_ptr()
        a.cam_pos = self._cam_pos.data_ptr()
        a.tan_fovx, a.tan_fovy = self._tan
        a.cov3D, a.radii = gst.cov3D, gst.internal_radii
        if shs_colour:
            a.shs, a.clamped, a.sh_dims = self.shs.data_ptr(), gst.clamped, int(sh_degree)
            a.dL_dcolors = ptr("dL_dcolors")
        a.dL_dmean2D, a.dL_dcov2D = ptr("dL_dmean2D"), ptr("dL_dcov2D")
        if depth:
            a.dL_ddepths = ptr("dL_ddepths")
        if into is not None:
            self._check_into(into, (35,))
            g = into
        a.dL_dview_matrix, a.dL_dproj_matrix, a.dL_dcam_pos = g[0:16].data_ptr(), g[16:32].data_ptr(), g[32:35].data_ptr()
        a.scratch = scratch.data_ptr()
        a.stream = _capi.stream(dev)
        self._call("gsr_camera_backward", a, ms="last_camera_ms", sync=sync)
        return {"dL_dview_matrix": g[0:16], "dL_dproj_matrix": g[16:32], "dL_dcam_pos": g[32:35]}

    def map_geometry_state(self) -> dict:
        st = _capi.GeometryState()
        self.lib.gsr_geometry_from_chunk(self.geom.base(), self.num_gaussians, C.byref(st))
        n, v = self.num_gaussians, self.geom.view
        return {
            "tilesTouched": v(st.tiles_touched, n, torch.int32),
            "depths": v(st.depths, n, torch.float32),
            "radii": v(st.internal_radii, n, torch.int32),
            "means2D": v(st.means2D, 2 * n, torch.float32).view(n, 2),
            "cov3D": v(st.cov3D, 6 * n, torch.float32).view(n, 6),
            "conicOpacity": v(st.conic_opacity, 4 * n, torch.float32).view(n, 4),
            "rgb": v(st.rgb, 3 * n, torch.float32).view(n, 3),
            "pointOffsets": v(st.point_offsets, n, torch.int32),
            "clamped": v(st.clamped, 3 * n, torch.uint8).view(torch.bool).view(n, 3),
        }

    def map_image_state(self) -> dict:
        st = _capi.ImageState()
        P = self.width * self.height
        self.lib.gsr_image_from_chunk(self.image.base(), P, C.byref(st))
        T = ((self.width + 15) // 16) * ((self.height + 15) // 16)
        v = self.image.view
        return {
            "ranges": v(st.ranges, 2 * T, torch.int32).view(T, 2),
            "nContrib": v(st.n_contrib, P, torch.int32).view(self.height, self.width),
            "finalT": v(st.accum_alpha, P, torch.float32).view(self.height, self.width),
        }

    def map_binning_state(self) -> dict:
        st = _capi.BinningState()
        R = self.last_num_rendered
        self.lib.gsr_binning_from_chunk(self.binning.base(), R, C.byref(st))
        v = self.binning.view
        return {
            "keys_unsorted": v(st.keys_unsorted, R, torch.int64),
            "keys": v(st.keys, R, torch.int64),
            "values_unsorted": v(st.values_unsorted, R, torch.int32),
            "values": v(st.values, R, torch.int32),
        }


def inclusive_scan_u32(x: torch.Tensor) -> torch.Tensor:
    assert x.dtype == torch.int32 and x.is_cuda and x.is_contiguous()
    out = torch.empty_like(x)
    temp = torch.empty(max(int(_capi.lib().gsr_scan_temp_bytes(x.numel())), 128), dtype=torch.uint8, device=x.device)
    _capi.call("gsr_inclusive_scan_u32", x.data_ptr(), out.data_ptr(), x.numel(), temp.data_ptr(), _capi.stream(x.device), device=x.device)
    torch.cuda.current_stream(x.device).synchronize()
    return out


def sort_pairs(keys: torch.Tensor, values: torch.Tensor, end_bit: int = 64, begin_bit: int = 0, sync: bool = True,
               out=None, temp=None):
    assert keys.dtype == torch.int64 and values.dtype == torch.int32 and keys.is_cuda
    assert keys.is_contiguous() and values.is_contiguous() and keys.numel() == values.numel()
    n = keys.numel()
    ko, vo = out if out is not None else (torch.empty_like(keys), torch.empty_like(values))
    if temp is None:
        temp = torch.empty(max(int(_capi.lib().gsr_sort_temp_bytes(n)), 128), dtype=torch.uint8, device=keys.device)
    _capi.call("gsr_sort_pairs_u64_u32", keys.data_ptr(), ko.data_ptr(), values.data_ptr(), vo.data_ptr(), n, begin_bit, end_bit,
               temp.data_ptr(), _capi.stream(keys.device), device=keys.device)
    if sync:
        torch.cuda.current_stream(keys.device).synchronize()
    return ko, vo
```

Measured before the change: 4916.

## Gate backward chain work on per-gaussian touched flags set during render backward

Render backward, the flush kernel, and the features and distortion walks now mark each gaussian that actually receives a gradient in a uint8 touched buffer. The preprocess/chain backward then processes only flagged gaussians, clears their flags, and skips the SH loads for untouched rows. This replaces the radii-based visibility test, avoiding chain maths and memory traffic for gaussians that are visible but contributed no gradient. It adds byte writes and a scratch buffer, and new gated entry points are now the default in the Python backward path.

```diff
diff --git a/gsrast_amd/_capi.py b/gsrast_amd/_capi.py
--- a/gsrast_amd/_capi.py
+++ b/gsrast_amd/_capi.py
@@ -451,6 +451,12 @@
     "gsr_median_backward": (C.c_int, [C.POINTER(MedianArgs)]),
 }
 
+GATED_SIGNATURES = {
+    "gsr_backward_gated": (C.c_int, [C.POINTER(BackwardArgs), C.c_void_p, C.c_void_p]),
+    "gsr_features_backward_gated": (C.c_int, [C.POINTER(FeaturesArgs), C.c_void_p]),
+    "gsr_distortion_backward_gated": (C.c_int, [C.POINTER(DistortionArgs), C.c_void_p]),
+}
+
 _lib = None
 
 
@@ -475,7 +481,8 @@
                                   + list(MCMC_SIGNATURES.items()) + list(CONTRIB_SIGNATURES.items()) + list(ANTIALIAS_SIGNATURES.items())
                                   + list(FILTER3D_SIGNATURES.items()) + list(ABSGRAD_SIGNATURES.items())
                                   + list(FEATURES_SIGNATURES.items()) + list(DISTORTION_SIGNATURES.items())
-                                  + list(NORMALS_SIGNATURES.items()) + list(MEDIAN_SIGNATURES.items())):
+                                  + list(NORMALS_SIGNATURES.items()) + list(MEDIAN_SIGNATURES.items())
+                                  + list(GATED_SIGNATURES.items())):
             fn = getattr(L, name, None)
             if fn is None and _TAG:
                 continue
diff --git a/gsrast_amd/build.py b/gsrast_amd/build.py
--- a/gsrast_amd/build.py
+++ b/gsrast_amd/build.py
@@ -26,7 +26,8 @@
     paths = [os.path.join(CSRC, f) for f in os.listdir(CSRC) if f.endswith((".hpp", ".h"))]
     paths += [os.path.join(HERE, "..", "include", h) for h in ("gsrast_amd.h", "gsrast_amd_init.h", "gsrast_amd_opacity.h", "gsrast_amd_mcmc.h",
                                                                       "gsrast_amd_contrib.h", "gsrast_amd_antialias.h", "gsrast_amd_filter3d.h", "gsrast_amd_absgrad.h",
-                                                                      "gsrast_amd_features.h", "gsrast_amd_distortion.h", "gsrast_amd_normals.h", "gsrast_amd_median.h")]
+                                                                      "gsrast_amd_features.h", "gsrast_amd_distortion.h", "gsrast_amd_normals.h", "gsrast_amd_median.h",
+                                                                      "gsrast_amd_gated.h")]
     return max(os.path.getmtime(p) for p in paths)
 
 
diff --git a/gsrast_amd/csrc/backward.hip b/gsrast_amd/csrc/backward.hip
--- a/gsrast_amd/csrc/backward.hip
+++ b/gsrast_amd/csrc/backward.hip
@@ -3,6 +3,7 @@
 
 #include "backward_policy.hpp"
 #include "../../include/gsrast_amd_opacity.h"
+#include "../../include/gsrast_amd_gated.h"
 #include "blend_core.hpp"
 #include "blockbin.hpp"
 #include "gaussian_chain.hpp"
@@ -37,6 +38,7 @@
     float* dL_ddepths;
     double* depth_sums64;
     const float* dL_dout_alpha;
+    uint8_t* touched;
 };
 
 __device__ __forceinline__ float wave_sum12(float a0, float a1, float a2, float a3, float a4, float a5, float a6, float a7, float a8,
@@ -81,7 +83,8 @@
 __global__ __launch_bounds__(256) void flush_block_acc_kernel(const BlockFeed f, float* __restrict__ dL_dmean2D,
                                                               float* __restrict__ dL_dconic_opacity, float* __restrict__ dL_dcolors,
                                                               float* __restrict__ dL_dcov2D, double* __restrict__ sums64,
-                                                              float* __restrict__ dL_ddepths, double* __restrict__ depth_sums64) {
+                                                              float* __restrict__ dL_ddepths, double* __restrict__ depth_sums64,
+                                                              uint8_t* __restrict__ touched) {
     constexpr uint32_t kAcc = kAccOf<DEPTH>;
     size_t e0, e1;
     walked_slice<DEPTH>(f, e0, e1);
@@ -95,6 +98,7 @@
         for (int k = 0; k < (int)kAcc; ++k) any = any || v[k] != 0.0f;
         if (!any) continue;
         const size_t id = f.ent_idx[e];
+        if (touched) touched[id] = 1;
         if constexpr (DEPTH) {
             if (v[kAccFloats] != 0.0f) {
                 if (sums64) unsafeAtomicAdd(depth_sums64 + id, (double)v[kAccFloats]);
@@ -184,6 +188,7 @@
                          (my_sum < 9 ? p.dL_dcolors + (my_sum - 6) : p.dL_dcov2D + (my_sum - 9)));
     const uint32_t direct_stride = my_sum < 2 ? 2u : (my_sum < 6 ? 4u : (my_sum < 9 ? 3u : 4u));
     bool per_entry = false;
+    bool mark = false;
     auto walk_batch = [&](const bool present, const uint32_t id, const uint32_t idx_l, const uint32_t key, const float2 xy_l,
                           const float4 co_l) {
         const bool keep = present && !record_misses_tile(xy_l, co_l, box);
@@ -203,6 +208,7 @@
             const float op = co_l.w;
             s_floor[slot] = !(op > -__builtin_inff()) ? -__builtin_inff() : (op <= 0.0f ? __builtin_inff() : -__logf(255.0f * op) - 1e-3f);
         }
+        unsigned long long filed = 0ull;
         for (int j = (int)__popcll(kept_mask) - 1; j >= 0; --j) {
             const uint32_t idx0 = __float_as_uint(s_rgb[j].w);
             const float2 xy = s_xy[j];
@@ -255,6 +261,7 @@
                 a_m00 = __builtin_fmaf(hux, ux, a_m00); a_m01 = __builtin_fmaf(hux, uy, a_m01); a_m11 = __builtin_fmaf(huy, uy, a_m11);
             }
             if (!any) continue;
+            filed |= 1ull << j;
             const float total = wave_sum12(a_mx, a_my, a_A, a_B, a_C, a_op, a_r, a_g, a_b, a_m00, a_m01, a_m11);
             if (my_sum >= 0) {
                 const size_t key = s_id[j];
@@ -273,6 +280,7 @@
                 }
             }
         }
+        if (mark && (filed >> lane & 1ull)) p.touched[s_id[lane]] = 1;
     };
 
     struct Batch {
@@ -284,6 +292,7 @@
     const BlockFeed& f = p.feed;
     const uint32_t b = (uint32_t)(ty / kBH) * (uint32_t)f.nbx + (uint32_t)(tx / kBW);
     per_entry = f.ent_idx != nullptr && block_acc_fits<DEPTH>(f, b);
+    mark = p.touched != nullptr && !per_entry;
     const bool sorted = p.point_list && !per_entry;
     int it_c = (int)((hi - 1) / kWave);
     const uint32_t col = (uint32_t)(tx % kBW), row = 8u + (uint32_t)(ty % kBH), t_in_block = (uint32_t)((ty % kBH) * kBW + tx % kBW);
@@ -388,6 +397,7 @@
     const float* dL_ddepths;
     double* depth_sums64;
     float* out_ddepths;
+    uint8_t* touched;
 };
 
 __constant__ float kShC2[5] = {1.0925484305920792f, -1.0925484305920792f, 0.31539156525252005f, -1.0925484305920792f,
@@ -433,7 +443,8 @@
     __shared__ float s_sh[INRIA ? 4 * kWave * kShRow : 1];
     const int idx = blockIdx.x * 256 + threadIdx.x;
     const bool valid = idx < p.n;
-    const bool has_tile = valid && (p.radii == nullptr || p.radii[idx] > 0);
+    const bool flagged = p.touched != nullptr && valid && p.touched[idx] != 0;
+    const bool has_tile = p.touched ? flagged : valid && (p.radii == nullptr || p.radii[idx] > 0);
     const bool visible = has_tile && p.chain != 0;
     float4 mean = make_float4(0.0f, 0.0f, 0.0f, 0.0f), g = mean, sc = mean, rot = mean;
     float2 g2 = make_float2(0.0f, 0.0f), c3a = g2, c3b = g2, c3c = g2;
@@ -524,14 +535,16 @@
     if constexpr (INRIA) {
         if (p.dL_dshs) {
             const int terms = (p.sh_deg + 1) * (p.sh_deg + 1);
-            if (__ballot(visible) != 0ull) {
+            const unsigned long long vis_rows = __ballot(visible);
+            const unsigned long long rows = p.touched ? vis_rows : ~0ull;
+            if (vis_rows != 0ull) {
                 const int pieces = p.sh_deg > 2 ? 12 : (p.sh_deg > 1 ? 7 : (p.sh_deg > 0 ? 3 : 1));
                 float4 piece[12];
 #pragma unroll
                 for (int q = 0; q < 12; ++q) {
                     const int f4 = q * kWave + lane;
                     const size_t at = sh_first + 4 * (size_t)f4;
-                    piece[q] = ((f4 % 12) < pieces && at + 3 < sh_limit) ? *reinterpret_cast<const float4*>(p.shs + at)
+                    piece[q] = ((f4 % 12) < pieces && at + 3 < sh_limit && (rows >> (f4 / 12) & 1ull)) ? *reinterpret_cast<const float4*>(p.shs + at)
                                                                         : make_float4(0.0f, 0.0f, 0.0f, 0.0f);
                 }
 #pragma unroll
@@ -582,6 +595,7 @@
         scale_rotation_gradient(gS, Rm, sv, mod, gsc, gR);
         quaternion_gradient<INRIA>(gR, qn, inv, gq);
     }
+    if (p.touched && valid && flagged) p.touched[idx] = 0;
     if constexpr (INRIA) {
         if (p.dL_dshs) {
 #pragma unroll
@@ -605,10 +619,10 @@
             if (p.out_ddepths) p.out_ddepths[idx] = (float)gdep;
             if (gdep != 0.0) p.depth_sums64[idx] = 0.0;
         }
-        bool touched = false;
-#pragma unroll
-        for (int k = 0; k < 12; ++k) touched = touched || sum[k] != 0.0;
-        if (touched) {
+        bool nonzero = false;
+#pragma unroll
+        for (int k = 0; k < 12; ++k) nonzero = nonzero || sum[k] != 0.0;
+        if (nonzero) {
             double2* sp = reinterpret_cast<double2*>(p.sums64 + 12 * (size_t)idx);
 #pragma unroll
             for (int k = 0; k < 6; ++k) sp[k] = make_double2(0.0, 0.0);
@@ -652,12 +666,13 @@
     const hipStream_t stream;
     const BackwardChoice choice;
     const float* const dL_dout_alpha;
+    uint8_t* const touched;
     BlockFeed feed = {};
     bool from_blocks = false, lists_written = true, nothing_rendered = false;
     CallEvents<3> events;
 
-    BackwardCall(gsr_backward_args* a_, const BackwardChoice& choice_, const float* alpha_)
-        : a(a_), stream((hipStream_t)a_->stream), choice(choice_), dL_dout_alpha(alpha_) {}
+    BackwardCall(gsr_backward_args* a_, const BackwardChoice& choice_, const float* alpha_, uint8_t* touched_)
+        : a(a_), stream((hipStream_t)a_->stream), choice(choice_), dL_dout_alpha(alpha_), touched(touched_) {}
     int begin_profile() { if (choice.profile) GSR_TRY(events.create()); return mark(0); }
     int mark(int k) { if (choice.profile) GSR_HIP_TRY(hipEventRecord(events.ev[k], stream)); return GSR_OK; }
 };
@@ -724,6 +739,7 @@
     r.dL_ddepths = a->dL_ddepths;
     r.depth_sums64 = c.choice.wide ? a->depth_sums_f64 : nullptr;
     r.dL_dout_alpha = c.dL_dout_alpha;
+    r.touched = c.touched;
     return r;
 }
 
@@ -767,6 +783,7 @@
     q.depth_sums64 = r.depth_sums64;
     q.out_ddepths = a->dL_ddepths;
     q.shs = a->shs; q.cam_pos = a->cam_pos; q.clamped = a->clamped;
+    q.touched = c.touched;
     return q;
 }
 
@@ -786,7 +803,7 @@
     GSR_LAUNCH_CHECK("render_backward_kernel");
     if (per_entry) {
         hipLaunchKernelGGL(flush_block_acc_kernel<DEPTH>, dim3(acc_wgs), dim3(256), 0, c.stream, c.feed, a->dL_dmean2D,
-                           a->dL_dconic_opacity, a->dL_dcolors, a->dL_dcov2D, a->sums_f64, r.dL_ddepths, r.depth_sums64);
+                           a->dL_dconic_opacity, a->dL_dcolors, a->dL_dcov2D, a->sums_f64, r.dL_ddepths, r.depth_sums64, r.touched);
         GSR_LAUNCH_CHECK("flush_block_acc_kernel");
     }
     return GSR_OK;
@@ -830,14 +847,19 @@
 
 using namespace gsr;
 
-static int backward_impl(gsr_backward_args* a, const float* dL_dout_alpha) {
+static int backward_impl(gsr_backward_args* a, const float* dL_dout_alpha, uint8_t* touched) {
     if (!a || a->struct_size != sizeof(gsr_backward_args)) return GSR_ERR_INVALID_ARG;
     a->stage_ms[0] = a->stage_ms[1] = 0.0f;
     BackwardChoice choice;
-    GSR_TRY(choose_backward(*a, &choice, dL_dout_alpha));
-    BackwardCall call(a, choice, dL_dout_alpha);
+    GSR_TRY(choose_backward(*a, &choice, dL_dout_alpha, touched));
+    BackwardCall call(a, choice, dL_dout_alpha, touched);
     return backward_stages(call);
 }
 
-extern "C" int gsr_backward(gsr_backward_args* a) { return entry_point(backward_impl, a, (const float*)nullptr); }
-extern "C" int gsr_backward_alpha(gsr_backward_args* a, const float* dL_dout_alpha) { return entry_point(backward_impl, a, dL_dout_alpha); }
+extern "C" int gsr_backward(gsr_backward_args* a) { return entry_point(backward_impl, a, (const float*)nullptr, (uint8_t*)nullptr); }
+extern "C" int gsr_backward_alpha(gsr_backward_args* a, const float* dL_dout_alpha) {
+    return entry_point(backward_impl, a, dL_dout_alpha, (uint8_t*)nullptr);
+}
+extern "C" int gsr_backward_gated(gsr_backward_args* a, const float* dL_dout_alpha, uint8_t* touched) {
+    return entry_point(backward_impl, a, dL_dout_alpha, touched);
+}
diff --git a/gsrast_amd/csrc/backward_policy.hpp b/gsrast_amd/csrc/backward_policy.hpp
--- a/gsrast_amd/csrc/backward_policy.hpp
+++ b/gsrast_amd/csrc/backward_policy.hpp
@@ -16,10 +16,12 @@
     bool profile;
     bool depth_inverse;
     bool alpha;
+    bool gated;
     FrameDims d;
 };
 
-inline int choose_backward(const gsr_backward_args& a, BackwardChoice* out, const float* dL_dout_alpha = nullptr) {
+inline int choose_backward(const gsr_backward_args& a, BackwardChoice* out, const float* dL_dout_alpha = nullptr,
+                           const uint8_t* touched = nullptr) {
     BackwardChoice c{};
     if (a.num_gaussians <= 0 || a.width <= 0 || a.height <= 0 || !a.background || !a.means2D || !a.conic_opacity || !a.colors ||
         !a.ranges || !a.n_contrib || !a.final_t || !a.dL_dout_color)
@@ -35,6 +37,8 @@
     if (c.inria && a.dL_dshs && (!a.shs || !a.cam_pos || !a.clamped || !a.means3D)) return GSR_ERR_INVALID_ARG;
     c.depth = a.dL_dout_depth != nullptr;
     if (c.depth && (!a.means3D || !a.view_matrix || (c.wide ? !a.depth_sums_f64 : !a.dL_ddepths))) return GSR_ERR_INVALID_ARG;
+    c.gated = touched != nullptr;
+    if (c.gated && !c.chain && !c.wide) return GSR_ERR_INVALID_ARG;
     c.alpha = dL_dout_alpha != nullptr;
     c.profile = (a.flags & GSR_FLAG_PROFILE) != 0;
     c.depth_inverse = (a.flags & GSR_FLAG_DEPTH_INVERSE) != 0;
diff --git a/gsrast_amd/csrc/distortion.hip b/gsrast_amd/csrc/distortion.hip
--- a/gsrast_amd/csrc/distortion.hip
+++ b/gsrast_amd/csrc/distortion.hip
@@ -2,6 +2,7 @@
 
 #include "list_walk.hpp"
 #include "../../include/gsrast_amd_distortion.h"
+#include "../../include/gsrast_amd_gated.h"
 
 namespace gsr {
 namespace {
@@ -14,6 +15,7 @@
     const float* dL_dout;
     double* value_sums;
     double* geometry_sums;
+    uint8_t* geometry_touched;
 };
 
 struct DistortionStage : ReplayStage {
@@ -139,7 +141,7 @@
          [&](const int j) {
             const size_t id = st.id[j];
             if constexpr (GEO) {
-                const float total = geo.file(p.geometry_sums, id, lane, a_v);
+                const float total = geo.file(p.geometry_sums, p.geometry_touched, id, lane, a_v);
                 if (files_value && total != 0.0f) unsafeAtomicAdd(p.value_sums + id, (double)total);
             } else {
                 const float total = wave_sum2(a_v, 0.0f);
@@ -157,7 +159,7 @@
     return GSR_OK;
 }
 
-DistortionParams distortion_params(const gsr_distortion_args* a, const WalkFrame& frame) {
+DistortionParams distortion_params(const gsr_distortion_args* a, const WalkFrame& frame, uint8_t* geometry_touched = nullptr) {
     DistortionParams p;
     p.frame = frame;
     p.values = a->values;
@@ -166,6 +168,7 @@
     p.dL_dout = a->dL_dout;
     p.value_sums = a->value_sums_f64;
     p.geometry_sums = a->geometry_sums_f64;
+    p.geometry_touched = geometry_touched;
     return p;
 }
 
@@ -183,13 +186,14 @@
     });
 }
 
-int distortion_backward_impl(gsr_distortion_args* a) {
+int distortion_backward_impl(gsr_distortion_args* a, uint8_t* geometry_touched) {
     FrameDims d;
     bool nothing = false;
     GSR_TRY(distortion_check(a, true, &d, &nothing));
+    if (geometry_touched && !a->geometry_sums_f64) return GSR_ERR_INVALID_ARG;
     const WalkSums sums = {(size_t)a->num_gaussians, a->value_sums_f64, a->dL_dvalues};
     return walk_pass_call(a, d, nothing, &sums, [&](const WalkFrame& frame, unsigned blocks, hipStream_t stream) {
-        const DistortionParams p = distortion_params(a, frame);
+        const DistortionParams p = distortion_params(a, frame, geometry_touched);
         const bool square = a->power == 2, geo = a->geometry_sums_f64 != nullptr;
         const dim3 grid(blocks);
         if (square && geo) hipLaunchKernelGGL((distortion_backward_kernel<2, true>), grid, dim3(kWave), 0, stream, p);
@@ -208,4 +212,7 @@
     return num_gaussians <= 0 ? 0 : sizeof(double) * (size_t)num_gaussians;
 }
 extern "C" int gsr_distortion_forward(gsr_distortion_args* a) { return gsr::entry_point(gsr::distortion_forward_impl, a); }
-extern "C" int gsr_distortion_backward(gsr_distortion_args* a) { return gsr::entry_point(gsr::distortion_backward_impl, a); }
+extern "C" int gsr_distortion_backward(gsr_distortion_args* a) { return gsr::entry_point(gsr::distortion_backward_impl, a, (uint8_t*)nullptr); }
+extern "C" int gsr_distortion_backward_gated(gsr_distortion_args* a, uint8_t* geometry_touched) {
+    return gsr::entry_point(gsr::distortion_backward_impl, a, geometry_touched);
+}
diff --git a/gsrast_amd/csrc/features.hip b/gsrast_amd/csrc/features.hip
--- a/gsrast_amd/csrc/features.hip
+++ b/gsrast_amd/csrc/features.hip
@@ -2,6 +2,7 @@
 
 #include "list_walk.hpp"
 #include "../../include/gsrast_amd_features.h"
+#include "../../include/gsrast_amd_gated.h"
 
 namespace gsr {
 namespace {
@@ -19,6 +20,7 @@
     const float* dL_dout;
     double* feature_sums;
     double* geometry_sums;
+    uint8_t* geometry_touched;
     uint32_t channels;
 };
 
@@ -170,7 +172,7 @@
                 if (my_feat >= 0 && (uint32_t)(c + my_feat) < nc && total != 0.0f)
                     unsafeAtomicAdd(p.feature_sums + id * (size_t)p.channels + c0 + (uint32_t)(c + my_feat), (double)total);
             }
-            if constexpr (GEO) geo.file(p.geometry_sums, id, lane, 0.0f);
+            if constexpr (GEO) geo.file(p.geometry_sums, p.geometry_touched, id, lane, 0.0f);
         });
 }
 
@@ -183,7 +185,7 @@
     return GSR_OK;
 }
 
-FeatureParams feature_params(const gsr_features_args* a, const WalkFrame& frame) {
+FeatureParams feature_params(const gsr_features_args* a, const WalkFrame& frame, uint8_t* geometry_touched = nullptr) {
     FeatureParams p;
     p.frame = frame;
     p.features = a->features;
@@ -192,6 +194,7 @@
     p.dL_dout = a->dL_dout;
     p.feature_sums = a->feature_sums_f64;
     p.geometry_sums = a->geometry_sums_f64;
+    p.geometry_touched = geometry_touched;
     p.channels = (uint32_t)a->channels;
     return p;
 }
@@ -211,13 +214,14 @@
     });
 }
 
-int features_backward_impl(gsr_features_args* a) {
+int features_backward_impl(gsr_features_args* a, uint8_t* geometry_touched) {
     FrameDims d;
     bool nothing = false;
     GSR_TRY(features_check(a, true, &d, &nothing));
+    if (geometry_touched && !a->geometry_sums_f64) return GSR_ERR_INVALID_ARG;
     const WalkSums sums = {(size_t)a->num_gaussians * (size_t)a->channels, a->feature_sums_f64, a->dL_dfeatures};
     return walk_pass_call(a, d, nothing, &sums, [&](const WalkFrame& frame, unsigned blocks, hipStream_t stream) {
-        const FeatureParams p = feature_params(a, frame);
+        const FeatureParams p = feature_params(a, frame, geometry_touched);
         const int k = chunk_of(a->channels);
         const bool narrow = k == kChunkNarrow, geo = a->geometry_sums_f64 != nullptr;
         const dim3 grid(blocks, (unsigned)((a->channels + k - 1) / k));
@@ -238,4 +242,7 @@
     return sizeof(double) * (size_t)num_gaussians * (size_t)channels;
 }
 extern "C" int gsr_features_forward(gsr_features_args* a) { return gsr::entry_point(gsr::features_forward_impl, a); }
-extern "C" int gsr_features_backward(gsr_features_args* a) { return gsr::entry_point(gsr::features_backward_impl, a); }
+extern "C" int gsr_features_backward(gsr_features_args* a) { return gsr::entry_point(gsr::features_backward_impl, a, (uint8_t*)nullptr); }
+extern "C" int gsr_features_backward_gated(gsr_features_args* a, uint8_t* geometry_touched) {
+    return gsr::entry_point(gsr::features_backward_impl, a, geometry_touched);
+}
diff --git a/gsrast_amd/csrc/list_walk.hpp b/gsrast_amd/csrc/list_walk.hpp
--- a/gsrast_amd/csrc/list_walk.hpp
+++ b/gsrast_amd/csrc/list_walk.hpp
@@ -220,11 +220,12 @@
         const int of8 = sum8_of_lane(lane);
         slot = (lane & 7) == 0 ? (of8 < kExtra ? of8 : -1) : ((lane & 15) == 4 && kSumOfRow4[lane >> 4] < 12 ? kSumOfRow4[lane >> 4] : -1);
     }
-    __device__ __forceinline__ float file(double* geometry_sums, const size_t id, const int lane, const float extra) const {
+    __device__ __forceinline__ float file(double* geometry_sums, uint8_t* touched, const size_t id, const int lane, const float extra) const {
         const float t8 = wave_sum8(mx, my, A, B, C, op, extra, 0.0f, lane);
         const float t4 = wave_sum4(m00, m01, m11, 0.0f);
         const float total = (lane & 7) == 4 ? t4 : t8;
         if (slot >= 0 && total != 0.0f) unsafeAtomicAdd(geometry_sums + kFloats * id + (uint32_t)slot, (double)total);
+        if (touched != nullptr && lane == 0) touched[id] = 1;
         return t8;
     }
 };
diff --git a/gsrast_amd/rasterizer.py b/gsrast_amd/rasterizer.py
--- a/gsrast_amd/rasterizer.py
+++ b/gsrast_amd/rasterizer.py
@@ -68,10 +68,10 @@
             self.scratch[name] = torch.empty(shape, dtype=dtype, device=self.device)
         return self.scratch[name]
 
-    def sums(self, name: str, *shape) -> torch.Tensor:
+    def sums(self, name: str, *shape, dtype=torch.float64) -> torch.Tensor:
         t = self.scratch.get(name)
         if t is None or t.numel() < int(np.prod(shape)):
-            t = self.scratch[name] = torch.zeros(shape, dtype=torch.float64, device=self.device)
+            t = self.scratch[name] = torch.zeros(shape, dtype=dtype, device=self.device)
         return t
 
     def take(self, plan: backward_plan.BackwardPlan, semantics: str, with_cov3D: bool, into: "dict | None") -> dict:
@@ -422,7 +422,7 @@
                  outputs: "tuple[str, ...] | None" = None, dL_ddepth: "torch.Tensor | None" = None,
                  depth: "bool | str | None" = None, camera: bool = False, into: "dict | None" = None,
                  sync: bool = True, dL_dalpha: "torch.Tensor | None" = None, features: "tuple | None" = None,
-                 distortion: "tuple | None" = None) -> dict:
+                 distortion: "tuple | None" = None, gate_untouched: bool = True) -> dict:
         n, dev = self.num_gaussians, self.device
         rcpt = self.last_receipt if receipt is None else (None if receipt is False else receipt)
         if distortion is not None:
@@ -464,6 +464,8 @@
             a.scale_modifier = scale_modifier
         if tile_rows is not None:
             a.tile_row_begin, a.tile_row_end = int(tile_rows[0]), int(tile_rows[1])
+        gated = gate_untouched and (wide_sums or bool(a.dL_dcov3D)) and hasattr(self.lib, "gsr_backward_gated")
+        touched = self._bw.sums("touched", n, dtype=torch.uint8).data_ptr() if gated else None
         feature_call = None
         if features is not None:
             feature_call, feature_keep = self._features_call(rcpt, features[0], features[2] if len(features) > 2 else None,
@@ -475,19 +477,28 @@
         try:
             if feature_call is not None:
                 feature_call.geometry_sums_f64 = a.sums_f64
-                _capi.call("gsr_features_backward", C.byref(feature_call), device=dev)
+                if gated:
+                    _capi.call("gsr_features_backward_gated", C.byref(feature_call), touched, device=dev)
+                else:
+                    _capi.call("gsr_features_backward", C.byref(feature_call), device=dev)
             if distortion_call is not None:
                 distortion_call.geometry_sums_f64 = a.sums_f64
-                _capi.call("gsr_distortion_backward", C.byref(distortion_call), device=dev)
-            if dL_dalpha is None:
+                if gated:
+                    _capi.call("gsr_distortion_backward_gated", C.byref(distortion_call), touched, device=dev)
+                else:
+                    _capi.call("gsr_distortion_backward", C.byref(distortion_call), device=dev)
+            ga = None if dL_dalpha is None else dL_dalpha.contiguous()
+            if gated:
+                _capi.call("gsr_backward_gated", C.byref(a), None if ga is None else ga.data_ptr(), touched, device=dev)
+            elif ga is None:
                 _capi.call("gsr_backward", C.byref(a), device=dev)
             else:
-                ga = dL_dalpha.contiguous()
                 _capi.call("gsr_backward_alpha", C.byref(a), ga.data_ptr(), device=dev)
         except _capi.GsrError:
             if wide_sums:
                 self._bw.scratch.pop("sums_f64", None)
                 self._bw.scratch.pop("depth_sums_f64", None)
+            self._bw.scratch.pop("touched", None)
             self._bw.scratch.pop("feature_sums_f64", None)
             self._bw.scratch.pop("distortion_sums_f64", None)
             raise
diff --git a/include/gsrast_amd_gated.h b/include/gsrast_amd_gated.h
--- /dev/null
+++ b/include/gsrast_amd_gated.h
@@ -0,0 +1,19 @@
+#ifndef GSRAST_AMD_GATED_H
+#define GSRAST_AMD_GATED_H
+
+#include "gsrast_amd.h"
+#include "gsrast_amd_distortion.h"
+#include "gsrast_amd_features.h"
+
+#ifdef __cplusplus
+extern "C" {
+#endif
+
+int gsr_backward_gated(gsr_backward_args* args, const float* dL_dout_alpha, uint8_t* touched);
+int gsr_features_backward_gated(gsr_features_args* args, uint8_t* geometry_touched);
+int gsr_distortion_backward_gated(gsr_distortion_args* args, uint8_t* geometry_touched);
+
+#ifdef __cplusplus
+}
+#endif
+#endif
```

Result: no change. 4907 (-0.2%).
